# amazon-science/crossnorm-selfnorm

Hardware: AMD Instinct MI355X
Metric: fused CNSN fwd+bwd GB/s vs HBM roofline (higher is better)
Workload: dtype f32

## Files before the change

### crossnorm-selfnorm_amd/_ffi.py

```python
from __future__ import annotations

import ctypes as C
import os

_HERE = os.path.dirname(os.path.abspath(__file__))
LIB_PATH = os.environ.get("CNSN_LIB_PATH") or os.path.join(_HERE, "libcnsn_hip.so")

CNSN_F32, CNSN_BF16, CNSN_F16 = 0, 1, 2
STRATEGY_AUTO, STRATEGY_TWO_PASS, STRATEGY_RESIDENT, STRATEGY_LOCAL, STRATEGY_MONO = 0, 1, 2, 3, 4
ADD_NONE, ADD_PRE, ADD_POST = 0, 1, 2
LAYOUT_NCHW, LAYOUT_NHWC = 0, 1
PATHS = {0: "streaming", 1: "packed", 2: "resident", 3: "local", 4: "mono"}
ABI_VERSION = 9
PERM_INLINE_MAX = 1024
E_UNSUPPORTED = -9


class Problem(C.Structure):
    _fields_ = [
        ("struct_bytes", C.c_int32), ("dtype", C.c_int32),
        ("N", C.c_int32), ("C", C.c_int32), ("H", C.c_int32), ("W", C.c_int32),
        ("cn_active", C.c_int32), ("content_box", C.c_int32 * 4), ("style_box", C.c_int32 * 4),
        ("lam", C.c_float), ("eps_cn", C.c_float),
        ("sn_active", C.c_int32), ("sn_two", C.c_int32), ("sn_training", C.c_int32),
        ("eps_sn", C.c_float), ("eps_bn", C.c_float), ("momentum", C.c_float),
        ("strategy", C.c_int32), ("layout", C.c_int32),
        ("context", C.c_void_p), ("context_bytes", C.c_uint64),
        ("perm_host", C.c_void_p),
    ]


class Gate(C.Structure):
    _fields_ = [("fc_weight", C.c_void_p), ("bn_weight", C.c_void_p), ("bn_bias", C.c_void_p),
                ("running_mean", C.c_void_p), ("running_var", C.c_void_p), ("num_batches_tracked", C.c_void_p)]


class GateGrad(C.Structure):
    _fields_ = [("d_fc_weight", C.c_void_p), ("d_bn_weight", C.c_void_p), ("d_bn_bias", C.c_void_p)]


class BnTail(C.Structure):
    _fields_ = [("struct_bytes", C.c_int32), ("training", C.c_int32), ("eps", C.c_float), ("momentum", C.c_float),
                ("weight", C.c_void_p), ("bias", C.c_void_p), ("running_mean", C.c_void_p), ("running_var", C.c_void_p),
                ("num_batches_tracked", C.c_void_p)]


class Ibn(C.Structure):
    _fields_ = [("struct_bytes", C.c_int32), ("dtype", C.c_int32), ("N", C.c_int32), ("C", C.c_int32), ("H", C.c_int32),
                ("W", C.c_int32), ("half", C.c_int32), ("relu", C.c_int32), ("eps_in", C.c_float), ("reserved", C.c_int32),
                ("in_weight", C.c_void_p), ("in_bias", C.c_void_p), ("bn", BnTail), ("context", C.c_void_p),
                ("context_bytes", C.c_uint64)]


class BnAct(C.Structure):
    _fields_ = [("struct_bytes", C.c_int32), ("dtype", C.c_int32), ("N", C.c_int32), ("C", C.c_int32), ("H", C.c_int32),
                ("W", C.c_int32), ("relu", C.c_int32), ("add", C.c_int32), ("bn", BnTail), ("context", C.c_void_p),
                ("context_bytes", C.c_uint64)]


class ArenaStats(C.Structure):
    _fields_ = [("struct_bytes", C.c_int32), ("device", C.c_int32), ("chunk_bytes", C.c_uint64), ("mapped_bytes", C.c_uint64),
                ("in_use_bytes", C.c_uint64), ("blocks", C.c_uint64), ("blocks_in_use", C.c_uint64), ("hits", C.c_uint64),
                ("misses", C.c_uint64), ("failed", C.c_uint64), ("probed", C.c_uint64), ("tries", C.c_uint64),
                ("evicted", C.c_uint64), ("limit_bytes", C.c_uint64), ("broken", C.c_uint64)]


class Epilogue(C.Structure):
    _fields_ = [("struct_bytes", C.c_int32), ("add_mode", C.c_int32), ("relu", C.c_int32),
                ("reserved", C.c_int32), ("addend", C.c_void_p), ("sum_out", C.c_void_p)]


SIGNATURES = {
    "cnsn_abi_version": (C.c_int, []),
    "cnsn_status_string": (C.c_char_p, [C.c_int]),
    "cnsn_context_bytes": (C.c_size_t, [C.POINTER(Problem)]),
    "cnsn_context_init": (C.c_int, [C.c_void_p, C.c_size_t, C.c_void_p]),
    "cnsn_resident_timeouts": (C.c_int, []),
    "cnsn_resident_enable": (None, [C.c_int]),
    "cnsn_resident_rearm": (C.c_int, []),
    "cnsn_resident_degraded": (C.c_int, []),
    "cnsn_reload_env": (None, []),
    "cnsn_set_wait_ms": (None, [C.c_int]),
    "cnsn_wait_ms": (C.c_int, []),
    "cnsn_set_headroom_cus": (None, [C.c_int]),
    "cnsn_headroom_cus": (C.c_int, []),
    "cnsn_arena_map": (C.c_void_p, [C.c_size_t, C.c_int, C.c_void_p]),
    "cnsn_arena_unmap": (None, [C.c_void_p, C.c_size_t, C.c_int, C.c_void_p]),
    "cnsn_arena_alloc": (C.c_void_p, [C.c_int, C.c_size_t, C.c_void_p]),
    "cnsn_arena_record_stream": (C.c_int, [C.c_void_p, C.c_void_p]),
    "cnsn_arena_set_limit": (C.c_int, [C.c_int, C.c_uint64]),
    "cnsn_arena_free": (C.c_int, [C.c_void_p]),
    "cnsn_arena_trim": (C.c_size_t, [C.c_int]),
    "cnsn_arena_owns": (C.c_int, [C.c_void_p]),
    "cnsn_arena_stats": (C.c_int, [C.c_int, C.POINTER(ArenaStats)]),
    "cnsn_arena_set_chunk_bytes": (C.c_int, [C.c_size_t]),
    "cnsn_arena_prospect": (C.c_int, [C.c_int, C.c_size_t, C.c_int, C.c_int, C.c_void_p, C.POINTER(C.c_float)]),
    "cnsn_arena_block_gbps": (C.c_int, [C.c_void_p, C.POINTER(C.c_float)]),
    "cnsn_arena_set_tries": (C.c_int, [C.c_int]),
    "cnsn_saved_floats": (C.c_size_t, [C.POINTER(Problem)]),
    "cnsn_workspace_bytes": (C.c_size_t, [C.POINTER(Problem)]),
    "cnsn_forward": (C.c_int, [C.POINTER(Problem), C.c_void_p, C.c_void_p, C.c_void_p,
                               C.POINTER(Gate), C.POINTER(Gate), C.c_void_p, C.c_void_p,
                               C.c_void_p, C.c_size_t, C.c_void_p]),
    "cnsn_backward": (C.c_int, [C.POINTER(Problem), C.c_void_p, C.c_void_p, C.c_void_p, C.c_void_p,
                                C.POINTER(Gate), C.POINTER(Gate), C.c_void_p, C.c_void_p,
                                C.POINTER(GateGrad), C.POINTER(GateGrad), C.c_void_p, C.c_size_t,
                                C.c_void_p]),
    "cnsn_forward_fused": (C.c_int, [C.POINTER(Problem), C.POINTER(Epilogue), C.c_void_p, C.c_void_p,
                                     C.c_void_p, C.POINTER(Gate), C.POINTER(Gate), C.c_void_p,
                                     C.c_void_p, C.c_void_p, C.c_size_t, C.c_void_p]),
    "cnsn_backward_fused": (C.c_int, [C.POINTER(Problem), C.POINTER(Epilogue), C.c_void_p, C.c_void_p,
                                      C.c_void_p, C.c_void_p, C.POINTER(Gate), C.POINTER(Gate),
                                      C.c_void_p, C.c_void_p, C.c_void_p, C.POINTER(GateGrad),
                                      C.POINTER(GateGrad), C.c_void_p, C.c_size_t, C.c_void_p]),
    "cnsn_which_path": (C.c_int, [C.POINTER(Problem), C.POINTER(Epilogue), C.c_int, C.c_int]),
    "cnsn_keeps_sum": (C.c_int, [C.POINTER(Problem), C.POINTER(Epilogue)]),
    "cnsn_sn_cluster_plan": (C.c_int, [C.POINTER(Problem), C.POINTER(Epilogue), C.c_int]),
    "cnsn_bnrelu_plan": (C.c_int, [C.POINTER(Problem), C.POINTER(Epilogue), C.c_int]),
    "cnsn_bn_block_plan": (C.c_int, [C.POINTER(Problem), C.POINTER(Epilogue)]),
    "cnsn_forward_bn_block": (C.c_int, [C.POINTER(Problem), C.POINTER(Epilogue), C.POINTER(BnTail), C.POINTER(BnTail), C.c_void_p,
                                        C.POINTER(Gate), C.c_void_p, C.c_void_p, C.c_void_p, C.c_void_p, C.c_size_t, C.c_void_p]),
    "cnsn_backward_bn_block": (C.c_int, [C.POINTER(Problem), C.POINTER(Epilogue), C.POINTER(BnTail), C.POINTER(BnTail), C.c_void_p,
                                         C.c_void_p, C.POINTER(Gate), C.c_void_p, C.c_void_p, C.c_void_p, C.c_void_p,
                                         C.POINTER(GateGrad), C.c_void_p, C.c_void_p, C.c_void_p, C.c_void_p, C.c_void_p, C.c_size_t,
                                         C.c_void_p]),
    "cnsn_forward_bnrelu": (C.c_int, [C.POINTER(Problem), C.POINTER(Epilogue), C.POINTER(BnTail), C.c_void_p,
                                      C.POINTER(Gate), C.c_void_p, C.c_void_p, C.c_void_p, C.c_void_p, C.c_void_p,
                                      C.c_size_t, C.c_void_p]),
    "cnsn_backward_bnrelu": (C.c_int, [C.POINTER(Problem), C.POINTER(Epilogue), C.POINTER(BnTail), C.c_void_p, C.c_void_p,
                                       C.c_void_p, C.POINTER(Gate), C.c_void_p, C.c_void_p, C.c_void_p,
                                       C.POINTER(GateGrad), C.c_void_p, C.c_void_p, C.c_void_p, C.c_size_t, C.c_void_p]),
    "cnsn_ibn_plan": (C.c_int, [C.POINTER(Ibn), C.c_int, C.c_int]),
    "cnsn_ibn_saved_floats": (C.c_size_t, [C.POINTER(Ibn)]),
    "cnsn_ibn_workspace_bytes": (C.c_size_t, [C.POINTER(Ibn)]),
    "cnsn_forward_ibn": (C.c_int, [C.POINTER(Ibn), C.c_void_p, C.c_void_p, C.c_void_p, C.c_void_p, C.c_void_p, C.c_size_t,
                                   C.c_void_p]),
    "cnsn_backward_ibn": (C.c_int, [C.POINTER(Ibn), C.c_void_p, C.c_void_p, C.c_void_p, C.c_void_p, C.c_void_p, C.c_void_p,
                                    C.c_void_p, C.c_void_p, C.c_void_p, C.c_void_p, C.c_size_t, C.c_void_p]),
    "cnsn_bn_act_plan": (C.c_int, [C.POINTER(BnAct), C.c_int, C.c_int]),
    "cnsn_bn_act_saved_floats": (C.c_size_t, [C.POINTER(BnAct)]),
    "cnsn_bn_act_workspace_bytes": (C.c_size_t, [C.POINTER(BnAct)]),
    "cnsn_forward_bn_act": (C.c_int, [C.POINTER(BnAct), C.c_void_p, C.c_void_p, C.c_void_p, C.c_void_p, C.c_void_p, C.c_size_t,
                                      C.c_void_p]),
    "cnsn_backward_bn_act": (C.c_int, [C.POINTER(BnAct), C.c_void_p, C.c_void_p, C.c_void_p, C.c_void_p, C.c_void_p, C.c_void_p,
                                       C.c_void_p, C.c_void_p, C.c_void_p, C.c_size_t, C.c_void_p]),
    "cnsn_jsd_workspace_bytes": (C.c_size_t, [C.c_int]),
    "cnsn_jsd": (C.c_int, [C.c_void_p, C.c_void_p, C.c_void_p, C.c_int, C.c_int, C.c_int, C.c_void_p,
                           C.c_void_p, C.c_void_p, C.c_void_p, C.c_void_p, C.c_size_t, C.c_void_p]),
    "cnsn_plane_stats": (C.c_int, [C.c_void_p, C.c_int, C.c_int, C.c_int, C.c_int, C.c_int,
                                   C.POINTER(C.c_int32), C.c_float, C.c_void_p, C.c_void_p]),
    "cnsn_plane_stats_backward": (C.c_int, [C.c_void_p, C.c_int, C.c_int, C.c_int, C.c_int, C.c_int,
                                            C.POINTER(C.c_int32), C.c_void_p, C.c_void_p,
                                            C.c_void_p, C.c_void_p, C.c_void_p, C.c_void_p]),
    "cnsn_plane_affine": (C.c_int, [C.c_void_p, C.c_int, C.c_int, C.c_int, C.c_int, C.c_int,
                                    C.c_void_p, C.c_void_p, C.c_void_p, C.c_void_p]),
    "cnsn_plane_dot": (C.c_int, [C.c_void_p, C.c_void_p, C.c_int, C.c_int, C.c_int, C.c_int,
                                 C.c_int, C.c_void_p, C.c_void_p]),
    "cnsn_plane_dot_shifted": (C.c_int, [C.c_void_p, C.c_void_p, C.c_int, C.c_int, C.c_int, C.c_int,
                                         C.c_int, C.c_void_p, C.c_void_p, C.c_void_p]),
    "cnsn_plane_combine": (C.c_int, [C.c_void_p, C.c_void_p, C.c_int, C.c_int, C.c_int, C.c_int,
                                     C.c_int, C.c_void_p, C.c_void_p, C.c_void_p]),
}

_lib = None


class CnsnError(RuntimeError):
    pass


def lib():
    global _lib
    if _lib is None:
        if not os.path.exists(LIB_PATH):
            raise CnsnError(
                f"{LIB_PATH} is missing: the CrossNorm/SelfNorm HIP library has not been built. "
                "Run `python __graft_entry__.py` (hipcc --offload-arch=gfx950). There is no "
                "CPU or eager fallback.")
        handle = C.CDLL(LIB_PATH)
        for name, (res, args) in SIGNATURES.items():
            fn = getattr(handle, name)
            fn.restype, fn.argtypes = res, args
        got = handle.cnsn_abi_version()
        if got != ABI_VERSION:
            raise CnsnError(f"libcnsn_hip.so ABI {got} != binding ABI {ABI_VERSION}")
        _lib = handle
    return _lib


GLUE_DIR = os.path.join(_HERE, "_glue")
GLUE_PATH = os.path.join(GLUE_DIR, "cnsn_glue.so")
_glue = None
_glue_tried = False


def glue():
    global _glue, _glue_tried
    if _glue_tried:
        return _glue
    _glue_tried = True
    if os.environ.get("CNSN_NO_GLUE") == "1" or not os.path.exists(GLUE_PATH):
        return None
    lib()
    C.CDLL(LIB_PATH, mode=C.RTLD_GLOBAL)
    import importlib.machinery
    import importlib.util
    import torch
    loader = importlib.machinery.ExtensionFileLoader("cnsn_glue", GLUE_PATH)
    spec = importlib.util.spec_from_loader("cnsn_glue", loader)
    mod = importlib.util.module_from_spec(spec)
    loader.exec_module(mod)
    if mod.abi_version() != ABI_VERSION:
        raise CnsnError(f"cnsn_glue.so was built against ABI {mod.abi_version()}, binding expects {ABI_VERSION}")
    _glue = mod
    return _glue


_timeouts_reported = 0
_defer_depth = 0


def _timeout_count() -> int:
    return lib().cnsn_resident_timeouts()


_TIMEOUT_TEXT = ("{what}: an earlier cluster-resident launch timed out waiting for part of its grid ({n} so far) — the GPU "
                 "is shared with work that kept it off the device for seconds.  The outputs of the step that was in flight "
                 "are invalid: repeat it.  The library now uses the two-pass kernels (CNSN_RESIDENT=0 selects them from "
                 "the start).")


def check_resident_health(what: str):
    global _timeouts_reported
    if _defer_depth:
        return
    n = _timeout_count()
    if n > _timeouts_reported:
        _timeouts_reported = n
        raise CnsnError(_TIMEOUT_TEXT.format(what=what, n=n))


class deferred_timeouts:

    def __enter__(self):
        global _defer_depth
        _defer_depth += 1
        return self

    def __exit__(self, *exc):
        global _defer_depth
        _defer_depth -= 1
        return False


def poll_timeouts() -> int:
    global _timeouts_reported
    n = _timeout_count()
    new = max(0, n - _timeouts_reported)
    _timeouts_reported = max(n, _timeouts_reported)
    return new


def settle_step(device=None, raise_on_timeout: bool = True) -> int:
    import torch
    torch.cuda.current_stream(device).synchronize()
    if not raise_on_timeout:
        return poll_timeouts()
    check_resident_health("training step")
    return 0


_plan_caches = []


def forget_plans():
    for c in _plan_caches:
        c.clear()


def reload_env():
    lib().cnsn_reload_env()
    forget_plans()


_following = False


def follow_environ():
    global _following
    if _following:
        return
    _following = True
    put, unset = os.putenv, os.unsetenv

    def reread(key):
        if os.fsdecode(key).startswith("CNSN_") and _lib is not None:
            _lib.cnsn_reload_env()
            forget_plans()

    def putenv(key, value):
        put(key, value)
        reread(key)

    def unsetenv(key):
        unset(key)
        reread(key)

    os.putenv, os.unsetenv = putenv, unsetenv


def default_headroom_cus() -> int:
    try:
        ch = int(os.environ.get("NCCL_MAX_NCHANNELS", "") or 16)
    except ValueError:
        ch = 16
    return max(0, min(2 * ch, 64))


def under_process_group_defaults() -> dict:
    try:
        import torch.distributed as dist
        if not (dist.is_available() and dist.is_initialized() and dist.get_world_size() > 1):
            return {}
        handle = lib()
        if "CNSN_WAIT_MS" not in os.environ:
            handle.cnsn_set_wait_ms(2000)
        if "CNSN_HEADROOM_CUS" not in os.environ:
            handle.cnsn_set_headroom_cus(default_headroom_cus())
            forget_plans()
        return {"wait_ms": int(handle.cnsn_wait_ms()), "headroom_cus": int(handle.cnsn_headroom_cus())}
    except Exception:
        return {}


def check(status: int, what: str):
    if status != 0:
        msg = lib().cnsn_status_string(status).decode()
        if status == -7:
            raise ValueError(f"{what}: {msg}")
        raise CnsnError(f"{what} failed with status {status}: {msg}")


def box4(b):
    arr = (C.c_int32 * 4)(-1, -1, -1, -1)
    if b is not None:
        for i in range(4):
            arr[i] = int(b[i])
    return arr
```

### crossnorm-selfnorm_amd/callers/_sites.py

```python
import os

import numpy as np
import torch

FUSE_BLOCK = os.environ.get("CNSN_FUSE_BLOCK", "1") != "0"
FUSE_TAIL = FUSE_BLOCK and os.environ.get("CNSN_FUSE_TAIL", "1") != "0"
FUSE_BN_ACT = os.environ.get("CNSN_BN_ACT", "1") != "0"


def residual_sum(cnsn, pos, residual, skip, relu, skip_first=False):
    fb = getattr(cnsn, "forward_block", None) if (FUSE_BLOCK and cnsn is not None) else None
    fusable = (fb is not None and pos in ("post", "residual", "identity") and residual.is_cuda
               and residual.shape == skip.shape and residual.dtype == skip.dtype)
    if fusable:
        if pos == "post":
            a, b = (skip, residual) if skip_first else (residual, skip)
            return fb(a, b, add_mode="pre", relu=relu)
        if pos == "residual":
            return fb(residual, skip, add_mode="post", relu=relu)
        return fb(skip, residual, add_mode="post", relu=relu)
    if pos == "residual":
        residual = cnsn(residual)
    elif pos == "identity":
        skip = cnsn(skip)
    y = torch.add(skip, residual) if skip_first else residual + skip
    if pos == "post":
        y = cnsn(y)
    return torch.relu(y) if relu else y


def make_cnsn(impl, cnsn_type, crop, beta, width):
    assert cnsn_type in ("sn", "cn", "cnsn")
    cross = impl.CrossNorm(crop=crop, beta=beta) if "cn" in cnsn_type else None
    selfn = impl.SelfNorm(width) if "sn" in cnsn_type else None
    return impl.CNSN(crossnorm=cross, selfnorm=selfn)


class CrossNormSites:

    def _collect_sites(self, impl, cnsn_type, active_num):
        object.__setattr__(self, "cn_modules", [m for m in self.modules() if isinstance(m, impl.CrossNorm)])
        if cnsn_type is not None and "cn" in cnsn_type:
            self.cn_num = len(self.cn_modules)
            self.active_num = active_num
            assert self.cn_num > 0 and self.active_num > 0

    def _enable_cross_norm(self):
        picked = np.random.choice(self.cn_num, self.active_num, replace=False).tolist()
        for i in picked:
            self.cn_modules[i].active = True
        return picked
```

### crossnorm-selfnorm_amd/callers/resnet.py

```python
import torch
import torch.nn as nn

from . import _sites
from ._sites import CrossNormSites, make_cnsn, residual_sum
from .bn_act import bn_act
from .ibn import IBN, InstanceNorm2d


class _Bottleneck(nn.Module):
    expansion = 4

    def __init__(self, impl, c_in, planes, stride, downsample, pos, beta, crop, cnsn_type, ibn=None):
        super().__init__()
        c_out = planes * self.expansion
        self.ibn = ibn
        self.conv1 = nn.Conv2d(c_in, planes, 1, bias=False)
        self.bn1 = IBN(planes) if ibn == "a" else nn.BatchNorm2d(planes)
        self.conv2 = nn.Conv2d(planes, planes, 3, stride, 1, bias=False)
        self.bn2 = nn.BatchNorm2d(planes)
        self.conv3 = nn.Conv2d(planes, c_out, 1, bias=False)
        self.bn3 = nn.BatchNorm2d(c_out)
        if ibn == "b":
            self.IN = InstanceNorm2d(c_out, affine=True)
        self.relu = nn.ReLU(inplace=True)
        self.downsample = downsample
        if ibn == "b" and pos == "post":
            cnsn_type = None
        if cnsn_type is not None:
            assert pos in ("residual", "pre", "post", "identity")
            self.cnsn = make_cnsn(impl, cnsn_type, crop, beta, c_in if pos == "pre" else c_out)
        self.pos = pos if cnsn_type is not None else None

    def forward(self, x):
        h = self.cnsn(x) if self.pos == "pre" else x
        h = self.conv1(h)
        h = self.bn1.forward_act(h) if self.ibn == "a" else bn_act(self.bn1, h)
        h = bn_act(self.bn2, self.conv2(h))
        h = self.conv3(h)
        if self.ibn == "b":
            skip = x if self.downsample is None else self.downsample(x)
            h = self.bn3(h)
            if self.pos == "residual":
                h = self.cnsn(h)
            elif self.pos == "identity":
                skip = self.cnsn(skip)
            return self.IN.forward_act(h, skip, relu=True)
        fb = getattr(getattr(self, "cnsn", None), "forward_bn_block", None) if (_sites.FUSE_BLOCK and self.pos == "post") else None
        if fb is not None and h.is_cuda:
            if self.downsample is None:
                return fb(h, self.bn3, x, relu=True)
            if len(self.downsample) == 2 and isinstance(self.downsample[1], nn.BatchNorm2d):
                return fb(h, self.bn3, self.downsample[0](x), relu=True, identity_bn=self.downsample[1])
            return fb(h, self.bn3, self.downsample(x), relu=True)
        skip = x if self.downsample is None else self.downsample(x)
        if getattr(self, "cnsn", None) is None:
            return bn_act(self.bn3, h, skip)
        return residual_sum(self.cnsn, self.pos, self.bn3(h), skip, relu=True)


class ResNet50CNSN(nn.Module, CrossNormSites):
    def __init__(self, num_classes=1000, layers=(3, 4, 6, 3), active_num=1, pos="post", beta=None, crop=None,
                 cnsn_type="sn", impl=None):
        super().__init__()
        if impl is None:
            from .. import cnsn as impl
        self.conv1 = nn.Conv2d(3, 64, 7, 2, 3, bias=False)
        self.bn1 = nn.BatchNorm2d(64)
        self.relu = nn.ReLU(inplace=True)
        self.maxpool = nn.MaxPool2d(3, 2, 1)
        kw = dict(pos=pos, beta=beta, crop=crop, cnsn_type=cnsn_type)
        c_in = 64
        for i, (planes, blocks) in enumerate(zip((64, 128, 256, 512), layers)):
            stride = 1 if i == 0 else 2
            units = []
            for b in range(blocks):
                down = None
                if b == 0 and (stride != 1 or c_in != planes * 4):
                    down = nn.Sequential(nn.Conv2d(c_in, planes * 4, 1, stride, bias=False), nn.BatchNorm2d(planes * 4))
                units.append(_Bottleneck(impl, c_in, planes, stride if b == 0 else 1, down, **kw))
                c_in = planes * 4
            setattr(self, f"layer{i + 1}", nn.Sequential(*units))
        self.avgpool = nn.AdaptiveAvgPool2d((1, 1))
        self.fc = nn.Linear(c_in, num_classes)
        for m in self.modules():
            if isinstance(m, nn.Conv2d):
                nn.init.kaiming_normal_(m.weight, mode="fan_out", nonlinearity="relu")
            elif isinstance(m, nn.BatchNorm2d):
                nn.init.constant_(m.weight, 1)
                nn.init.constant_(m.bias, 0)
        self._collect_sites(impl, cnsn_type, active_num)

    def forward(self, x, aug=False):
        if aug:
            self._enable_cross_norm()
        x = self.maxpool(bn_act(self.bn1, self.conv1(x)))
        x = self.layer4(self.layer3(self.layer2(self.layer1(x))))
        return self.fc(torch.flatten(self.avgpool(x), 1))
```

### crossnorm-selfnorm_amd/cnsn.py

```python
from __future__ import annotations

import functools
from dataclasses import dataclass
from typing import Optional, Tuple

import numpy as np
import torch
import torch.nn as nn

from . import functional as _F
from .functional import FusedConfig, GateParams

__all__ = ["calc_ins_mean_std", "instance_norm_mix", "cn_rand_bbox", "cn_op_2ins_space_chan",
           "CrossNorm", "SelfNorm", "CNSN"]

Box = Tuple[int, int, int, int]
_CROPS = ("neither", "style", "content", "both")


def _is_f64(x) -> bool:
    return isinstance(x, torch.Tensor) and x.dtype == torch.float64


def calc_ins_mean_std(x, eps=1e-5):
    assert x.dim() == 4
    if _is_f64(x):
        mean, std = _F.PlaneStats.apply(x.float(), float(eps), None, True)
        return mean.double(), std.double()
    return _F.PlaneStats.apply(x, float(eps), None)


def instance_norm_mix(content_feat, style_feat):
    assert content_feat.size()[:2] == style_feat.size()[:2]
    if _is_f64(content_feat):
        return instance_norm_mix(content_feat.float(), style_feat.float()).double()
    s_mean, s_std = calc_ins_mean_std(style_feat)
    c_mean, c_std = calc_ins_mean_std(content_feat)
    scale = s_std.float() / c_std.float()
    shift = s_mean.float() - c_mean.float() * scale
    return _F.PlaneAffine.apply(content_feat, scale, shift)


def cn_rand_bbox(size, beta, bbx_thres):
    ext2, ext3 = int(size[2]), int(size[3])
    plane = float(ext2 * ext3)
    while True:
        side = np.sqrt(np.random.beta(beta, beta))
        half2, half3 = int(ext2 * side) // 2, int(ext3 * side) // 2
        mid2 = np.random.randint(ext2)
        mid3 = np.random.randint(ext3)
        x1, x2 = max(mid2 - half2, 0), min(mid2 + half2, ext2)
        y1, y2 = max(mid3 - half3, 0), min(mid3 + half3, ext3)
        if (x2 - x1) * (y2 - y1) / plane > bbx_thres:
            return int(x1), int(y1), int(x2), int(y2)


@dataclass
class CNDraws:
    perm: torch.Tensor
    style_box: Optional[Box] = None
    chan_perm: Optional[torch.Tensor] = None
    content_box: Optional[Box] = None


def draw_cn(size, crop, beta, bbx_thres=0.1, chan=False) -> CNDraws:
    assert crop in _CROPS
    d = CNDraws(perm=torch.randperm(int(size[0])))
    if crop in ("style", "both"):
        d.style_box = cn_rand_bbox(size, beta=beta, bbx_thres=bbx_thres)
    if chan:
        d.chan_perm = torch.randperm(int(size[1]))
    if crop in ("content", "both"):
        d.content_box = cn_rand_bbox(size, beta=beta, bbx_thres=bbx_thres)
    return d


def _cn_config(d: CNDraws, lam) -> FusedConfig:
    return FusedConfig(cn_active=True, content_box=d.content_box, style_box=d.style_box, lam=lam)


def cn_op_2ins_space_chan(x, crop='neither', beta=1, bbx_thres=0.1, lam=None, chan=False, draws=None):
    assert crop in _CROPS
    if draws is None:
        draws = draw_cn(x.size(), crop, beta, bbx_thres, chan)
    if _is_f64(x):
        return _F.fused_cnsn(x.float(), _cn_config(draws, lam), perm=draws.perm, chan_perm=draws.chan_perm).double()
    return _F.fused_cnsn(x, _cn_config(draws, lam), perm=draws.perm, chan_perm=draws.chan_perm)


class CrossNorm(nn.Module):

    def __init__(self, crop=None, beta=None):
        super().__init__()
        self.active = False
        self.crop, self.beta = crop, beta
        self.cn_op = functools.partial(cn_op_2ins_space_chan, crop=crop, beta=beta)
        self.next_draws: Optional[CNDraws] = None

    def _take_draws(self, x) -> CNDraws:
        d, self.next_draws = self.next_draws, None
        return d if d is not None else draw_cn(x.size(), self.crop, self.beta)

    def forward(self, x):
        if self.training and self.active:
            x = self.cn_op(x, draws=self._take_draws(x))
        self.active = False
        return x


class SelfNorm(nn.Module):

    def __init__(self, chan_num, is_two=False):
        super().__init__()
        self.g_fc = nn.Conv1d(chan_num, chan_num, kernel_size=2, bias=False, groups=chan_num)
        self.g_bn = nn.BatchNorm1d(chan_num)
        if is_two is True:
            self.f_fc = nn.Conv1d(chan_num, chan_num, kernel_size=2, bias=False, groups=chan_num)
            self.f_bn = nn.BatchNorm1d(chan_num)
        else:
            self.f_fc = None

    @staticmethod
    def _gate(fc, bn, counter=None) -> GateParams:
        rm, rv = bn.running_mean, bn.running_var
        if rm is None or rv is None:
            w = fc.weight
            rm = torch.zeros(w.shape[0], dtype=torch.float32, device=w.device)
            rv = torch.ones(w.shape[0], dtype=torch.float32, device=w.device)
        return GateParams(fc.weight, bn.weight, bn.bias, rm, rv, counter)

    @staticmethod
    def _bn_call_state(bn, in_kernel=False):
        momentum = 0.0 if bn.momentum is None else float(bn.momentum)
        counter = None
        if bn.training and bn.track_running_stats and bn.num_batches_tracked is not None:
            if in_kernel and bn.momentum is not None and bn.num_batches_tracked.is_cuda and not _F.LEGACY_LAUNCHES:
                counter = bn.num_batches_tracked
            else:
                bn.num_batches_tracked.add_(1)
                if bn.momentum is None:
                    momentum = 1.0 / float(bn.num_batches_tracked)
        use_batch = bn.training or (bn.running_mean is None and bn.running_var is None)
        if in_kernel:
            return use_batch, float(bn.eps), momentum, counter
        return use_batch, float(bn.eps), momentum

    @staticmethod
    def _bn_peek(bn):
        use_batch = bn.training or (bn.running_mean is None and bn.running_var is None)
        return use_batch, float(bn.eps), (None if bn.momentum is None else float(bn.momentum)), bool(
            bn.training and bn.track_running_stats)

    def _fusable(self) -> bool:
        mods = self._modules
        g_bn = mods["g_bn"]

        def affine(bn):
            par, own = bn._parameters, bn.__dict__
            return (par.get("weight") if "weight" in par else own.get("weight")) is not None and \
                   (par.get("bias") if "bias" in par else own.get("bias")) is not None

        if type(g_bn) is not nn.BatchNorm1d or not affine(g_bn):
            return False
        if self.f_fc is None:
            return True
        f_bn = mods["f_bn"]
        if type(f_bn) is not nn.BatchNorm1d or not affine(f_bn):
            return False
        return self._bn_peek(g_bn) == self._bn_peek(f_bn)

    def _forward_composed(self, x):
        b, c = int(x.size(0)), int(x.size(1))
        mean, std = _F.PlaneStats.apply(x, 1e-12, None, True)
        with torch.autocast(device_type=x.device.type, enabled=False):
            stats = torch.cat((mean.view(b, c, 1), std.view(b, c, 1)), -1)
            g_y = torch.sigmoid(self.g_bn(self.g_fc(stats))).view(b, c, 1, 1)
            if self.f_fc is not None:
                f_y = torch.sigmoid(self.f_bn(self.f_fc(stats))).view(b, c, 1, 1)
                shift = mean * (f_y - g_y)
            else:
                shift = torch.zeros_like(g_y)
        return _F.PlaneAffine.apply(x, g_y, shift)

    def _fused_args(self):
        *state, counter = self._bn_call_state(self.g_bn, in_kernel=True)
        state = tuple(state)
        g = self._gate(self.g_fc, self.g_bn, counter)
        f = None
        if self.f_fc is not None:
            *state_f, counter_f = self._bn_call_state(self.f_bn, in_kernel=True)
            state_f = tuple(state_f)
            if state_f != state:
                raise _F._ffi.CnsnError(
                    "SelfNorm(is_two=True): g_bn and f_bn must share mode, eps and momentum "
                    f"(g_bn: training/eps/momentum = {state}, f_bn: {state_f})")
            f = self._gate(self.f_fc, self.f_bn, counter_f)
        use_batch, eps, momentum = state
        kw = dict(sn_active=True, sn_two=f is not None, sn_training=use_batch, eps_bn=eps, momentum=momentum)
        return kw, g, f

    def _fused_args_peek(self):
        bn = self.g_bn
        use_batch = bn.training or (bn.running_mean is None and bn.running_var is None)
        kw = dict(sn_active=True, sn_two=self.f_fc is not None, sn_training=use_batch, eps_bn=float(bn.eps),
                  momentum=0.0 if bn.momentum is None else float(bn.momentum))
        return kw, None, None

    def forward(self, x):
        if _is_f64(x):
            return self.forward(x.float()).double()
        if not self._fusable():
            return self._forward_composed(x)
        kw, g, f = self._fused_args()
        return _F.fused_cnsn(x, FusedConfig(**kw), g=g, f=f)


class CNSN(nn.Module):

    def __init__(self, crossnorm, selfnorm):
        super().__init__()
        self.crossnorm = crossnorm
        self.selfnorm = selfnorm

    def forward(self, x):
        if _is_f64(x):
            return self.forward(x.float()).double()
        cn, sn = self.crossnorm, self.selfnorm
        fuse = (cn is not None and sn is not None and type(cn) is CrossNorm and type(sn) is SelfNorm and sn._fusable()
                and cn.active and cn.training)
        if not fuse:
            if cn and cn.active:
                x = cn(x)
            if sn:
                x = sn(x)
            return x
        d = cn._take_draws(x)
        cn.active = False
        kw, g, f = sn._fused_args()
        cfg = FusedConfig(cn_active=True, content_box=d.content_box, style_box=d.style_box, **kw)
        return _F.fused_cnsn(x, cfg, perm=d.perm, chan_perm=d.chan_perm, g=g, f=f)

    def forward_block(self, x, addend=None, add_mode="none", relu=False):
        assert add_mode in ("none", "pre", "post")
        assert (addend is None) == (add_mode == "none")
        if _is_f64(x):
            return self.forward_block(x.float(), None if addend is None else addend.float(), add_mode, relu).double()
        cn, sn = self.crossnorm, self.selfnorm
        ours = (cn is None or type(cn) is CrossNorm) and (sn is None or (type(sn) is SelfNorm and sn._fusable()))
        cn_on = cn is not None and cn.active and cn.training
        if not ours or not (cn_on or sn is not None):
            if add_mode == "pre":
                x = x + addend
            x = self.forward(x)
            if add_mode == "post":
                x = x + addend
            return torch.relu(x) if relu else x
        kw, g, f, perm, chan = {}, None, None, None, None
        if cn is not None and cn.active:
            if cn_on:
                d = cn._take_draws(x)
                kw.update(cn_active=True, content_box=d.content_box, style_box=d.style_box)
                perm, chan = d.perm, d.chan_perm
            cn.active = False
        if sn is not None:
            skw, g, f = sn._fused_args()
            kw.update(skw)
        cfg = FusedConfig(add_mode=add_mode, relu=bool(relu), **kw)
        return _F.fused_cnsn(x, cfg, perm=perm, chan_perm=chan, g=g, f=f, addend=addend)

    def forward_bn_block(self, conv_out, bn, identity, relu=True, identity_bn=None):
        cn, sn = self.crossnorm, self.selfnorm
        armed = cn is not None and cn.active

        def plain(m):
            return type(m) is nn.BatchNorm2d and m.affine and m.track_running_stats and m.training
        fused = (plain(bn) and (identity_bn is None or plain(identity_bn)) and sn is not None
                 and type(sn) is SelfNorm and sn.f_fc is None and sn._fusable() and not armed and conv_out.is_cuda
                 and (cn is None or type(cn) is CrossNorm) and identity.shape == conv_out.shape
                 and identity.dtype == conv_out.dtype and not torch.cuda.is_current_stream_capturing())
        if fused:
            kw, _, _ = sn._fused_args_peek()
            fused = kw["sn_training"] and _F.bn_block_plan(conv_out, FusedConfig(add_mode="pre", relu=bool(relu), **kw))
        if not fused:
            skip = identity if identity_bn is None else identity_bn(identity)
            return self.forward_block(bn(conv_out), skip, add_mode="pre", relu=relu)
        kw, g, _ = sn._fused_args()
        _, bn_eps, bn_mom, bn_counter = SelfNorm._bn_call_state(bn, in_kernel=True)
        cfg = FusedConfig(add_mode="pre", relu=bool(relu), **kw)
        extra = ()
        if identity_bn is not None:
            _, e2, m2, c2 = SelfNorm._bn_call_state(identity_bn, in_kernel=True)
            extra = (identity_bn.weight, identity_bn.bias, identity_bn.running_mean, identity_bn.running_var, e2, m2, c2)
        return _F.FusedBnBlock.apply(conv_out, identity, cfg, g.fc_weight, g.bn_weight, g.bn_bias, g.running_mean, g.running_var,
                                     bn.weight, bn.bias, bn.running_mean, bn.running_var, bn_eps, bn_mom, g.num_batches_tracked,
                                     bn_counter, *extra)

    def forward_block_bn(self, x, addend, add_mode, bn, want_y=True):
        assert add_mode in ("none", "pre")
        cn, sn = self.crossnorm, self.selfnorm
        armed = cn is not None and cn.active
        fused = (type(bn) is nn.BatchNorm2d and bn.affine and bn.track_running_stats and sn is not None
                 and type(sn) is SelfNorm and sn.f_fc is None and sn._fusable() and not armed and x.is_cuda
                 and (cn is None or type(cn) is CrossNorm))
        if fused:
            kw, g, _ = sn._fused_args_peek()
            cfg = FusedConfig(add_mode=add_mode, relu=False, **kw)
            fused = _F.bnrelu_plan_cached(x, cfg, torch.is_grad_enabled())
        if not fused:
            y = self.forward_block(x, addend, add_mode=add_mode, relu=False) if add_mode != "none" else self.forward(x)
            return (y if want_y else None), torch.relu(bn(y))
        kw, g, _ = sn._fused_args()
        bn_batch, bn_eps, bn_mom, bn_counter = SelfNorm._bn_call_state(bn, in_kernel=True)
        cfg = FusedConfig(add_mode=add_mode, relu=False, **kw)
        return _F.fused_cnsn_tail(x, cfg, addend, bool(want_y), g, bn.weight, bn.bias, bn.running_mean, bn.running_var,
                                  bn_batch, bn_eps, bn_mom, bn_counter)
```

### crossnorm-selfnorm_amd/csrc/cnsn_env.h

```cpp
#pragma once

namespace cnsn {

enum Knob {
    K_LOCAL_LB = 0,
    K_LOCAL_CG,
    K_STAGGER,
    K_WAIT_MS,
    K_FAULT_INJECT,
    K_DEBUG,
    K_PROF,
    K_MONO,
    K_MONO_RELOAD,
    K_NO_PACKED,
    K_MID_TILE,
    K_SNX,
    K_RESIDENT,
    K_CONTEXT,
    K_EPOCH_START,
    K_KEEP,
    K_PIPE,
    K_WIDE,
    K_PONG,
    K_SNXCN,
    K_ARENA_CHUNK_MB,
    K_XCD,
    K_HEADROOM_CUS,
    K_ARENA_TRIES,
    K_ARENA_SPREAD_GB,
    K_MID_BLOCK,
    K_NHWC_FUSED,
    K_ARENA_MAX_MB,
    K_COUNT
};

const char* knob(Knob k);
void reload_knobs();

}
```

### crossnorm-selfnorm_amd/csrc/cnsn_env.hip

```cpp
#include "cnsn_env.h"

#include <cstdlib>
#include <mutex>
#include <string>

namespace cnsn {
namespace {

const char* const kNames[K_COUNT] = {
    "CNSN_LOCAL_LB", "CNSN_LOCAL_CG", "CNSN_STAGGER",     "CNSN_WAIT_MS", "CNSN_FAULT_INJECT", "CNSN_DEBUG",
    "CNSN_PROF",     "CNSN_MONO",     "CNSN_MONO_RELOAD", "CNSN_NO_PACKED", "CNSN_MID_TILE",   "CNSN_SNX",
    "CNSN_RESIDENT", "CNSN_CONTEXT",  "CNSN_EPOCH_START", "CNSN_KEEP",    "CNSN_PIPE",         "CNSN_WIDE",
    "CNSN_PONG",
    "CNSN_SNXCN",
    "CNSN_ARENA_CHUNK_MB",
    "CNSN_XCD",
    "CNSN_HEADROOM_CUS",
    "CNSN_ARENA_TRIES",
    "CNSN_ARENA_SPREAD_GB",
    "CNSN_MID_BLOCK",
    "CNSN_NHWC_FUSED",
    "CNSN_ARENA_MAX_MB",
};

struct Table {
    std::string text[K_COUNT];
    const char* value[K_COUNT];
    std::mutex mu;
    Table() { read(); }
    void read() {
        std::lock_guard<std::mutex> lock(mu);
        for (int k = 0; k < K_COUNT; ++k) {
            const char* e = getenv(kNames[k]);
            if (e) {
                text[k] = e;
                value[k] = text[k].c_str();
            } else {
                text[k].clear();
                value[k] = nullptr;
            }
        }
    }
};

Table& table() {
    static Table t;
    return t;
}

struct AtLoad {
    AtLoad() { (void)table(); }
} g_at_load;

}

const char* knob(Knob k) { return table().value[k]; }
void reload_knobs() { table().read(); }

}
```

### crossnorm-selfnorm_amd/csrc/cnsn_fused.hip

```cpp
#include "../../include/cnsn_hip.h"

#include <hip/hip_runtime.h>

#include "cnsn_fused_stream_kernels.h"
#include "cnsn_host_plan.h"
#include "cnsn_local.h"
#include "cnsn_mono.h"
#include "cnsn_nhwc.h"
#include "cnsn_wide.h"
#include "cnsn_packed.h"
#include "cnsn_resident_fused.h"
#include "cnsn_resident_sn.h"

using namespace cnsn;

namespace {

struct EpiPlan {
    int add;
    int relu;
    const void* addend;
    void* sum_out;
};

int parse_epilogue(const cnsn_epilogue_t* epi, EpiPlan& e) {
    e = EpiPlan{ADD_NONE, 0, nullptr, nullptr};
    if (!epi) return CNSN_OK;
    if (epi->struct_bytes != (int32_t)sizeof(cnsn_epilogue_t)) return CNSN_E_STRUCT;
    if (epi->add_mode != CNSN_ADD_NONE && epi->add_mode != CNSN_ADD_PRE && epi->add_mode != CNSN_ADD_POST)
        return CNSN_E_UNSUPPORTED;
    e.add = epi->add_mode;
    e.relu = epi->relu ? 1 : 0;
    e.addend = epi->addend;
    if (e.add != ADD_NONE) {
        if (!e.addend) return CNSN_E_NULL;
        if (((uintptr_t)e.addend & 15u) != 0) return CNSN_E_ALIGN;
    }
    e.sum_out = epi->sum_out;
    if (e.sum_out) {
        if (e.add != ADD_PRE) return CNSN_E_UNSUPPORTED;
        if (((uintptr_t)e.sum_out & 15u) != 0) return CNSN_E_ALIGN;
    }
    return CNSN_OK;
}

int parse_epilogue_shape(const cnsn_epilogue_t* epi, EpiPlan& e) {
    e = EpiPlan{ADD_NONE, 0, nullptr, nullptr};
    if (!epi) return CNSN_OK;
    if (epi->struct_bytes != (int32_t)sizeof(cnsn_epilogue_t)) return CNSN_E_STRUCT;
    if (epi->add_mode != CNSN_ADD_NONE && epi->add_mode != CNSN_ADD_PRE && epi->add_mode != CNSN_ADD_POST)
        return CNSN_E_UNSUPPORTED;
    e.add = epi->add_mode;
    e.relu = epi->relu ? 1 : 0;
    return CNSN_OK;
}

template <typename F>
inline void with_add(int add, F&& f) {
    if (add == ADD_PRE)
        f(IntTag<ADD_PRE>{});
    else if (add == ADD_POST)
        f(IntTag<ADD_POST>{});
    else
        f(IntTag<ADD_NONE>{});
}

}

extern "C" {

int cnsn_which_path(const cnsn_problem_t* prob, const cnsn_epilogue_t* epi, int has_chan_perm, int backward) {
    EpiPlan e;
    int st = parse_epilogue_shape(epi, e);
    if (st) return st;
    Plan pl;
    st = make_plan(prob, pl);
    if (st) return st;
    const cnsn_problem_t& p = pl.pr;
    const bool chan = p.cn_active && has_chan_perm;
    const bool bwd = backward != 0;
    if (p.layout == CNSN_LAYOUT_NHWC)
        return (chan || !nhwc_supported(pl, false)) ? CNSN_E_UNSUPPORTED : (nhwc_fused_ok(pl) ? CNSN_PATH_RESIDENT : CNSN_PATH_STREAMING);
    const bool fused = bwd ? (e.relu || e.add == ADD_PRE) : (e.relu || e.add != ADD_NONE);
    if (resident_sn_prefers(p, pl.boxed, fused ? e.add : ADD_NONE, fused ? e.relu : 0, bwd)) return CNSN_PATH_RESIDENT;
    if (wide_plan(pl, fused ? e.add : 0, bwd, chan).ok) return CNSN_PATH_MONO;
    if (mono_plan(pl, fused ? e.add : 0, bwd).ok) return CNSN_PATH_MONO;
    if (mono_cn_plan(pl, chan, fused ? e.add : 0, bwd).ok) return CNSN_PATH_MONO;
    if (local_plan(pl, fused ? e.add : 0, bwd).ok) return CNSN_PATH_LOCAL;
    if (resident_sn_plan(p, pl.boxed, fused ? e.add : ADD_NONE, fused ? e.relu : 0, bwd).ok) return CNSN_PATH_RESIDENT;
    if (bwd && !fused && resident_sn_cn_plan(p, pl.boxed, chan).ok) return CNSN_PATH_RESIDENT;
    if (fused ? resident_fused_plan(p, pl.boxed, chan, e.add, bwd).ok : resident_plan(p, pl.boxed, chan, bwd).ok)
        return CNSN_PATH_RESIDENT;
    if (resident_split_plan(p, pl.boxed, chan, fused ? e.add : ADD_NONE, fused ? e.relu : 0, bwd).ok) return CNSN_PATH_RESIDENT;
    PackedGeom pg;
    return packed_plan(pl, pg) ? CNSN_PATH_PACKED : CNSN_PATH_STREAMING;
}

int cnsn_sn_cluster_plan(const cnsn_problem_t* prob, const cnsn_epilogue_t* epi, int backward) {
    EpiPlan e;
    int st = parse_epilogue_shape(epi, e);
    if (st) return st;
    Plan pl;
    st = make_plan(prob, pl);
    if (st) return st;
    const bool bwd = backward != 0;
    const bool fused = bwd ? (e.relu || e.add == ADD_PRE) : (e.relu || e.add != ADD_NONE);
    if (pl.pr.layout == CNSN_LAYOUT_NHWC) return 0;
    if (resident_sn_prefers(pl.pr, pl.boxed, fused ? e.add : ADD_NONE, fused ? e.relu : 0, bwd)) return 1;
    if (wide_plan(pl, fused ? e.add : 0, bwd).ok || mono_plan(pl, fused ? e.add : 0, bwd).ok ||
        local_plan(pl, fused ? e.add : 0, bwd).ok)
        return 0;
    if (bwd && !fused && resident_sn_cn_plan(pl.pr, pl.boxed, false).ok) return 1;
    return resident_sn_plan(pl.pr, pl.boxed, fused ? e.add : ADD_NONE, fused ? e.relu : 0, bwd).ok ? 1 : 0;
}

int cnsn_keeps_sum(const cnsn_problem_t* prob, const cnsn_epilogue_t* epi) {
    EpiPlan e;
    if (!prob || parse_epilogue_shape(epi, e) != CNSN_OK || e.add != ADD_PRE || prob->layout != CNSN_LAYOUT_NHWC) return 0;
    Plan pl;
    if (make_plan(prob, pl) != CNSN_OK) return 0;
    return nhwc_supported(pl, false) ? 1 : 0;
}

namespace {
int bn_block_parse(const cnsn_problem_t* prob, const cnsn_epilogue_t* epi, const cnsn_bn_tail_t* bn, Plan& pl, EpiPlan& e, bool shape_only,
                   bool check_health = true) {
    int st = shape_only ? parse_epilogue_shape(epi, e) : parse_epilogue(epi, e);
    if (st) return st;
    st = make_plan(prob, pl);
    if (st) return st;
    if (bn && bn->struct_bytes != (int32_t)sizeof(cnsn_bn_tail_t)) return CNSN_E_STRUCT;
    if (pl.pr.layout != CNSN_LAYOUT_NHWC || e.add != ADD_PRE || e.sum_out || !nhwc_bnhead_ok(pl, check_health) || (bn && !bn->training))
        return CNSN_E_UNSUPPORTED;
    return CNSN_OK;
}
}

int cnsn_bn_block_plan(const cnsn_problem_t* prob, const cnsn_epilogue_t* epi) {
    Plan pl;
    EpiPlan e;
    const int st = bn_block_parse(prob, epi, nullptr, pl, e, true);
    return st == CNSN_OK ? 1 : (st == CNSN_E_UNSUPPORTED ? 0 : st);
}

int cnsn_forward_bn_block(const cnsn_problem_t* prob, const cnsn_epilogue_t* epi, const cnsn_bn_tail_t* bn,
                          const cnsn_bn_tail_t* bn_skip, const void* conv_out, const cnsn_gate_t* g, void* y, float* saved, float* bn_stats,
                          void* workspace, size_t workspace_bytes, void* stream_) {
    if (!bn) return CNSN_E_NULL;
    if (bn_skip && (bn_skip->struct_bytes != (int32_t)sizeof(cnsn_bn_tail_t))) return CNSN_E_STRUCT;
    if (bn_skip && (!bn_skip->weight || !bn_skip->bias || !bn_skip->running_mean || !bn_skip->running_var)) return CNSN_E_NULL;
    if (bn_skip && !bn_skip->training) return CNSN_E_UNSUPPORTED;
    Plan pl;
    EpiPlan e;
    const int st = bn_block_parse(prob, epi, bn, pl, e, false);
    if (st) return st;
    if (!conv_out || !y || !workspace || !bn_stats || !bn->weight || !bn->bias || !bn->running_mean || !bn->running_var) return CNSN_E_NULL;
    if ((((uintptr_t)conv_out | (uintptr_t)y | (uintptr_t)workspace | (uintptr_t)bn_stats) & 15u) != 0) return CNSN_E_ALIGN;
    if (!gate_ok(g)) return CNSN_E_NULL;
    return nhwc_bnhead_forward(pl, e.relu, *bn, bn_skip, conv_out, e.addend, gate_dev(g), y, saved, bn_stats, workspace, workspace_bytes,
                               (hipStream_t)stream_);
}

int cnsn_backward_bn_block(const cnsn_problem_t* prob, const cnsn_epilogue_t* epi, const cnsn_bn_tail_t* bn,
                           const cnsn_bn_tail_t* bn_skip, const void* grad_y, const void* conv_out, const cnsn_gate_t* g, const float* saved,
                           const float* bn_stats, void* grad_conv_out, void* grad_identity, const cnsn_gate_grad_t* dg, float* d_bn_weight,
                           float* d_bn_bias, float* d_bn_skip_weight, float* d_bn_skip_bias, void* workspace, size_t workspace_bytes,
                           void* stream_) {
    if (!bn) return CNSN_E_NULL;
    if (bn_skip && (bn_skip->struct_bytes != (int32_t)sizeof(cnsn_bn_tail_t))) return CNSN_E_STRUCT;
    if (bn_skip && (!bn_skip->weight || !d_bn_skip_weight || !d_bn_skip_bias)) return CNSN_E_NULL;
    Plan pl;
    EpiPlan e;
    const int st = bn_block_parse(prob, epi, bn, pl, e, false, false);
    if (st) return st;
    if (!grad_y || !conv_out || !grad_conv_out || !grad_identity || !saved || !bn_stats || !workspace || !bn->weight) return CNSN_E_NULL;
    if ((((uintptr_t)grad_y | (uintptr_t)conv_out | (uintptr_t)grad_conv_out | (uintptr_t)grad_identity | (uintptr_t)workspace |
          (uintptr_t)bn_stats) & 15u) != 0)
        return CNSN_E_ALIGN;
    if (!gate_ok(g) || !dg || !dg->d_fc_weight || !dg->d_bn_weight || !dg->d_bn_bias) return CNSN_E_NULL;
    return nhwc_bnhead_backward(pl, e.relu, *bn, bn_skip, grad_y, conv_out, e.addend, gate_dev(g), saved, bn_stats, grad_conv_out,
                                grad_identity, gate_grad_dev(dg), d_bn_weight, d_bn_bias, d_bn_skip_weight, d_bn_skip_bias, workspace,
                                workspace_bytes, (hipStream_t)stream_);
}

int cnsn_forward_fused(const cnsn_problem_t* prob, const cnsn_epilogue_t* epi, const void* x, const int64_t* perm,
                       const int64_t* chan_perm, const cnsn_gate_t* g, const cnsn_gate_t* f, void* y, float* saved,
                       void* workspace, size_t workspace_bytes, void* stream_) {
    EpiPlan e;
    int st = parse_epilogue(epi, e);
    if (st) return st;
    if (prob && prob->layout == CNSN_LAYOUT_NHWC) {
        Plan pl;
        st = make_plan(prob, pl);
        if (st) return st;
        if (!x || !y || !workspace) return CNSN_E_NULL;
        if ((((uintptr_t)x | (uintptr_t)y | (uintptr_t)workspace) & 15u) != 0) return CNSN_E_ALIGN;
        if (chan_perm || !nhwc_supported(pl, false)) return CNSN_E_UNSUPPORTED;
        if (pl.pr.sn_active && !gate_ok(g)) return CNSN_E_NULL;
        if (pl.pr.sn_active && pl.pr.sn_two && !gate_ok(f)) return CNSN_E_NULL;
        return nhwc_forward(pl, e.add, e.relu, x, e.addend, perm, gate_dev(g), gate_dev(f), y, saved, workspace, workspace_bytes,
                            (hipStream_t)stream_, e.sum_out);
    }
    if (e.sum_out) return CNSN_E_UNSUPPORTED;
    if (e.add == ADD_NONE && !e.relu)
        return cnsn_forward(prob, x, perm, chan_perm, g, f, y, saved, workspace, workspace_bytes, stream_);
    Plan pl;
    st = make_plan(prob, pl);
    if (st) return st;
    const cnsn_problem_t& p = pl.pr;
    if (!x || !y || !workspace) return CNSN_E_NULL;
    if ((((uintptr_t)x | (uintptr_t)y | (uintptr_t)workspace) & 15u) != 0) return CNSN_E_ALIGN;
    const bool perm_inline = p.cn_active && !perm;
    if (perm_inline && (!p.perm_host || chan_perm || p.N > CNSN_PERM_INLINE_MAX)) return p.perm_host ? CNSN_E_UNSUPPORTED : CNSN_E_NULL;
    if (p.sn_active && !gate_ok(g)) return CNSN_E_NULL;
    if (p.sn_active && p.sn_two && !gate_ok(f)) return CNSN_E_NULL;
    if (workspace_bytes < workspace_bytes_of(pl)) return CNSN_E_WORKSPACE;
    hipStream_t stream = (hipStream_t)stream_;
    pl.mid.save_coefs = (e.relu && saved) ? 1 : 0;

    double* mom = (double*)workspace;
    double* saved_d = saved ? (double*)saved : mom + 6 * pl.P;
    float* coef = (float*)(mom + 6 * pl.P + saved_doubles_of(pl));

    if (resident_sn_prefers(p, pl.boxed, e.add, e.relu, false)) {
        st = resident_sn_forward(pl.pr, pl.mid, e.add, e.relu, x, e.addend, gate_dev(g), y, saved ? saved_d : nullptr, workspace,
                                 stream);
        if (st != CNSN_E_UNSUPPORTED) return st;
    }
    {
        const WidePlan wp = wide_plan(pl, e.add, false, chan_perm != nullptr);
        if (wp.ok && !perm_inline) {
            st = wide_forward(pl, wp, e.add, e.relu, x, e.addend, perm, gate_dev(g), y, saved ? saved_d : nullptr, stream);
            if (st != CNSN_E_UNSUPPORTED) return st;
        }
    }
    {
        const MonoPlan mp = mono_plan(pl, e.add, false);
        if (mp.ok) {
            st = mono_forward(pl, mp, e.add, e.relu, x, e.addend, gate_dev(g), gate_dev(f), y, saved ? saved_d : nullptr, stream);
            if (st != CNSN_E_UNSUPPORTED) return st;
        }
    }
    {
        const MonoPlan mp = mono_cn_plan(pl, chan_perm != nullptr, e.add, false);
        if (mp.ok && !perm_inline) {
            st = mono_cn_forward(pl, mp, e.add, e.relu, x, e.addend, perm, gate_dev(g), y, saved ? saved_d : nullptr, stream);
            if (st != CNSN_E_UNSUPPORTED) return st;
        }
    }
    {
        const LocalPlan lp = local_plan(pl, e.add, false);
        if (lp.ok) {
            st = local_forward(pl, lp, e.add, e.relu, x, e.addend, gate_dev(g), gate_dev(f), y, saved ? saved_d : nullptr,
                               stream);
            if (st != CNSN_E_UNSUPPORTED) return st;
        }
    }
    if (resident_sn_plan(p, pl.boxed, e.add, e.relu, false).ok) {
        st = resident_sn_forward(pl.pr, pl.mid, e.add, e.relu, x, e.addend, gate_dev(g), y, saved ? saved_d : nullptr, workspace,
                                 stream);
        if (st != CNSN_E_UNSUPPORTED) return st;
    }
    if (resident_fused_plan(p, pl.boxed, p.cn_active && chan_perm != nullptr, e.add, false).ok) {
        st = resident_fused_forward(pl.pr, pl.cb, pl.sb, pl.boxed, pl.mid, e.add, e.relu, x, e.addend, perm, gate_dev(g),
                                    gate_dev(f), y, saved ? saved_d : nullptr, workspace, stream);
        if (st != CNSN_E_UNSUPPORTED) return st;
    }
    if (resident_split_plan(p, pl.boxed, p.cn_active && chan_perm != nullptr, e.add, e.relu, false).ok) {
        st = resident_split_forward(pl.pr, pl.cb, pl.sb, pl.boxed, pl.mid, e.add, e.relu, x, e.addend, perm, gate_dev(g),
                                    gate_dev(f), y, saved ? saved_d : nullptr, workspace, stream);
        if (st != CNSN_E_UNSUPPORTED) return st;
    }

    if (perm_inline) return CNSN_E_UNSUPPORTED;
    PackedGeom pg;
    if (packed_plan(pl, pg)) {
        packed_stats(pl, pg, e.add, x, e.addend, mom, stream);
        launch_mid_fwd(pl, mom, perm, chan_perm, gate_dev(g), gate_dev(f), coef, saved_d, stream);
        packed_apply_fwd(pl, pg, e.add, e.relu, x, e.addend, y, coef, stream);
        return launch_status();
    }

    const int blocks = blocks_for(pl.geom.P, pl.shape.lpp);
    dispatch(p.dtype, pl.shape, [&](auto tt, auto vt, auto lt) {
        using T = typename decltype(tt)::type;
        constexpr int VEC = decltype(vt)::value, LPP = decltype(lt)::value;
        if (e.add == ADD_PRE) {
            if (pl.boxed)
                fused_stats_kernel<T, VEC, LPP, true><<<blocks, kBlock, 0, stream>>>((const T*)x, (const T*)e.addend, pl.geom, mom);
            else
                fused_stats_kernel<T, VEC, LPP, false><<<blocks, kBlock, 0, stream>>>((const T*)x, (const T*)e.addend, pl.geom, mom);
        } else {
            if (pl.boxed)
                plane_stats_kernel<T, VEC, LPP, true><<<blocks, kBlock, 0, stream>>>((const T*)x, pl.geom, mom, nullptr, 0.f);
            else
                plane_stats_kernel<T, VEC, LPP, false><<<blocks, kBlock, 0, stream>>>((const T*)x, pl.geom, mom, nullptr, 0.f);
        }
    });
    launch_mid_fwd(pl, mom, perm, chan_perm, gate_dev(g), gate_dev(f), coef, saved_d, stream);
    const size_t P = pl.P;
    ApplyCoef cf{coef + FC_A_IN * P, coef + FC_XR * P, coef + FC_B_IN * P, coef + FC_A_OUT * P, coef + FC_B_OUT * P};
    dispatch(p.dtype, pl.shape, [&](auto tt, auto vt, auto lt) {
        using T = typename decltype(tt)::type;
        constexpr int VEC = decltype(vt)::value, LPP = decltype(lt)::value;
        with_add(e.add, [&](auto at) {
            constexpr int ADD = decltype(at)::value;
            if (pl.boxed)
                fused_apply_fwd_kernel<T, VEC, LPP, true, ADD><<<blocks, kBlock, 0, stream>>>(
                    (const T*)x, (const T*)e.addend, (T*)y, pl.geom, cf, e.relu);
            else
                fused_apply_fwd_kernel<T, VEC, LPP, false, ADD><<<blocks, kBlock, 0, stream>>>(
                    (const T*)x, (const T*)e.addend, (T*)y, pl.geom, cf, e.relu);
        });
    });
    return launch_status();
}

int cnsn_backward_fused(const cnsn_problem_t* prob, const cnsn_epilogue_t* epi, const void* grad_y, const void* x,
                        const int64_t* perm, const int64_t* chan_perm, const cnsn_gate_t* g, const cnsn_gate_t* f,
                        const float* saved, void* grad_x, void* grad_addend, const cnsn_gate_grad_t* dg,
                        const cnsn_gate_grad_t* df, void* workspace, size_t workspace_bytes, void* stream_) {
    EpiPlan e;
    int st = parse_epilogue(epi, e);
    if (st) return st;
    if (prob && prob->layout == CNSN_LAYOUT_NHWC) {
        Plan pl;
        st = make_plan(prob, pl);
        if (st) return st;
        if (!grad_y || !x || !grad_x || !saved || !workspace) return CNSN_E_NULL;
        if ((((uintptr_t)x | (uintptr_t)grad_y | (uintptr_t)grad_x | (uintptr_t)grad_addend | (uintptr_t)workspace) & 15u) != 0)
            return CNSN_E_ALIGN;
        if (chan_perm || !nhwc_supported(pl, false)) return CNSN_E_UNSUPPORTED;
        if (pl.pr.sn_active && (!gate_ok(g) || !gate_grad_ok(dg))) return CNSN_E_NULL;
        if (pl.pr.sn_active && pl.pr.sn_two && (!gate_ok(f) || !gate_grad_ok(df))) return CNSN_E_NULL;
        return nhwc_backward(pl, e.add, e.relu, grad_y, x, e.addend, perm, gate_dev(g), gate_dev(f), saved, grad_x, grad_addend,
                             gate_grad_dev(dg), gate_grad_dev(df), workspace, workspace_bytes, (hipStream_t)stream_);
    }
    if (!e.relu && e.add != ADD_PRE)
        return cnsn_backward(prob, grad_y, x, perm, chan_perm, g, f, saved, grad_x, dg, df, workspace, workspace_bytes,
                             stream_);
    Plan pl;
    st = make_plan(prob, pl);
    if (st) return st;
    const cnsn_problem_t& p = pl.pr;
    if (!grad_y || !x || !grad_x || !saved || !workspace) return CNSN_E_NULL;
    if (e.add == ADD_POST && !grad_addend) return CNSN_E_NULL;
    if ((((uintptr_t)x | (uintptr_t)grad_y | (uintptr_t)grad_x | (uintptr_t)grad_addend | (uintptr_t)workspace) & 15u) != 0)
        return CNSN_E_ALIGN;
    const bool perm_inline = p.cn_active && !perm;
    if (perm_inline && (!p.perm_host || chan_perm || p.N > CNSN_PERM_INLINE_MAX)) return p.perm_host ? CNSN_E_UNSUPPORTED : CNSN_E_NULL;
    if (p.sn_active && (!gate_ok(g) || !gate_grad_ok(dg))) return CNSN_E_NULL;
    if (p.sn_active && p.sn_two && (!gate_ok(f) || !gate_grad_ok(df))) return CNSN_E_NULL;
    if (workspace_bytes < workspace_bytes_of(pl)) return CNSN_E_WORKSPACE;
    hipStream_t stream = (hipStream_t)stream_;

    const size_t P = pl.P;
    double* tmp = (double*)workspace;
    float* sums = (float*)(tmp + BT_ROWS * P);
    float* coef = sums + 4 * P;
    const double* saved_d = (const double*)saved;

    if (resident_sn_prefers(p, pl.boxed, e.add, e.relu, true)) {
        st = resident_sn_backward(pl.pr, pl.mid, e.add, e.relu, grad_y, x, e.addend, gate_dev(g), saved_d, grad_x,
                                  gate_grad_dev(dg), workspace, stream);
        if (st != CNSN_E_UNSUPPORTED) return st;
    }
    {
        const WidePlan wp = wide_plan(pl, e.add, true, chan_perm != nullptr);
        if (wp.ok && !perm_inline) {
            st = wide_backward(pl, wp, e.add, e.relu, grad_y, x, e.addend, perm, gate_dev(g), saved_d, grad_x, gate_grad_dev(dg), stream);
            if (st != CNSN_E_UNSUPPORTED) return st;
        }
    }
    {
        const MonoPlan mp = mono_plan(pl, e.add, true);
        if (mp.ok) {
            st = mono_backward(pl, mp, e.add, e.relu, grad_y, x, e.addend, gate_dev(g), gate_dev(f), saved_d, grad_x,
                               gate_grad_dev(dg), gate_grad_dev(df), stream);
            if (st != CNSN_E_UNSUPPORTED) return st;
        }
    }
    {
        const MonoPlan mp = mono_cn_plan(pl, chan_perm != nullptr, e.add, true);
        if (mp.ok && !perm_inline) {
            st = mono_cn_backward(pl, mp, e.add, e.relu, grad_y, x, e.addend, perm, gate_dev(g), saved_d, grad_x,
                                  gate_grad_dev(dg), stream);
            if (st != CNSN_E_UNSUPPORTED) return st;
        }
    }
    {
        const LocalPlan lp = local_plan(pl, e.add, true);
        if (lp.ok) {
            st = local_backward(pl, lp, e.add, e.relu, grad_y, x, e.addend, gate_dev(g), gate_dev(f), saved_d, grad_x,
                                gate_grad_dev(dg), gate_grad_dev(df), stream);
            if (st != CNSN_E_UNSUPPORTED) return st;
        }
    }
    if (resident_sn_plan(p, pl.boxed, e.add, e.relu, true).ok) {
        st = resident_sn_backward(pl.pr, pl.mid, e.add, e.relu, grad_y, x, e.addend, gate_dev(g), saved_d, grad_x,
                                  gate_grad_dev(dg), workspace, stream);
        if (st != CNSN_E_UNSUPPORTED) return st;
    }
    if (resident_fused_plan(p, pl.boxed, p.cn_active && chan_perm != nullptr, e.add, true).ok) {
        st = resident_fused_backward(pl.pr, pl.cb, pl.sb, pl.boxed, pl.mid, e.add, e.relu, grad_y, x, e.addend, perm,
                                     gate_dev(g), gate_dev(f), saved_d, grad_x, grad_addend, gate_grad_dev(dg),
                                     gate_grad_dev(df), workspace, stream);
        if (st != CNSN_E_UNSUPPORTED) return st;
    }
    if (resident_split_plan(p, pl.boxed, p.cn_active && chan_perm != nullptr, e.add, e.relu, true).ok) {
        st = resident_split_backward(pl.pr, pl.cb, pl.sb, pl.boxed, pl.mid, e.add, e.relu, grad_y, x, e.addend, perm,
                                     gate_dev(g), gate_dev(f), saved_d, grad_x, grad_addend, gate_grad_dev(dg),
                                     gate_grad_dev(df), workspace, stream);
        if (st != CNSN_E_UNSUPPORTED) return st;
    }

    if (perm_inline) return CNSN_E_UNSUPPORTED;
    PackedGeom pg;
    if (packed_plan(pl, pg)) {
        packed_reduce(pl, pg, e.add, e.relu, grad_y, x, e.addend, saved_d, sums, stream);
        launch_mid_bwd(pl, sums, saved_d, perm, chan_perm, gate_dev(g), gate_dev(f), gate_grad_dev(dg), gate_grad_dev(df),
                       tmp, coef, stream);
        packed_apply_bwd(pl, pg, e.add, e.relu, grad_y, x, e.addend, grad_x, grad_addend, coef, saved_d, stream);
        return launch_status();
    }

    const int blocks = blocks_for(pl.geom.P, pl.shape.lpp);
    dispatch(p.dtype, pl.shape, [&](auto tt, auto vt, auto lt) {
        using T = typename decltype(tt)::type;
        constexpr int VEC = decltype(vt)::value, LPP = decltype(lt)::value;
        with_add(e.add, [&](auto at) {
            constexpr int ADD = decltype(at)::value;
            if (pl.boxed)
                fused_bwd_reduce_kernel<T, VEC, LPP, true, ADD><<<blocks, kBlock, 0, stream>>>(
                    (const T*)grad_y, (const T*)x, (const T*)e.addend, pl.geom, saved_d, e.relu, sums);
            else
                fused_bwd_reduce_kernel<T, VEC, LPP, false, ADD><<<blocks, kBlock, 0, stream>>>(
                    (const T*)grad_y, (const T*)x, (const T*)e.addend, pl.geom, saved_d, e.relu, sums);
        });
    });
    launch_mid_bwd(pl, sums, saved_d, perm, chan_perm, gate_dev(g), gate_dev(f), gate_grad_dev(dg), gate_grad_dev(df), tmp,
                   coef, stream);
    dispatch(p.dtype, pl.shape, [&](auto tt, auto vt, auto lt) {
        using T = typename decltype(tt)::type;
        constexpr int VEC = decltype(vt)::value, LPP = decltype(lt)::value;
        with_add(e.add, [&](auto at) {
            constexpr int ADD = decltype(at)::value;
            if (pl.boxed)
                fused_apply_bwd_kernel<T, VEC, LPP, true, ADD><<<blocks, kBlock, 0, stream>>>(
                    (const T*)grad_y, (const T*)x, (const T*)e.addend, (T*)grad_x, (T*)grad_addend, pl.geom, coef, saved_d,
                    e.relu);
            else
                fused_apply_bwd_kernel<T, VEC, LPP, false, ADD><<<blocks, kBlock, 0, stream>>>(
                    (const T*)grad_y, (const T*)x, (const T*)e.addend, (T*)grad_x, (T*)grad_addend, pl.geom, coef, saved_d,
                    e.relu);
        });
    });
    return launch_status();
}

}
```

### crossnorm-selfnorm_amd/csrc/cnsn_nhwc.h

```cpp
#pragma once
#include <type_traits>

#include "cnsn_host_plan.h"

namespace cnsn {

namespace nhwc_host {

inline int vec_of(int dtype) { return 16 / elem_bytes(dtype); }
inline size_t align256(size_t v) { return (v + 255) & ~(size_t)255; }
inline bool aligned16(const void* p) { return ((uintptr_t)p & 15u) == 0; }

template <typename F>
bool dispatch_t(int dtype, F&& f) {
    if (dtype == CNSN_F32) return f(TypeTag<float>{}, IntTag<4>{}), true;
    if (dtype == CNSN_BF16) return f(TypeTag<bf16_t>{}, IntTag<8>{}), true;
    if (dtype == CNSN_F16) return f(TypeTag<_Float16>{}, IntTag<8>{}), true;
    return false;
}

template <typename F>
void with_add(int add, F&& f) {
    if (add == CNSN_ADD_PRE)
        f(IntTag<CNSN_ADD_PRE>{});
    else if (add == CNSN_ADD_POST)
        f(IntTag<CNSN_ADD_POST>{});
    else
        f(IntTag<CNSN_ADD_NONE>{});
}

template <typename F>
void with_flag(bool on, F&& f) {
    if (on)
        f(std::true_type{});
    else
        f(std::false_type{});
}

struct Carver {
    char* base;
    size_t used = 0;
    explicit Carver(void* workspace) : base((char*)workspace) {}
    template <typename T = float>
    T* take(size_t bytes) {
        T* p = base ? (T*)(base + used) : nullptr;
        used += align256(bytes);
        return p;
    }
    size_t bytes() const { return used + 256; }
};

inline int keep_first_read(int tensors, size_t tensor_bytes) { return (size_t)tensors * tensor_bytes <= ((size_t)320 << 20) ? 1 : 0; }

}

bool nhwc_supported(const Plan& pl, bool has_chan_perm);
size_t nhwc_extra_bytes(const Plan& pl);
int nhwc_forward(Plan& pl, int add, int relu, const void* x, const void* addend, const int64_t* perm, GateDev g, GateDev f, void* y,
                 float* saved, void* workspace, size_t workspace_bytes, hipStream_t stream, void* sum_out = nullptr);
int nhwc_backward(Plan& pl, int add, int relu, const void* gy, const void* x, const void* addend, const int64_t* perm, GateDev g,
                  GateDev f, const float* saved, void* dx, void* d_addend, GateGradDev dg, GateGradDev df, void* workspace,
                  size_t workspace_bytes, hipStream_t stream);

size_t nhwc_workspace_bytes(const Plan& pl);

bool nhwc_slim_record(const Plan& pl);
bool nhwc_fused_ok(const Plan& pl, bool check_health = true);
size_t nhwc_fused_extra_bytes(const Plan& pl);
int nhwc_fused_forward(Plan& pl, int add, int relu, const void* x, const void* addend, GateDev g, void* y, float* saved,
                       void* workspace, size_t workspace_bytes, hipStream_t stream, void* sum_out = nullptr);
int nhwc_fused_backward(Plan& pl, int add, int relu, const void* gy, const void* x, const void* addend, GateDev g,
                        const float* saved, void* dx, void* d_addend, GateGradDev dg, void* workspace, size_t workspace_bytes,
                        hipStream_t stream);
void nhwc_slim_from_saved(const Plan& pl, const double* saved_d, float* slim, hipStream_t stream);
void nhwc_saved_from_slim(const Plan& pl, const float* slim, int relu, double* saved_d, float* rows, hipStream_t stream);

bool nhwc_bnhead_ok(const Plan& pl, bool check_health = true);
size_t nhwc_bnhead_extra_bytes(const Plan& pl);
int nhwc_bnhead_forward(Plan& pl, int relu, const cnsn_bn_tail_t& bn, const cnsn_bn_tail_t* bn2, const void* conv_out, const void* identity,
                        GateDev gg, void* y, float* saved, float* bn_stats, void* workspace, size_t workspace_bytes, hipStream_t stream);
int nhwc_bnhead_backward(Plan& pl, int relu, const cnsn_bn_tail_t& bn, const cnsn_bn_tail_t* bn2, const void* gy, const void* conv_out,
                         const void* identity, GateDev gg, const float* saved, const float* bn_stats, void* d_conv, void* d_identity,
                         GateGradDev dg, float* dbn_w, float* dbn_b, float* dbn2_w, float* dbn2_b, void* workspace,
                         size_t workspace_bytes, hipStream_t stream);

}
```

### crossnorm-selfnorm_amd/csrc/cnsn_nhwc_bnhead_kernels.h

```cpp
#pragma once
#include "cnsn_nhwc_fused_kernels.h"

#ifndef CNSN_BNHEAD_UA
#define CNSN_BNHEAD_UA 2
#endif
#ifndef CNSN_BNHEAD_WG_PER_CU
#define CNSN_BNHEAD_WG_PER_CU 3
#endif

namespace cnsn {

enum BnSlimRow { SLB_E = SL_ROWS, SLB_DM, SLB_E2, SLB_DM2, SLB_ROWS };
__host__ __device__ inline size_t bn_slim_floats(size_t P, int C) { return (size_t)SLB_ROWS * P + 2 * (size_t)C; }
__host__ __device__ inline double* bn_slim_rstd(float* slim, size_t P) { return reinterpret_cast<double*>(slim + (size_t)SLB_ROWS * P); }
__host__ __device__ inline const double* bn_slim_rstd(const float* slim, size_t P) {
    return reinterpret_cast<const double*>(slim + (size_t)SLB_ROWS * P);
}
enum BnStatRow { BS_MEAN = 0, BS_RSTD, BS_ALPHA, BS_BETA, BS_ROWS };

struct BnHeadDev {
    const float* weight;
    const float* bias;
    float* run_mean;
    float* run_var;
    long long* nbt;
    float eps, momentum;
};

struct NhwcBnArgs {
    NhwcFusedArgs f;
    BnHeadDev bn;
    BnHeadDev bn2;
    double inv_r, unbias_r;
    float* kshift_b;
    float* chan;
    float* bn_stats;
    float* dbn_w;
    float* dbn_b;
    float* dbn2_w;
    float* dbn2_b;
};

template <int VEC, int NK, int NTOT>
__device__ __forceinline__ void nhwc_rows_sum_part(const NhwcGeom& g, const NhwcThread<VEC>& t, const float (&acc)[NK][VEC], int k0,
                                                   float* lds, float* __restrict__ part) {
    const int col = (int)threadIdx.x % g.tcb, width = g.tcb * VEC;
    if (t.r < g.rows) {
#pragma unroll
        for (int k = 0; k < NK; ++k)
#pragma unroll
            for (int j = 0; j < VEC; ++j) lds[((size_t)k * g.rows + t.r) * width + col * VEC + j] = t.active ? acc[k][j] : 0.f;
    }
    __syncthreads();
    const CohBuf pb(part);
    const int total = NK * width, first = (t.vc - col) * VEC;
    for (int ch = (int)threadIdx.x * 4; ch < total; ch += kBlock * 4) {
        const int k = ch / width, off = ch - k * width;
        if (first + off >= g.C) continue;
        float4 v = make_float4(0.f, 0.f, 0.f, 0.f);
        for (int q = 0; q < g.rows; ++q) {
            const float4 w = *reinterpret_cast<const float4*>(lds + ((size_t)k * g.rows + q) * width + off);
            v.x += w.x, v.y += w.y, v.z += w.z, v.w += w.w;
        }
        pb.st4(((size_t)t.s * NTOT + k0 + k) * g.P + (size_t)t.n * g.C + first + off, v.x, v.y, v.z, v.w);
    }
    __syncthreads();
}

template <int GC>
__device__ __forceinline__ double pick(const double (&v)[GC], int j) {
    double r = 0.0;
#pragma unroll
    for (int q = 0; q < GC; ++q)
        if (q == j) r = v[q];
    return r;
}

template <typename T>
__device__ __forceinline__ float bn_sum(float c, float b, float alpha, float beta) {
    const float x = to_float(from_float<T>(fmaf(alpha, c, beta)));
    return sum_t<T>(x, b);
}

template <typename T, bool TWO>
__device__ __forceinline__ float bn_skip(float c2, float alpha2, float beta2) {
    if constexpr (TWO)
        return to_float(from_float<T>(fmaf(alpha2, c2, beta2)));
    else
        return c2;
}

constexpr int kBnGc = 4;
constexpr int kBnFwd = 5;
constexpr int kBnBwd = 4;

template <typename T, int VEC, bool KEEP, bool TWO>
__global__ __launch_bounds__(kBlock, CNSN_BNHEAD_WG_PER_CU) void nhwc_bnhead_fwd_kernel(NhwcBnArgs a, const T* __restrict__ cv,
                                                                                         const T* __restrict__ idt, T* __restrict__ y,
                                                                                         GateDev gg) {
    extern __shared__ float lds[];
    __shared__ double red[4 * kBnGc];
    __shared__ int bar_flag;
    constexpr int GC = kBnGc;
    const NhwcGeom& g = a.f.g;

    for (int tile = blockIdx.x; tile < a.f.ntiles; tile += gridDim.x) {
        const NhwcThread<VEC> t(g, tile);
        float Kc[VEC], Kb[VEC], acc[3][VEC], acc2[2][VEC];
#pragma unroll
        for (int j = 0; j < VEC; ++j) Kc[j] = Kb[j] = acc[0][j] = acc[1][j] = acc[2][j] = acc2[0][j] = acc2[1][j] = 0.f;
        if (t.active) {
            const size_t o = t.elem(g, 0);
            const Vec<T, VEC> c0 = load_vec<T, VEC>(cv + o), b0 = load_vec<T, VEC>(idt + o);
#pragma unroll
            for (int j = 0; j < VEC; ++j) Kc[j] = to_float(c0.v[j]), Kb[j] = to_float(b0.v[j]);
            auto eat = [&](const Vec<T, VEC>& vc, const Vec<T, VEC>& vb) {
#pragma unroll
                for (int j = 0; j < VEC; ++j) {
                    const float dc = to_float(vc.v[j]) - Kc[j], db = to_float(vb.v[j]) - Kb[j];
                    acc[0][j] += dc;
                    acc[1][j] = fmaf(dc, dc, acc[1][j]);
                    acc[2][j] += db;
                    acc2[0][j] = fmaf(db, db, acc2[0][j]);
                    acc2[1][j] = fmaf(dc, db, acc2[1][j]);
                }
            };
            constexpr int U = CNSN_BNHEAD_UA;
            int p = t.p0 + t.r;
            for (; p + (U - 1) * g.rows < t.p1; p += U * g.rows) {
                Vec<T, VEC> vc[U], vb[U];
#pragma unroll
                for (int u = 0; u < U; ++u) {
                    const size_t e = t.elem(g, p + u * g.rows);
                    vc[u] = nhwc_ld<T, VEC, !KEEP>(cv + e);
                    vb[u] = nhwc_ld<T, VEC, !KEEP>(idt + e);
                }
#pragma unroll
                for (int u = 0; u < U; ++u) eat(vc[u], vb[u]);
            }
            for (; p < t.p1; p += g.rows) {
                const size_t e = t.elem(g, p);
                const Vec<T, VEC> vc = nhwc_ld<T, VEC, !KEEP>(cv + e), vb = nhwc_ld<T, VEC, !KEEP>(idt + e);
                eat(vc, vb);
            }
            if (t.s == 0 && t.r == 0) {
                CohBuf(a.f.kshift).store<VEC>(t.plane0(g), Kc);
                CohBuf(a.kshift_b).store<VEC>(t.plane0(g), Kb);
            }
        }
        nhwc_rows_sum_part<VEC, 3, kBnFwd>(g, t, acc, 0, lds, a.f.part);
        nhwc_rows_sum_part<VEC, 2, kBnFwd>(g, t, acc2, 3, lds, a.f.part);
    }
    if (!grid_barrier(a.f.bar, 1, &bar_flag)) {
        nhwc_mark_owed<T, VEC>(g, a.f.ntiles, y);
        return;
    }

    for (int slot = blockIdx.x; slot < a.f.ngroups; slot += gridDim.x) {
        const int grp = phase_b_group(slot, a.f.ngroups);
        const int c0 = grp * GC, n = threadIdx.x;
        const bool live = n < g.N;
        const size_t p0 = (size_t)(live ? n : 0) * g.C + c0;
        double Sc[GC], Qc[GC], Sb[GC], Qb[GC], Pcb[GC], Kc[GC], Kb[GC];
#pragma unroll
        for (int j = 0; j < GC; ++j) Sc[j] = Qc[j] = Sb[j] = Qb[j] = Pcb[j] = 0.0;
        const CohBuf pb(a.f.part);
        for (int s = 0; s < g.S; ++s) {
            const size_t base = (size_t)s * kBnFwd * g.P + p0;
            add_group_coh<GC>(pb, base, Sc);
            add_group_coh<GC>(pb, base + g.P, Qc);
            add_group_coh<GC>(pb, base + 2 * g.P, Sb);
            add_group_coh<GC>(pb, base + 3 * g.P, Qb);
            add_group_coh<GC>(pb, base + 4 * g.P, Pcb);
        }
        load_group_coh<GC>(CohBuf(a.f.kshift), p0, Kc);
        load_group_coh<GC>(CohBuf(a.kshift_b), p0, Kb);
        const double M = (double)g.M;
        double mc[GC], M2c[GC], mb[GC], M2b[GC], Ccb[GC], t1[GC], m2d[GC], v2d[GC];
#pragma unroll
        for (int j = 0; j < GC; ++j) {
            mc[j] = Kc[j] + Sc[j] / M;
            M2c[j] = Qc[j] - Sc[j] * Sc[j] / M;
            mb[j] = Kb[j] + Sb[j] / M;
            M2b[j] = Qb[j] - Sb[j] * Sb[j] / M;
            Ccb[j] = Pcb[j] - Sc[j] * Sb[j] / M;
            t1[j] = live ? mc[j] : 0.0;
        }
        block_sum_d<GC>(t1, red);
#pragma unroll
        for (int j = 0; j < GC; ++j) {
            m2d[j] = t1[j] * a.f.inv_n;
            const double d = mc[j] - m2d[j];
            t1[j] = live ? M2c[j] + M * d * d : 0.0;
        }
        block_sum_d<GC>(t1, red);
        double al[GC], be[GC], mf[GC], rs2[GC], al2[GC], be2[GC], mf2[GC];
#pragma unroll
        for (int j = 0; j < GC; ++j) al2[j] = 1.0, be2[j] = 0.0, mf2[j] = 0.0;
#pragma unroll
        for (int j = 0; j < GC; ++j) {
            v2d[j] = t1[j] * a.inv_r;
            v2d[j] = v2d[j] > 0.0 ? v2d[j] : 0.0;
            rs2[j] = 1.0 / sqrt(v2d[j] + (double)a.bn.eps);
            const double alpha = (double)a.bn.weight[c0 + j] * rs2[j];
            const float af = (float)alpha, bf = (float)((double)a.bn.bias[c0 + j] - m2d[j] * alpha);
            al[j] = (double)af, be[j] = (double)bf;
            mf[j] = (double)(float)m2d[j];
        }
        if (threadIdx.x < GC) {
            const int j = threadIdx.x, c = c0 + j;
            const double mj = pick<GC>(m2d, j), vj = pick<GC>(v2d, j), mom = (double)a.bn.momentum;
            a.bn.run_mean[c] = (float)((1.0 - mom) * (double)a.bn.run_mean[c] + mom * mj);
            a.bn.run_var[c] = (float)((1.0 - mom) * (double)a.bn.run_var[c] + mom * vj * a.unbias_r);
            if (c == 0) bump_batches_tracked(a.bn.nbt);
            a.bn_stats[(size_t)BS_MEAN * g.C + c] = (float)pick<GC>(mf, j);
            a.bn_stats[(size_t)BS_RSTD * g.C + c] = (float)pick<GC>(rs2, j);
        }
        if (threadIdx.x == 0) {
            const CohBuf sb(a.bn_stats);
            sb.st4((size_t)BS_ALPHA * g.C + c0, (float)al[0], (float)al[1], (float)al[2], (float)al[3]);
            sb.st4((size_t)BS_BETA * g.C + c0, (float)be[0], (float)be[1], (float)be[2], (float)be[3]);
        }
        if constexpr (TWO) {
            double m2b[GC], v2b[GC], rsb[GC];
#pragma unroll
            for (int j = 0; j < GC; ++j) t1[j] = live ? mb[j] : 0.0;
            block_sum_d<GC>(t1, red);
#pragma unroll
            for (int j = 0; j < GC; ++j) {
                m2b[j] = t1[j] * a.f.inv_n;
                const double d = mb[j] - m2b[j];
                t1[j] = live ? M2b[j] + M * d * d : 0.0;
            }
            block_sum_d<GC>(t1, red);
#pragma unroll
            for (int j = 0; j < GC; ++j) {
                v2b[j] = t1[j] * a.inv_r;
                v2b[j] = v2b[j] > 0.0 ? v2b[j] : 0.0;
                rsb[j] = 1.0 / sqrt(v2b[j] + (double)a.bn2.eps);
                const double alpha = (double)a.bn2.weight[c0 + j] * rsb[j];
                const float af = (float)alpha, bf = (float)((double)a.bn2.bias[c0 + j] - m2b[j] * alpha);
                al2[j] = (double)af, be2[j] = (double)bf;
                mf2[j] = (double)(float)m2b[j];
            }
            float* st2 = a.bn_stats + (size_t)BS_ROWS * g.C;
            if (threadIdx.x < GC) {
                const int j = threadIdx.x, c = c0 + j;
                const double mj = pick<GC>(m2b, j), vj = pick<GC>(v2b, j), mom = (double)a.bn2.momentum;
                a.bn2.run_mean[c] = (float)((1.0 - mom) * (double)a.bn2.run_mean[c] + mom * mj);
                a.bn2.run_var[c] = (float)((1.0 - mom) * (double)a.bn2.run_var[c] + mom * vj * a.unbias_r);
                if (c == 0) bump_batches_tracked(a.bn2.nbt);
                st2[(size_t)BS_MEAN * g.C + c] = (float)pick<GC>(mf2, j);
                st2[(size_t)BS_RSTD * g.C + c] = (float)pick<GC>(rsb, j);
            }
            if (threadIdx.x == 0) {
                const CohBuf sb(st2);
                sb.st4((size_t)BS_ALPHA * g.C + c0, (float)al2[0], (float)al2[1], (float)al2[2], (float)al2[3]);
                sb.st4((size_t)BS_BETA * g.C + c0, (float)be2[0], (float)be2[1], (float)be2[2], (float)be2[3]);
            }
        }
        double mean[GC], sig[GC], z[GC], s1[GC], s2[GC];
#pragma unroll
        for (int j = 0; j < GC; ++j) {
            mean[j] = al[j] * mc[j] + be[j] + al2[j] * mb[j] + be2[j];
            const double m2 = al[j] * al[j] * M2c[j] + al2[j] * al2[j] * M2b[j] + 2.0 * al[j] * al2[j] * Ccb[j];
            sig[j] = sqrt((m2 > 0.0 ? m2 : 0.0) / (M - 1.0) + (double)a.f.eps_sn);
            z[j] = (double)gg.w[2 * (c0 + j)] * mean[j] + (double)gg.w[2 * (c0 + j) + 1] * sig[j];
            s1[j] = live ? z[j] : 0.0;
        }
        double mz[GC], rstd[GC];
        block_sum_d<GC>(s1, red);
#pragma unroll
        for (int j = 0; j < GC; ++j) {
            mz[j] = s1[j] * a.f.inv_n;
            const double d = z[j] - mz[j];
            s2[j] = live ? d * d : 0.0;
        }
        block_sum_d<GC>(s2, red);
#pragma unroll
        for (int j = 0; j < GC; ++j) rstd[j] = 1.0 / sqrt(s2[j] * a.f.inv_n + (double)a.f.eps_bn);
        if (threadIdx.x < GC) {
            const int j = threadIdx.x, c = c0 + j;
            const double vj = pick<GC>(s2, j) * a.f.inv_n, mj = pick<GC>(mz, j), mom = a.f.momentum;
            gg.run_mean[c] = (float)((1.0 - mom) * gg.run_mean[c] + mom * mj);
            gg.run_var[c] = (float)((1.0 - mom) * gg.run_var[c] + mom * vj * a.f.unbias_n);
            if (c == 0) bump_batches_tracked(gg.nbt);
            if (a.f.slim) bn_slim_rstd(a.f.slim, g.P)[c] = pick<GC>(rstd, j);
        }
        if (live) {
            float o_g[GC], o_zh[GC], o_hi[GC], o_lo[GC], o_sig[GC], o_e[GC], o_dm[GC], o_e2[GC], o_dm2[GC];
#pragma unroll
            for (int j = 0; j < GC; ++j) {
                const double zh = (z[j] - mz[j]) * rstd[j];
                o_g[j] = (float)sigmoid_d((double)gg.gamma[c0 + j] * zh + (double)gg.beta[c0 + j]);
                o_zh[j] = (float)zh;
                o_hi[j] = (float)mean[j];
                o_lo[j] = (float)(mean[j] - (double)o_hi[j]);
                o_sig[j] = (float)sig[j];
                o_e[j] = (float)(al[j] * M2c[j] + al2[j] * Ccb[j]);
                o_dm[j] = (float)(mc[j] - mf[j]);
                o_e2[j] = (float)(al2[j] * M2b[j] + al[j] * Ccb[j]);
                o_dm2[j] = (float)(mb[j] - mf2[j]);
            }
            CohBuf(a.f.gout).store<GC>(p0, o_g);
            if (a.f.slim) {
                store_group<GC>(a.f.slim + (size_t)SL_MU_HI * g.P + p0, o_hi);
                store_group<GC>(a.f.slim + (size_t)SL_MU_LO * g.P + p0, o_lo);
                store_group<GC>(a.f.slim + (size_t)SL_SIG * g.P + p0, o_sig);
                store_group<GC>(a.f.slim + (size_t)SL_ZH * g.P + p0, o_zh);
                store_group<GC>(a.f.slim + (size_t)SLB_E * g.P + p0, o_e);
                store_group<GC>(a.f.slim + (size_t)SLB_DM * g.P + p0, o_dm);
                if constexpr (TWO) {
                    store_group<GC>(a.f.slim + (size_t)SLB_E2 * g.P + p0, o_e2);
                    store_group<GC>(a.f.slim + (size_t)SLB_DM2 * g.P + p0, o_dm2);
                }
            }
        }
        __syncthreads();
    }
    if (!grid_barrier(a.f.bar, 2, &bar_flag)) {
        nhwc_mark_owed<T, VEC>(g, a.f.ntiles, y);
        return;
    }

    const int relu = a.f.relu;
    const int mine = a.f.ntiles > (int)blockIdx.x ? (a.f.ntiles - 1 - (int)blockIdx.x) / (int)gridDim.x : -1;
    for (int i = mine; i >= 0; --i) {
        const int tile = blockIdx.x + i * gridDim.x;
        const NhwcThread<VEC> t(g, tile);
        if (!t.active) continue;
        float gate[VEC], al[VEC], be[VEC], al2[TWO ? VEC : 1], be2[TWO ? VEC : 1];
        CohBuf(a.f.gout).load<VEC>(t.plane0(g), gate);
        const CohBuf sb(a.bn_stats);
        sb.load<VEC>((size_t)BS_ALPHA * g.C + (size_t)t.vc * VEC, al);
        sb.load<VEC>((size_t)BS_BETA * g.C + (size_t)t.vc * VEC, be);
        if constexpr (TWO) {
            sb.load<VEC>((size_t)(BS_ROWS + BS_ALPHA) * g.C + (size_t)t.vc * VEC, al2);
            sb.load<VEC>((size_t)(BS_ROWS + BS_BETA) * g.C + (size_t)t.vc * VEC, be2);
        }
        auto emit = [&](const Vec<T, VEC>& vc, const Vec<T, VEC>& vb, size_t e) {
            Vec<T, VEC> o;
#pragma unroll
            for (int j = 0; j < VEC; ++j) {
                const float b = bn_skip<T, TWO>(to_float(vb.v[j]), al2[TWO ? j : 0], be2[TWO ? j : 0]);
                const float X = bn_sum<T>(to_float(vc.v[j]), b, al[j], be[j]);
                const float v = gate[j] * X;
                o.v[j] = from_float<T>(relu ? fmaxf(v, 0.f) : v);
            }
            store_vec_nt<T, VEC>(y + e, o);
        };
        constexpr int U = 2;
        const int cnt = (t.p1 - t.p0 - t.r + g.rows - 1) / g.rows;
        int q = cnt - 1;
        for (; q - (U - 1) >= 0; q -= U) {
            Vec<T, VEC> vc[U], vb[U];
#pragma unroll
            for (int u = 0; u < U; ++u) {
                const size_t e = t.elem(g, t.p0 + t.r + (q - u) * g.rows);
                vc[u] = load_vec_nt<T, VEC>(cv + e);
                vb[u] = load_vec_nt<T, VEC>(idt + e);
            }
#pragma unroll
            for (int u = 0; u < U; ++u) emit(vc[u], vb[u], t.elem(g, t.p0 + t.r + (q - u) * g.rows));
        }
        for (; q >= 0; --q) {
            const size_t e = t.elem(g, t.p0 + t.r + q * g.rows);
            emit(load_vec_nt<T, VEC>(cv + e), load_vec_nt<T, VEC>(idt + e), e);
        }
    }
}

template <typename T, int VEC, bool KEEP, bool TWO>
__global__ __launch_bounds__(kBlock, TWO ? 2 : CNSN_BNHEAD_WG_PER_CU) void nhwc_bnhead_bwd_kernel(NhwcBnArgs a, const T* __restrict__ gy,
                                                                                         const T* __restrict__ cv,
                                                                                         const T* __restrict__ idt, T* __restrict__ dconv,
                                                                                         T* __restrict__ didt, GateDev gg, GateGradDev dg) {
    extern __shared__ float lds[];
    __shared__ double red[4 * 2 * kBnGc];
    __shared__ int bar_flag;
    constexpr int GC = kBnGc;
    const NhwcGeom& g = a.f.g;
    const float* __restrict__ row_mu = a.f.slim + (size_t)SL_MU_HI * g.P;
    const float* __restrict__ row_g = a.f.slim + (size_t)SL_G * g.P;
    const float* __restrict__ st_m = a.bn_stats + (size_t)BS_MEAN * g.C;
    const float* __restrict__ st_al = a.bn_stats + (size_t)BS_ALPHA * g.C;
    const float* __restrict__ st_be = a.bn_stats + (size_t)BS_BETA * g.C;
    const float* __restrict__ st2 = a.bn_stats + (size_t)BS_ROWS * g.C;
    const int relu = a.f.relu;

    for (int tile = blockIdx.x; tile < a.f.ntiles; tile += gridDim.x) {
        const NhwcThread<VEC> t(g, tile);
        float acc[3][VEC], acc4[1][VEC], mu[VEC], gate[VEC], al[VEC], be[VEC], mch[VEC], al2[TWO ? VEC : 1], be2[TWO ? VEC : 1],
            m2ch[TWO ? VEC : 1];
#pragma unroll
        for (int j = 0; j < VEC; ++j) acc[0][j] = acc[1][j] = acc[2][j] = acc4[0][j] = mu[j] = gate[j] = al[j] = be[j] = mch[j] = 0.f;
#pragma unroll
        for (int j = 0; j < (TWO ? VEC : 1); ++j) al2[j] = be2[j] = m2ch[j] = 0.f;
        if (t.active) {
            const size_t pl = t.plane0(g), ch = (size_t)t.vc * VEC;
            load_planes<VEC>(row_mu + pl, mu);
            load_planes<VEC>(row_g + pl, gate);
            load_planes<VEC>(st_al + ch, al);
            load_planes<VEC>(st_be + ch, be);
            load_planes<VEC>(st_m + ch, mch);
            if constexpr (TWO) {
                load_planes<VEC>(st2 + (size_t)BS_ALPHA * g.C + ch, al2);
                load_planes<VEC>(st2 + (size_t)BS_BETA * g.C + ch, be2);
                load_planes<VEC>(st2 + (size_t)BS_MEAN * g.C + ch, m2ch);
            }
            auto eat = [&](const Vec<T, VEC>& vg, const Vec<T, VEC>& vc, const Vec<T, VEC>& vb) {
#pragma unroll
                for (int j = 0; j < VEC; ++j) {
                    const float c = to_float(vc.v[j]), c2 = to_float(vb.v[j]);
                    const float X = bn_sum<T>(c, bn_skip<T, TWO>(c2, al2[TWO ? j : 0], be2[TWO ? j : 0]), al[j], be[j]);
                    float G = to_float(vg.v[j]);
                    if (relu) G = relu_open<T>(gate[j] * X) ? G : 0.f;
                    acc[0][j] += G;
                    acc[1][j] = fmaf(G, X - mu[j], acc[1][j]);
                    acc[2][j] = fmaf(G, c - mch[j], acc[2][j]);
                    if constexpr (TWO) acc4[0][j] = fmaf(G, c2 - m2ch[j], acc4[0][j]);
                }
            };
            int p = t.p0 + t.r;
            for (; p + g.rows < t.p1; p += 2 * g.rows) {
                Vec<T, VEC> vg[2], vc[2], vb[2];
#pragma unroll
                for (int u = 0; u < 2; ++u) {
                    const size_t e = t.elem(g, p + u * g.rows);
                    vg[u] = nhwc_ld<T, VEC, !KEEP>(gy + e);
                    vc[u] = nhwc_ld<T, VEC, !KEEP>(cv + e);
                    vb[u] = nhwc_ld<T, VEC, !KEEP>(idt + e);
                }
#pragma unroll
                for (int u = 0; u < 2; ++u) eat(vg[u], vc[u], vb[u]);
            }
            for (; p < t.p1; p += g.rows) {
                const size_t e = t.elem(g, p);
                eat(nhwc_ld<T, VEC, !KEEP>(gy + e), nhwc_ld<T, VEC, !KEEP>(cv + e), nhwc_ld<T, VEC, !KEEP>(idt + e));
            }
        }
        nhwc_rows_sum_part<VEC, 3, kBnBwd>(g, t, acc, 0, lds, a.f.part);
        if constexpr (TWO) nhwc_rows_sum_part<VEC, 1, kBnBwd>(g, t, acc4, 3, lds, a.f.part);
    }
    if (!grid_barrier(a.f.bar, 1, &bar_flag)) {
        nhwc_mark_owed<T, VEC>(g, a.f.ntiles, dconv);
        return;
    }

    for (int slot = blockIdx.x; slot < a.f.ngroups; slot += gridDim.x) {
        const int grp = phase_b_group(slot, a.f.ngroups);
        const int c0 = grp * GC, n = threadIdx.x;
        const bool live = n < g.N;
        const size_t p0 = (size_t)(live ? n : 0) * g.C + c0;
        double S1[GC], S2[GC], S3[GC], S4[GC], mu[GC], lo[GC], gate[GC], zh[GC], sig[GC], E[GC], DM[GC], E2[GC], DM2[GC];
#pragma unroll
        for (int j = 0; j < GC; ++j) S1[j] = S2[j] = S3[j] = S4[j] = E2[j] = DM2[j] = 0.0;
        const CohBuf pb(a.f.part);
        for (int s = 0; s < g.S; ++s) {
            const size_t base = (size_t)s * kBnBwd * g.P + p0;
            add_group_coh<GC>(pb, base, S1);
            add_group_coh<GC>(pb, base + g.P, S2);
            add_group_coh<GC>(pb, base + 2 * g.P, S3);
            if constexpr (TWO) add_group_coh<GC>(pb, base + 3 * g.P, S4);
        }
        load_group<GC>(a.f.slim + (size_t)SL_MU_HI * g.P + p0, mu);
        load_group<GC>(a.f.slim + (size_t)SL_MU_LO * g.P + p0, lo);
        load_group<GC>(a.f.slim + (size_t)SL_G * g.P + p0, gate);
        load_group<GC>(a.f.slim + (size_t)SL_ZH * g.P + p0, zh);
        load_group<GC>(a.f.slim + (size_t)SL_SIG * g.P + p0, sig);
        load_group<GC>(a.f.slim + (size_t)SLB_E * g.P + p0, E);
        load_group<GC>(a.f.slim + (size_t)SLB_DM * g.P + p0, DM);
        if constexpr (TWO) {
            load_group<GC>(a.f.slim + (size_t)SLB_E2 * g.P + p0, E2);
            load_group<GC>(a.f.slim + (size_t)SLB_DM2 * g.P + p0, DM2);
        }
        double dt[GC], acc[2 * GC];
#pragma unroll
        for (int j = 0; j < GC; ++j) {
            const double s2c = S2[j] - lo[j] * S1[j];
            const double mex = mu[j] + lo[j];
            dt[j] = (s2c + mex * S1[j]) * gate[j] * (1.0 - gate[j]);
            acc[j] = live ? dt[j] : 0.0;
            acc[GC + j] = live ? dt[j] * zh[j] : 0.0;
        }
        block_sum_d<2 * GC>(acc, red);
        if (threadIdx.x < GC) {
            double sd = 0.0, sdz = 0.0;
#pragma unroll
            for (int q = 0; q < GC; ++q)
                if (q == (int)threadIdx.x) sd = acc[q], sdz = acc[GC + q];
            dg.dgamma[c0 + threadIdx.x] = (float)sdz;
            dg.dbeta[c0 + threadIdx.x] = (float)sd;
        }
        const double M = (double)g.M;
        double dz[GC], cx[GC], cz[GC];
        float o_cx[GC], o_c0[GC];
#pragma unroll
        for (int j = 0; j < GC; ++j) {
            const double kg = (double)gg.gamma[c0 + j] * bn_slim_rstd(a.f.slim, g.P)[c0 + j];
            dz[j] = kg * (dt[j] - acc[j] * a.f.inv_n - zh[j] * acc[GC + j] * a.f.inv_n);
            const double dmu = dz[j] * (double)gg.w[2 * (c0 + j)], dsig = dz[j] * (double)gg.w[2 * (c0 + j) + 1];
            cx[j] = dsig / (sig[j] * (M - 1.0));
            cz[j] = dmu / M - cx[j] * lo[j];
            o_cx[j] = (float)cx[j];
            o_c0[j] = (float)cz[j];
        }
#pragma unroll
        for (int j = 0; j < GC; ++j) {
            acc[j] = live ? dz[j] * (mu[j] + lo[j]) : 0.0;
            acc[GC + j] = live ? dz[j] * sig[j] : 0.0;
        }
        block_sum_d<2 * GC>(acc, red);
        if (threadIdx.x < GC) {
            double w0 = 0.0, w1 = 0.0;
#pragma unroll
            for (int q = 0; q < GC; ++q)
                if (q == (int)threadIdx.x) w0 = acc[q], w1 = acc[GC + q];
            dg.dw[2 * (c0 + threadIdx.x)] = (float)w0;
            dg.dw[2 * (c0 + threadIdx.x) + 1] = (float)w1;
        }
#pragma unroll
        for (int j = 0; j < GC; ++j) {
            const double fx = (double)o_cx[j], f0 = (double)o_c0[j];
            acc[j] = live ? gate[j] * S1[j] + fx * M * lo[j] + f0 * M : 0.0;
            acc[GC + j] = live ? gate[j] * S3[j] + fx * (E[j] + lo[j] * M * DM[j]) + f0 * M * DM[j] : 0.0;
        }
        block_sum_d<2 * GC>(acc, red);
        if (threadIdx.x < GC) {
            const int c = c0 + threadIdx.x;
            double D1 = 0.0, D2 = 0.0;
#pragma unroll
            for (int q = 0; q < GC; ++q)
                if (q == (int)threadIdx.x) D1 = acc[q], D2 = acc[GC + q];
            const double rs = (double)a.bn_stats[(size_t)BS_RSTD * g.C + c], al = (double)a.bn_stats[(size_t)BS_ALPHA * g.C + c];
            a.dbn_b[c] = (float)D1;
            a.dbn_w[c] = (float)(rs * D2);
            const float e0 = (float)(-al * D1 * a.inv_r), e1 = (float)(-al * rs * rs * D2 * a.inv_r);
            __hip_atomic_store(a.chan + c, e0, __ATOMIC_RELAXED, __HIP_MEMORY_SCOPE_AGENT);
            __hip_atomic_store(a.chan + g.C + c, e1, __ATOMIC_RELAXED, __HIP_MEMORY_SCOPE_AGENT);
        }
        if constexpr (TWO) {
            double a2[GC];
#pragma unroll
            for (int j = 0; j < GC; ++j) {
                const double fx = (double)o_cx[j], f0 = (double)o_c0[j];
                a2[j] = live ? gate[j] * S4[j] + fx * (E2[j] + lo[j] * M * DM2[j]) + f0 * M * DM2[j] : 0.0;
            }
            double D1k = 0.0;
            if (threadIdx.x < GC) {
#pragma unroll
                for (int q = 0; q < GC; ++q)
                    if (q == (int)threadIdx.x) D1k = acc[q];
            }
            block_sum_d<GC>(a2, red);
            if (threadIdx.x < GC) {
                const int c = c0 + threadIdx.x;
                const double D2b = pick<GC>(a2, (int)threadIdx.x);
                const float* s2 = a.bn_stats + (size_t)BS_ROWS * g.C;
                const double rs = (double)s2[(size_t)BS_RSTD * g.C + c], al = (double)s2[(size_t)BS_ALPHA * g.C + c];
                a.dbn2_b[c] = (float)D1k;
                a.dbn2_w[c] = (float)(rs * D2b);
                const float e0 = (float)(-al * D1k * a.inv_r), e1 = (float)(-al * rs * rs * D2b * a.inv_r);
                __hip_atomic_store(a.chan + 2 * (size_t)g.C + c, e0, __ATOMIC_RELAXED, __HIP_MEMORY_SCOPE_AGENT);
                __hip_atomic_store(a.chan + 3 * (size_t)g.C + c, e1, __ATOMIC_RELAXED, __HIP_MEMORY_SCOPE_AGENT);
            }
        }
        if (live) {
            const CohBuf cb(a.f.coefb);
            cb.store<GC>(p0, o_cx);
            cb.store<GC>(g.P + p0, o_c0);
        }
        __syncthreads();
    }
    if (!grid_barrier(a.f.bar, 2, &bar_flag)) {
        nhwc_mark_owed<T, VEC>(g, a.f.ntiles, dconv);
        return;
    }

    const int mine = a.f.ntiles > (int)blockIdx.x ? (a.f.ntiles - 1 - (int)blockIdx.x) / (int)gridDim.x : -1;
    for (int i = mine; i >= 0; --i) {
        const int tile = blockIdx.x + i * gridDim.x;
        const NhwcThread<VEC> t(g, tile);
        if (!t.active) continue;
        const size_t pl = t.plane0(g), ch = (size_t)t.vc * VEC;
        float cG[VEC], cX[VEC], xr[VEC], c0[VEC], al[VEC], be[VEC], mch[VEC], e0[VEC], e1[VEC];
        float al2[TWO ? VEC : 1], be2[TWO ? VEC : 1], m2ch[TWO ? VEC : 1], e0b[TWO ? VEC : 1], e1b[TWO ? VEC : 1];
        load_planes<VEC>(row_g + pl, cG);
        load_planes<VEC>(row_mu + pl, xr);
        const CohBuf cb(a.f.coefb), eb(a.chan);
        cb.load<VEC>(pl, cX);
        cb.load<VEC>(g.P + pl, c0);
        load_planes<VEC>(st_al + ch, al);
        load_planes<VEC>(st_be + ch, be);
        load_planes<VEC>(st_m + ch, mch);
        eb.load<VEC>(ch, e0);
        eb.load<VEC>((size_t)g.C + ch, e1);
        if constexpr (TWO) {
            load_planes<VEC>(st2 + (size_t)BS_ALPHA * g.C + ch, al2);
            load_planes<VEC>(st2 + (size_t)BS_BETA * g.C + ch, be2);
            load_planes<VEC>(st2 + (size_t)BS_MEAN * g.C + ch, m2ch);
            eb.load<VEC>(2 * (size_t)g.C + ch, e0b);
            eb.load<VEC>(3 * (size_t)g.C + ch, e1b);
        }
        auto emit = [&](const Vec<T, VEC>& vg, const Vec<T, VEC>& vc, const Vec<T, VEC>& vb, size_t e) {
            Vec<T, VEC> o, od;
#pragma unroll
            for (int j = 0; j < VEC; ++j) {
                const float c = to_float(vc.v[j]), c2 = to_float(vb.v[j]);
                const float X = bn_sum<T>(c, bn_skip<T, TWO>(c2, al2[TWO ? j : 0], be2[TWO ? j : 0]), al[j], be[j]);
                float G = to_float(vg.v[j]);
                if (relu) G = relu_open<T>(cG[j] * X) ? G : 0.f;
                const float dX = fmaf(cG[j], G, fmaf(cX[j], X - xr[j], c0[j]));
                if constexpr (TWO)
                    od.v[j] = from_float<T>(fmaf(al2[j], dX, fmaf(e1b[j], c2 - m2ch[j], e0b[j])));
                else
                    od.v[j] = from_float<T>(dX);
                o.v[j] = from_float<T>(fmaf(al[j], dX, fmaf(e1[j], c - mch[j], e0[j])));
            }
            store_vec_nt<T, VEC>(dconv + e, o);
            store_vec_nt<T, VEC>(didt + e, od);
        };
        const int cnt = (t.p1 - t.p0 - t.r + g.rows - 1) / g.rows;
        for (int q = cnt - 1; q >= 0; --q) {
            const size_t e = t.elem(g, t.p0 + t.r + q * g.rows);
            emit(load_vec_nt<T, VEC>(gy + e), load_vec_nt<T, VEC>(cv + e), load_vec_nt<T, VEC>(idt + e), e);
        }
    }
}

}
```

### crossnorm-selfnorm_amd/csrc/cnsn_nhwc_fused.hip

```cpp
#include "cnsn_nhwc.h"

#include "cnsn_nhwc_fused_host.h"

namespace cnsn {

using namespace nhwc_host;

namespace {
struct FusedWs { float *part, *side; void* bar; size_t bytes; };
FusedWs fused_layout(const NhwcGeom& g, void* workspace) {
    Carver c(workspace);
    return {c.take((size_t)g.S * 2 * g.P * 4), c.take(4 * g.P * 4), c.take<void>(kBarBlock), c.bytes()};
}
struct BnHeadWs { float *part, *side, *chan; void* bar; size_t bytes; };
BnHeadWs bnhead_layout(const NhwcGeom& g, void* workspace) {
    Carver c(workspace);
    return {c.take((size_t)g.S * kBnFwd * g.P * 4), c.take(4 * g.P * 4), c.take(4 * (size_t)g.C * 4), c.take<void>(kBarBlock), c.bytes()};
}
}

NhwcGeom nhwc_fused_geom(const Plan& pl) {
    const cnsn_problem_t& p = pl.pr;
    NhwcGeom g;
    g.N = p.N;
    g.C = p.C;
    g.M = p.H * p.W;
    g.tc = p.C / vec_of(p.dtype);
    const long target = 2l * CNSN_NHWC_WG_PER_CU * reshost::cu_count();
    g.tcb = g.tc < kBlock ? g.tc : kBlock;
    while (g.tcb > 64 && g.tcb % 2 == 0 && (long)g.N * ((g.tc + g.tcb - 1) / g.tcb) < target) g.tcb /= 2;
    g.rows = kBlock / g.tcb;
    g.ncb = (g.tc + g.tcb - 1) / g.tcb;
    const long per_chunk = (long)g.N * g.ncb;
    int S = (int)((target + per_chunk - 1) / per_chunk);
    const int s_max = g.M / (8 * g.rows) > 0 ? g.M / (8 * g.rows) : 1;
    if (S > s_max) S = s_max;
    if (S < 1) S = 1;
    g.mchunk = (g.M + S - 1) / S;
    g.S = (g.M + g.mchunk - 1) / g.mchunk;
    g.P = pl.P;
    return g;
}

bool nhwc_slim_record(const Plan& pl) {
    const cnsn_problem_t& p = pl.pr;
    return p.layout == CNSN_LAYOUT_NHWC && !p.cn_active && p.sn_active && !p.sn_two;
}

bool nhwc_fused_ok(const Plan& pl, bool check_health) {
    const cnsn_problem_t& p = pl.pr;
    if (!nhwc_slim_record(pl) || !nhwc_supported(pl, false)) return false;
    if (p.strategy == CNSN_STRATEGY_TWO_PASS || p.strategy == CNSN_STRATEGY_LOCAL || p.strategy == CNSN_STRATEGY_MONO) return false;
    if (check_health && resident_degraded()) return false;
    const int mode = fused_mode();
    if (mode == 0) return false;
    if (p.N > kBlock || p.C % CNSN_NHWC_GC != 0 || p.H * p.W < 2) return false;
    if (check_health && p.strategy == CNSN_STRATEGY_AUTO && !resident_auto_enabled()) return false;
    if (mode > 2 && p.strategy == CNSN_STRATEGY_AUTO && tensor_bytes(pl) > ((size_t)mode << 20)) return false;
    const NhwcGeom g = nhwc_fused_geom(pl);
    return (long)g.N * g.S * g.ncb >= 8;
}

size_t nhwc_fused_extra_bytes(const Plan& pl) { return fused_layout(nhwc_fused_geom(pl), nullptr).bytes; }

int nhwc_fused_forward(Plan& pl, int add, int relu, const void* x, const void* addend, GateDev gg, void* y, float* saved,
                       void* workspace, size_t workspace_bytes, hipStream_t stream, void* sum_out) {
    if (!nhwc_fused_ok(pl)) return CNSN_E_UNSUPPORTED;
    if (add != ADD_NONE && !addend) return CNSN_E_NULL;
    const NhwcGeom ng = nhwc_fused_geom(pl);
    const FusedWs w = fused_layout(ng, workspace);
    if (workspace_bytes < w.bytes) return CNSN_E_WORKSPACE;
    NhwcFusedArgs a = make_args(pl, ng, relu, CNSN_NHWC_GC);
    a.part = w.part;
    a.kshift = w.side;
    a.slim = saved;
    a.sum_out = add == ADD_PRE ? sum_out : nullptr;
    a.gout = saved ? saved + (size_t)SL_G * pl.P : a.kshift + pl.P;
    a.keep = keep_first_read(add == ADD_PRE ? 2 : 1, tensor_bytes(pl));
    int status = CNSN_E_UNSUPPORTED;
    dispatch_t(pl.pr.dtype, [&](auto tt, auto vt) {
        using T = typename decltype(tt)::type;
        constexpr int VEC = decltype(vt)::value;
        const size_t lds = (size_t)2 * ng.rows * ng.tcb * VEC * 4;
        auto go = [&](auto kern) {
            status = launch_fused(pl, kern, lds, a, a, w.bar, stream, (const T*)x, (const T*)addend, (T*)y, gg);
        };
        if (a.sum_out)
            return go(nhwc_fused_fwd_kernel<T, VEC, ADD_PRE, false, true>);
        with_add(add, [&](auto at) {
            constexpr int ADD = decltype(at)::value;
            a.keep ? go(nhwc_fused_fwd_kernel<T, VEC, ADD, true>) : go(nhwc_fused_fwd_kernel<T, VEC, ADD, false>);
        });
    });
    if (knob(K_DEBUG))
        fprintf(stderr, "[cnsn] nhwc single-launch fwd: tiles=%d (S=%d rows=%d tcb=%d) groups=%d keep=%d -> status %d\n", a.ntiles,
                ng.S, ng.rows, ng.tcb, a.ngroups, a.keep, status);
    return status;
}

int nhwc_fused_backward(Plan& pl, int add, int relu, const void* gy, const void* x, const void* addend, GateDev gg,
                        const float* saved, void* dx, void* d_addend, GateGradDev dg, void* workspace, size_t workspace_bytes,
                        hipStream_t stream) {
    if (!nhwc_fused_ok(pl)) return CNSN_E_UNSUPPORTED;
    if (!saved) return CNSN_E_NULL;
    if (add == ADD_POST && relu && !d_addend) return CNSN_E_NULL;
    const NhwcGeom ng = nhwc_fused_geom(pl);
    const FusedWs w = fused_layout(ng, workspace);
    if (workspace_bytes < w.bytes) return CNSN_E_WORKSPACE;
    const int eff_add = (relu || add == ADD_PRE) ? add : ADD_NONE;
    if (eff_add != ADD_NONE && !addend) return CNSN_E_NULL;
    NhwcFusedArgs a = make_args(pl, ng, relu, CNSN_NHWC_GC_BWD);
    a.keep = keep_first_read(eff_add != ADD_NONE ? 3 : 2, tensor_bytes(pl));
    a.part = w.part;
    a.coefb = w.side;
    a.slim = const_cast<float*>(saved);
    int status = CNSN_E_UNSUPPORTED;
    dispatch_t(pl.pr.dtype, [&](auto tt, auto vt) {
        using T = typename decltype(tt)::type;
        constexpr int VEC = decltype(vt)::value;
        const size_t lds = (size_t)2 * ng.rows * ng.tcb * VEC * 4;
        auto go = [&](auto kern) {
            status = launch_fused(pl, kern, lds, a, a, w.bar, stream, (const T*)gy, (const T*)x, (const T*)addend, (T*)dx, (T*)d_addend, gg,
                                  dg);
        };
        with_add(eff_add, [&](auto at) {
            constexpr int ADD = decltype(at)::value;
            a.keep ? go(nhwc_fused_bwd_kernel<T, VEC, ADD, true>) : go(nhwc_fused_bwd_kernel<T, VEC, ADD, false>);
        });
    });
    if (knob(K_DEBUG))
        fprintf(stderr, "[cnsn] nhwc single-launch bwd: tiles=%d (S=%d rows=%d tcb=%d) groups=%d keep=%d -> status %d\n", a.ntiles,
                ng.S, ng.rows, ng.tcb, a.ngroups, a.keep, status);
    return status;
}

void nhwc_slim_from_saved(const Plan& pl, const double* saved_d, float* slim, hipStream_t stream) {
    const int blocks = (int)((pl.P + kBlock - 1) / kBlock);
    nhwc_slim_from_saved_kernel<<<blocks, kBlock, 0, stream>>>(saved_d, pl.pr.N, pl.pr.C, slim);
}

void nhwc_saved_from_slim(const Plan& pl, const float* slim, int relu, double* saved_d, float* rows, hipStream_t stream) {
    const int blocks = (int)((pl.P + kBlock - 1) / kBlock);
    nhwc_saved_from_slim_kernel<<<blocks, kBlock, 0, stream>>>(slim, pl.pr.N, pl.pr.C, relu, saved_d, rows);
}

bool nhwc_bnhead_ok(const Plan& pl, bool check_health) {
    const cnsn_problem_t& p = pl.pr;
    if (!nhwc_fused_ok(pl, check_health) || !p.sn_training || p.N < 2 || p.C % kBnGc != 0) return false;
    const NhwcGeom g = nhwc_fused_geom(pl);
    if ((long)g.N * g.S * g.ncb < 8) return false;
    return (size_t)g.S * kBnFwd * g.P * 4 < ((size_t)1 << 31);
}

namespace {
NhwcBnArgs make_bn_args(const Plan& pl, const NhwcGeom& ng, int relu, const cnsn_bn_tail_t& bn, const cnsn_bn_tail_t* bn2, float* bn_stats,
                        const BnHeadWs& w) {
    NhwcBnArgs a{};
    a.f = make_args(pl, ng, relu, kBnGc);
    a.bn = bn_head_dev(bn);
    if (bn2) a.bn2 = bn_head_dev(*bn2);
    set_bn_count(a, (double)ng.N * (double)ng.M);
    a.bn_stats = bn_stats;
    a.f.part = w.part;
    a.f.kshift = w.side;
    a.kshift_b = w.side + pl.P;
    a.f.gout = w.side + 2 * pl.P;
    a.f.coefb = w.side + 2 * pl.P;
    a.chan = w.chan;
    return a;
}
}

size_t nhwc_bnhead_extra_bytes(const Plan& pl) { return bnhead_layout(nhwc_fused_geom(pl), nullptr).bytes; }

int nhwc_bnhead_forward(Plan& pl, int relu, const cnsn_bn_tail_t& bn, const cnsn_bn_tail_t* bn2, const void* conv_out, const void* identity,
                        GateDev gg, void* y, float* saved, float* bn_stats, void* workspace, size_t workspace_bytes, hipStream_t stream) {
    if (!nhwc_bnhead_ok(pl) || !bn.training || (bn2 && !bn2->training)) return CNSN_E_UNSUPPORTED;
    const NhwcGeom ng = nhwc_fused_geom(pl);
    const BnHeadWs w = bnhead_layout(ng, workspace);
    if (workspace_bytes < w.bytes) return CNSN_E_WORKSPACE;
    NhwcBnArgs a = make_bn_args(pl, ng, relu, bn, bn2, bn_stats, w);
    a.f.slim = saved;
    if (saved) a.f.gout = saved + (size_t)SL_G * pl.P;
    a.f.keep = keep_first_read(2, tensor_bytes(pl));
    int status = CNSN_E_UNSUPPORTED;
    dispatch_t(pl.pr.dtype, [&](auto tt, auto vt) {
        using T = typename decltype(tt)::type;
        constexpr int VEC = decltype(vt)::value;
        const size_t lds = (size_t)3 * ng.rows * ng.tcb * VEC * 4;
        auto go = [&](auto kern) {
            status = launch_fused(pl, kern, lds, a, a.f, w.bar, stream, (const T*)conv_out, (const T*)identity, (T*)y, gg);
        };
        if (bn2)
            a.f.keep ? go(nhwc_bnhead_fwd_kernel<T, VEC, true, true>) : go(nhwc_bnhead_fwd_kernel<T, VEC, false, true>);
        else
            a.f.keep ? go(nhwc_bnhead_fwd_kernel<T, VEC, true, false>) : go(nhwc_bnhead_fwd_kernel<T, VEC, false, false>);
    });
    if (knob(K_DEBUG))
        fprintf(stderr, "[cnsn] nhwc bn-block fwd: tiles=%d (S=%d rows=%d tcb=%d) groups=%d keep=%d -> status %d\n", a.f.ntiles, ng.S,
                ng.rows, ng.tcb, a.f.ngroups, a.f.keep, status);
    return status;
}

int nhwc_bnhead_backward(Plan& pl, int relu, const cnsn_bn_tail_t& bn, const cnsn_bn_tail_t* bn2, const void* gy, const void* conv_out,
                         const void* identity, GateDev gg, const float* saved, const float* bn_stats, void* d_conv, void* d_identity,
                         GateGradDev dg, float* dbn_w, float* dbn_b, float* dbn2_w, float* dbn2_b, void* workspace,
                         size_t workspace_bytes, hipStream_t stream) {
    if (!nhwc_bnhead_ok(pl, false) || !bn.training || (bn2 && !bn2->training)) return CNSN_E_UNSUPPORTED;
    if (!saved || !bn_stats || !d_conv || !d_identity || !dbn_w || !dbn_b || (bn2 && (!dbn2_w || !dbn2_b))) return CNSN_E_NULL;
    const NhwcGeom ng = nhwc_fused_geom(pl);
    const BnHeadWs w = bnhead_layout(ng, workspace);
    if (workspace_bytes < w.bytes) return CNSN_E_WORKSPACE;
    NhwcBnArgs a = make_bn_args(pl, ng, relu, bn, bn2, const_cast<float*>(bn_stats), w);
    a.f.slim = const_cast<float*>(saved);
    a.dbn_w = dbn_w;
    a.dbn_b = dbn_b;
    a.dbn2_w = dbn2_w;
    a.dbn2_b = dbn2_b;
    a.f.keep = keep_first_read(3, tensor_bytes(pl));
    int status = CNSN_E_UNSUPPORTED;
    dispatch_t(pl.pr.dtype, [&](auto tt, auto vt) {
        using T = typename decltype(tt)::type;
        constexpr int VEC = decltype(vt)::value;
        const size_t lds = (size_t)3 * ng.rows * ng.tcb * VEC * 4;
        auto go = [&](auto kern) {
            status = launch_fused(pl, kern, lds, a, a.f, w.bar, stream, (const T*)gy, (const T*)conv_out, (const T*)identity,
                                  (T*)d_conv, (T*)d_identity, gg, dg);
        };
        if (bn2)
            a.f.keep ? go(nhwc_bnhead_bwd_kernel<T, VEC, true, true>) : go(nhwc_bnhead_bwd_kernel<T, VEC, false, true>);
        else
            a.f.keep ? go(nhwc_bnhead_bwd_kernel<T, VEC, true, false>) : go(nhwc_bnhead_bwd_kernel<T, VEC, false, false>);
    });
    if (knob(K_DEBUG))
        fprintf(stderr, "[cnsn] nhwc bn-block bwd: tiles=%d (S=%d rows=%d tcb=%d) groups=%d keep=%d -> status %d\n", a.f.ntiles, ng.S,
                ng.rows, ng.tcb, a.f.ngroups, a.f.keep, status);
    return status;
}

}
```

### crossnorm-selfnorm_amd/functional.py

```python
from __future__ import annotations

import ctypes as C
import dataclasses
import os
import threading
from dataclasses import dataclass
from typing import Optional, Sequence, Tuple

import torch

from . import _ffi

Box = Tuple[int, int, int, int]

_DTYPES = {torch.float32: _ffi.CNSN_F32, torch.bfloat16: _ffi.CNSN_BF16, torch.float16: _ffi.CNSN_F16}

_strategy = _ffi.STRATEGY_AUTO


def set_strategy(name: str):
    global _strategy
    _strategy = {"auto": _ffi.STRATEGY_AUTO, "two_pass": _ffi.STRATEGY_TWO_PASS,
                 "resident": _ffi.STRATEGY_RESIDENT, "local": _ffi.STRATEGY_LOCAL, "mono": _ffi.STRATEGY_MONO}[name]
    _ffi.forget_plans()


def set_resident(enabled: bool):
    global _resident_set
    _ffi.lib().cnsn_resident_enable(int(bool(enabled)))
    _resident_set = bool(enabled)
    _ffi.forget_plans()


_resident_set = None


def resident_allowed() -> bool:
    return _resident_set if _resident_set is not None else os.environ.get("CNSN_RESIDENT", "1") != "0"


def _require_device(x: torch.Tensor, what: str):
    if not isinstance(x, torch.Tensor):
        raise TypeError(f"{what}: expected a tensor")
    if not x.is_cuda:
        raise _ffi.CnsnError(
            f"{what}: got a {x.device.type} tensor. This implementation runs on MI355X HIP device "
            "tensors only; there is no CPU path.")
    if x.dtype not in _DTYPES:
        raise TypeError(f"{what}: dtype {x.dtype} not supported (float32, bfloat16, float16)")
    assert x.dim() == 4, "expected an (N, C, H, W) tensor"


def _dense(t: torch.Tensor) -> torch.Tensor:
    t = t.contiguous()
    if t.data_ptr() % 16:
        t = t.clone(memory_format=torch.contiguous_format)
    return t


NHWC = None


def _nhwc_call(x: torch.Tensor, cfg, chan_perm) -> bool:
    global NHWC
    if NHWC is None:
        NHWC = os.environ.get("CNSN_NHWC") != "0"
    if not NHWC or x.dim() != 4 or chan_perm is not None or cfg.content_box is not None or cfg.style_box is not None:
        return False
    if x.is_contiguous() or not x.is_contiguous(memory_format=torch.channels_last):
        return False
    vec = 16 // x.element_size()
    return x.shape[1] % vec == 0 and x.shape[2] * x.shape[3] >= 2 and x.data_ptr() % 16 == 0


def _dense_cl(t: torch.Tensor) -> torch.Tensor:
    t = t.contiguous(memory_format=torch.channels_last)
    if t.data_ptr() % 16:
        t = t.clone(memory_format=torch.channels_last)
    return t


def _on_device_of(fn):
    import functools

    @functools.wraps(fn)
    def wrapped(ctx, first, *rest):
        if not (isinstance(first, torch.Tensor) and first.is_cuda):
            return fn(ctx, first, *rest)
        with torch.cuda.device(first.device):
            return fn(ctx, first, *rest)
    return wrapped


def _out_like(x: torch.Tensor) -> torch.Tensor:
    g = _ffi.glue()
    return g.out_like(x) if g is not None else torch.empty_like(x)


def _stream(x):
    return C.c_void_p(torch._C._cuda_getCurrentRawStream(x.device.index))


def _ptr(t: Optional[torch.Tensor]):
    return C.c_void_p(t.data_ptr()) if t is not None else None


def _f32(t: torch.Tensor) -> torch.Tensor:
    if t.dtype == torch.float32 and t.is_contiguous():
        return t.detach() if t.requires_grad else t
    return t.detach().to(torch.float32).contiguous()


def _addend_like(x, addend, what, dense, name="addend"):
    _require_device(addend, f"{what}({name})")
    assert addend.shape == x.shape and addend.dtype == x.dtype, f"{name} must match the first input"
    return dense(addend)


def _cl_inputs(x, addend, what):
    x = _dense_cl(x)
    return x, (None if addend is None else _addend_like(x, addend, what, _dense_cl))


def _workspace(nbytes: int, dev) -> torch.Tensor:
    return torch.empty(nbytes // 4 + 4, dtype=torch.float32, device=dev)


def _grad_like(gy, x, cl: bool):
    gy = gy if gy.dtype == x.dtype else gy.to(x.dtype)
    return _dense_cl(gy) if cl else _dense(gy)


def _cast_grads(tensors, dtypes):
    return [None if d is None else (t if t.dtype == d else t.to(d)) for t, d in zip(tensors, dtypes)]


def _gate_grad_views(c: int, dev, extra: int = 0):
    flat = torch.empty((4 + extra) * c, dtype=torch.float32, device=dev)
    rows = [flat[:2 * c].view(c, 1, 2), *flat[2 * c:].view(2 + extra, c).unbind(0)]
    return rows, _ffi.GateGrad(_ptr(rows[0]), _ptr(rows[1]), _ptr(rows[2]))


def _plan_cache() -> dict:
    cache = {}
    _ffi._plan_caches.append(cache)
    return cache


def _remembered(cache: dict, key, ask) -> bool:
    hit = cache.get(key)
    if hit is None:
        hit = cache[key] = bool(ask())
    return hit


def _single_launch_tensor(x, poll: bool = True) -> bool:
    if not x.is_cuda or x.dim() != 4 or x.dtype not in _DTYPES:
        return False
    if not x.is_contiguous(memory_format=torch.channels_last) or x.is_contiguous():
        return False
    return not (poll and _ffi.lib().cnsn_resident_degraded())


_lock = threading.RLock()

_size_cache = _plan_cache()


def _sizes(prob):
    key = (prob.dtype, prob.N, prob.C, prob.H, prob.W, prob.cn_active, prob.sn_active, prob.sn_two,
           prob.sn_training, prob.content_box[0] >= 0, prob.style_box[0] >= 0, prob.strategy, prob.layout)
    hit = _size_cache.get(key)
    if hit is None:
        lib = _ffi.lib()
        hit = (lib.cnsn_saved_floats(C.byref(prob)), lib.cnsn_workspace_bytes(C.byref(prob)),
               lib.cnsn_context_bytes(C.byref(prob)))
        if hit[1] > 0:
            _size_cache[key] = hit
    return hit


_contexts = {}
_retired_contexts = []


def _context(prob, dev: torch.device):
    need = _sizes(prob)[2]
    if need == 0 or torch.cuda.is_current_stream_capturing():
        return
    have = _contexts.get(dev.index)
    if have is None or have.numel() < need:
        with _lock:
            have = _grow_context(need, dev)
    prob.context = have.data_ptr()
    prob.context_bytes = have.numel()


def _grow_context(need, dev):
    have = _contexts.get(dev.index)
    if have is None or have.numel() < need:
        size = max(need, 2 * have.numel() if have is not None else (4 << 20))
        buf = torch.empty(size, dtype=torch.uint8, device=dev)
        stream = torch.cuda.current_stream(dev)
        _ffi.check(_ffi.lib().cnsn_context_init(C.c_void_p(buf.data_ptr()), size, C.c_void_p(stream.cuda_stream)),
                   "cnsn_context_init")
        stream.synchronize()
        if have is not None:
            _retired_contexts.append(have)
        _contexts[dev.index] = have = buf
    return have


def _nhwc_context(x):
    prob = _problem(x, FusedConfig(sn_active=True))
    prob.layout = _ffi.LAYOUT_NHWC
    _context(prob, x.device)
    return prob.context, prob.context_bytes


class _PinnedRing:
    SLOTS = 8

    def __init__(self):
        self.rings = {}

    def to_device(self, idx: torch.Tensor, dev: torch.device) -> torch.Tensor:
        if idx.is_cuda:
            return idx.to(device=dev, dtype=torch.int64).contiguous()
        n = idx.numel()
        with _lock:
            ring = self.rings.setdefault((dev.index, n), {"next": 0, "slots": [None] * self.SLOTS})
            k = ring["next"] % self.SLOTS
            ring["next"] += 1
        if ring["slots"][k] is None:
            ring["slots"][k] = (torch.empty(n, dtype=torch.int64).pin_memory(), torch.cuda.Event())
        else:
            ring["slots"][k][1].synchronize()
        buf, evt = ring["slots"][k]
        buf.copy_(idx.reshape(-1))
        out = buf.to(dev, non_blocking=True)
        evt.record(torch.cuda.current_stream(dev))
        return out


_h2d = _PinnedRing()


@dataclass
class GateParams:
    fc_weight: torch.Tensor
    bn_weight: torch.Tensor
    bn_bias: torch.Tensor
    running_mean: torch.Tensor
    running_var: torch.Tensor
    num_batches_tracked: Optional[torch.Tensor] = None


@dataclass
class FusedConfig:
    cn_active: bool = False
    content_box: Optional[Box] = None
    style_box: Optional[Box] = None
    lam: Optional[float] = None
    sn_active: bool = False
    sn_two: bool = False
    sn_training: bool = True
    eps_cn: float = 1e-5
    eps_sn: float = 1e-12
    eps_bn: float = 1e-5
    momentum: float = 0.1
    add_mode: str = "none"
    relu: bool = False

    @property
    def has_epilogue(self):
        return self.add_mode != "none" or self.relu


_ADD_MODES = {"none": _ffi.ADD_NONE, "pre": _ffi.ADD_PRE, "post": _ffi.ADD_POST}


def _epilogue(cfg: FusedConfig, addend, sum_out=None):
    e = _ffi.Epilogue()
    e.struct_bytes = C.sizeof(_ffi.Epilogue)
    e.add_mode = _ADD_MODES[cfg.add_mode]
    e.relu = int(cfg.relu)
    e.addend = addend.data_ptr() if addend is not None else None
    e.sum_out = sum_out.data_ptr() if sum_out is not None else None
    return e


_KEEP_SUM = os.environ.get("CNSN_KEEP_SUM", "1") != "0"


def which_path(x: torch.Tensor, cfg: FusedConfig, backward: bool = False, chan_perm: bool = False) -> str:
    prob = _problem(x, cfg)
    if _nhwc_call(x, cfg, True if chan_perm else None):
        prob.layout = _ffi.LAYOUT_NHWC
    epi = _epilogue(cfg, None) if cfg.has_epilogue else None
    st = _ffi.lib().cnsn_which_path(C.byref(prob), C.byref(epi) if epi else None, int(chan_perm), int(backward))
    if st < 0:
        _ffi.check(st, "cnsn_which_path")
    return _ffi.PATHS[st]


_perm_inline_cache = _plan_cache()
LEGACY_LAUNCHES = os.environ.get("CNSN_LEGACY_LAUNCHES") == "1"


def perm_inline_ok(x: torch.Tensor, cfg: FusedConfig, perm, chan_perm) -> bool:
    if LEGACY_LAUNCHES or chan_perm is not None or not isinstance(perm, torch.Tensor) or perm.is_cuda or perm.dtype != torch.int64 \
            or not perm.is_contiguous() or perm.numel() > _ffi.PERM_INLINE_MAX or perm.numel() != x.shape[0]:
        return False
    key = (tuple(x.shape), x.dtype, x.device.index, cfg.sn_active, cfg.sn_two, cfg.sn_training, cfg.content_box is not None,
           cfg.style_box is not None, cfg.add_mode, cfg.relu, _strategy)
    return _remembered(_perm_inline_cache, key,
                       lambda: which_path(x, cfg, False) == "resident" and which_path(x, cfg, True) == "resident")


def sn_cluster(x: torch.Tensor, cfg: FusedConfig, backward: bool = False) -> bool:
    prob = _problem(x, cfg)
    epi = _epilogue(cfg, None) if cfg.has_epilogue else None
    st = _ffi.lib().cnsn_sn_cluster_plan(C.byref(prob), C.byref(epi) if epi else None, int(backward))
    if st < 0:
        _ffi.check(st, "cnsn_sn_cluster_plan")
    return st == 1


def _problem(x: torch.Tensor, cfg: FusedConfig) -> _ffi.Problem:
    p = _ffi.Problem()
    p.struct_bytes = C.sizeof(_ffi.Problem)
    p.dtype = _DTYPES[x.dtype]
    p.N, p.C, p.H, p.W = (int(s) for s in x.shape)
    p.cn_active = int(cfg.cn_active)
    p.content_box = _ffi.box4(cfg.content_box)
    p.style_box = _ffi.box4(cfg.style_box)
    p.lam = 0.0 if cfg.lam is None else float(cfg.lam)
    p.eps_cn = cfg.eps_cn
    p.sn_active = int(cfg.sn_active)
    p.sn_two = int(cfg.sn_two)
    p.sn_training = int(cfg.sn_training)
    p.eps_sn, p.eps_bn, p.momentum = cfg.eps_sn, cfg.eps_bn, cfg.momentum
    p.strategy = _strategy
    return p


class _RunningBuffers:

    def _take_running(self, rm, rv, nbt, training=True):
        self.src_rm, self.src_rv, self.training = rm, rv, bool(training)
        self.direct = rm.dtype == torch.float32 and rm.is_contiguous() and rv.dtype == torch.float32 and rv.is_contiguous()
        self.rm = rm.detach() if self.direct else _f32(rm)
        self.rv = rv.detach() if self.direct else _f32(rv)
        if nbt is not None and not (training and nbt.dtype == torch.int64 and nbt.is_cuda and nbt.numel() == 1):
            if training:
                nbt.add_(1)
            nbt = None
        self.nbt = nbt

    def write_back(self):
        if self.training and not self.direct:
            self.src_rm.copy_(self.rm)
            self.src_rv.copy_(self.rv)


class _GateBuffers(_RunningBuffers):

    def __init__(self, w, gamma, beta, rm, rv, nbt=None):
        self.w, self.gamma, self.beta = _f32(w), _f32(gamma), _f32(beta)
        self._take_running(rm, rv, nbt)
        self.c = _ffi.Gate(_ptr(self.w), _ptr(self.gamma), _ptr(self.beta), _ptr(self.rm), _ptr(self.rv), _ptr(self.nbt))


class _Bn2dBuffers(_RunningBuffers):

    def __init__(self, w, b, rm, rv, eps, momentum, nbt, training=True):
        self.w, self.b = _f32(w), _f32(b)
        self.eps, self.momentum = float(eps), float(momentum)
        self._take_running(rm, rv, nbt, training)
        self.c = self.struct(self.nbt)

    def struct(self, nbt=None):
        return _ffi.BnTail(C.sizeof(_ffi.BnTail), int(self.training), self.eps, self.momentum, self.w.data_ptr(), self.b.data_ptr(),
                           self.rm.data_ptr(), self.rv.data_ptr(), _ptr(nbt))


class FusedCNSN(torch.autograd.Function):

    @staticmethod
    def forward(ctx, x, cfg: FusedConfig, perm, chan_perm, g_w, g_gamma, g_beta, g_rm, g_rv,
                f_w, f_gamma, f_beta, f_rm, f_rv, addend=None, g_nbt=None, f_nbt=None):
        _require_device(x, "cnsn_forward")
        with torch.cuda.device(x.device):
            return FusedCNSN._forward(ctx, x, cfg, perm, chan_perm, g_w, g_gamma, g_beta, g_rm, g_rv,
                                      f_w, f_gamma, f_beta, f_rm, f_rv, addend, g_nbt, f_nbt)

    @staticmethod
    def _forward(ctx, x, cfg, perm, chan_perm, g_w, g_gamma, g_beta, g_rm, g_rv,
                 f_w, f_gamma, f_beta, f_rm, f_rv, addend, g_nbt, f_nbt):
        lib = _ffi.lib()
        _ffi.check_resident_health("cnsn_forward")
        nhwc = _nhwc_call(x, cfg, chan_perm if cfg.cn_active else None)
        x = x if nhwc else _dense(x)
        addend = _addend_like(x, addend, "cnsn_forward", _dense_cl if nhwc else _dense) if cfg.add_mode != "none" else None
        prob = _problem(x, cfg)
        prob.layout = _ffi.LAYOUT_NHWC if nhwc else _ffi.LAYOUT_NCHW
        dev = x.device
        _context(prob, dev)
        perm_host = None
        if cfg.cn_active:
            if not nhwc and perm_inline_ok(x, cfg, perm, chan_perm):
                perm_host, perm = (perm.clone() if any(ctx.needs_input_grad) else perm), None
                prob.perm_host = perm_host.data_ptr()
            else:
                perm = _h2d.to_device(perm, dev)
                if chan_perm is not None:
                    chan_perm = _h2d.to_device(chan_perm, dev)
        gate_g = _GateBuffers(g_w, g_gamma, g_beta, g_rm, g_rv, g_nbt if cfg.sn_training else None) if cfg.sn_active else None
        gate_f = _GateBuffers(f_w, f_gamma, f_beta, f_rm, f_rv, f_nbt if cfg.sn_training else None) \
            if (cfg.sn_active and cfg.sn_two) else None
        y = _out_like(x)
        need_bwd = any(ctx.needs_input_grad)
        saved_floats, ws_bytes = _sizes(prob)[:2]
        saved = torch.empty(saved_floats, dtype=torch.float32, device=dev) if need_bwd else None
        ws = _workspace(ws_bytes, dev)
        epi = _epilogue(cfg, addend) if cfg.has_epilogue else None
        xsum = None
        if need_bwd and nhwc and cfg.add_mode == "pre" and _KEEP_SUM and lib.cnsn_keeps_sum(C.byref(prob), C.byref(epi)) == 1:
            xsum = _out_like(x)
            epi.sum_out = xsum.data_ptr()

        def launch():
            return lib.cnsn_forward_fused(C.byref(prob), C.byref(epi) if epi else None, _ptr(x),
                                          _ptr(perm if cfg.cn_active else None),
                                          _ptr(chan_perm if cfg.cn_active else None),
                                          C.byref(gate_g.c) if gate_g else None, C.byref(gate_f.c) if gate_f else None,
                                          _ptr(y), _ptr(saved), _ptr(ws), ws_bytes, _stream(x))

        st = launch()
        if st == _ffi.E_UNSUPPORTED and perm_host is not None:
            perm, perm_host = _h2d.to_device(perm_host, dev), None
            prob.perm_host = None
            st = launch()
        _ffi.check(st, "cnsn_forward")
        if cfg.sn_active and cfg.sn_training:
            gate_g.write_back()
            if gate_f:
                gate_f.write_back()
        if need_bwd:
            ctx.cfg, ctx.prob = cfg, prob
            ctx.gates = (gate_g, gate_f)
            ctx.param_dtypes = tuple(t.dtype if t is not None else None
                                     for t in (g_w, g_gamma, g_beta, f_w, f_gamma, f_beta))
            ctx.perm_host = perm_host
            ctx.kept_sum = xsum is not None
            if xsum is not None:
                ctx.cfg = dataclasses.replace(cfg, add_mode="none")
                ctx.save_for_backward(xsum, saved, perm if cfg.cn_active else None,
                                      chan_perm if cfg.cn_active else None, None)
            else:
                ctx.save_for_backward(x, saved, perm if cfg.cn_active else None,
                                      chan_perm if cfg.cn_active else None, addend)
        return y

    @staticmethod
    @_on_device_of
    def backward(ctx, gy):
        lib = _ffi.lib()
        x, saved, perm, chan_perm, addend = ctx.saved_tensors
        cfg, prob = ctx.cfg, ctx.prob
        gate_g, gate_f = ctx.gates
        gy = _grad_like(gy, x, prob.layout == _ffi.LAYOUT_NHWC)
        dev = x.device
        dx = _out_like(x)
        ws_bytes = _sizes(prob)[1]
        _context(prob, dev)
        if torch.cuda.is_current_stream_capturing():
            prob.context, prob.context_bytes = None, 0
        ws = _workspace(ws_bytes, dev)
        gg = gf = None
        gg_c = gf_c = None
        if cfg.sn_active:
            gg, gg_c = _gate_grad_views(x.shape[1], dev)
            if cfg.sn_two:
                gf, gf_c = _gate_grad_views(x.shape[1], dev)
        epi = _epilogue(cfg, addend) if cfg.has_epilogue else None
        d_add = None
        if cfg.add_mode == "post":
            d_add = _out_like(x) if cfg.relu else gy
        perm_host = ctx.perm_host
        prob.perm_host = perm_host.data_ptr() if perm_host is not None else None

        def launch(perm_dev):
            return lib.cnsn_backward_fused(C.byref(prob), C.byref(epi) if epi else None, _ptr(gy), _ptr(x), _ptr(perm_dev),
                                           _ptr(chan_perm), C.byref(gate_g.c) if gate_g else None,
                                           C.byref(gate_f.c) if gate_f else None, _ptr(saved), _ptr(dx),
                                           _ptr(d_add) if (cfg.add_mode == "post" and cfg.relu) else None,
                                           C.byref(gg_c) if gg_c else None, C.byref(gf_c) if gf_c else None,
                                           _ptr(ws), ws_bytes, _stream(x))

        st = launch(perm)
        if st == _ffi.E_UNSUPPORTED and perm_host is not None:
            prob.perm_host = None
            st = launch(_h2d.to_device(perm_host, dev))
        _ffi.check(st, "cnsn_backward")
        if cfg.add_mode == "pre" or ctx.kept_sum:
            d_add = dx
        pd = ctx.param_dtypes
        out_g = [None] * 3 if gg is None else _cast_grads(gg, pd[:3])
        out_f = [None] * 3 if gf is None else _cast_grads(gf, pd[3:])
        return (dx, None, None, None, *out_g, None, None, *out_f, None, None, d_add, None, None)


def bnrelu_plan(x: torch.Tensor, cfg: FusedConfig, backward: bool = False) -> bool:
    prob = _problem(x, cfg)
    epi = _epilogue(cfg, None) if cfg.has_epilogue else None
    st = _ffi.lib().cnsn_bnrelu_plan(C.byref(prob), C.byref(epi) if epi else None, int(backward))
    if st < 0:
        _ffi.check(st, "cnsn_bnrelu_plan")
    return st == 1


class FusedCNSNTail(torch.autograd.Function):

    @staticmethod
    def forward(ctx, x, cfg: FusedConfig, addend, want_y, g_w, g_gamma, g_beta, g_rm, g_rv, bn_w, bn_b, bn_rm, bn_rv,
                bn_training, bn_eps, bn_momentum, g_nbt=None, bn_nbt=None):
        _require_device(x, "cnsn_forward_bnrelu")
        with torch.cuda.device(x.device):
            lib = _ffi.lib()
            _ffi.check_resident_health("cnsn_forward_bnrelu")
            x = _dense(x)
            addend = _addend_like(x, addend, "cnsn_forward_bnrelu", _dense) if cfg.add_mode != "none" else None
            prob = _problem(x, cfg)
            dev = x.device
            gate = _GateBuffers(g_w, g_gamma, g_beta, g_rm, g_rv, g_nbt if cfg.sn_training else None)
            bn = _Bn2dBuffers(bn_w, bn_b, bn_rm, bn_rv, bn_eps, bn_momentum, bn_nbt, bn_training)
            y = _out_like(x) if want_y else None
            z = _out_like(x)
            need_bwd = any(ctx.needs_input_grad)
            saved_floats, ws_bytes = _sizes(prob)[:2]
            saved = torch.empty(saved_floats, dtype=torch.float32, device=dev) if need_bwd else None
            stats = torch.empty(2 * x.shape[1], dtype=torch.float32, device=dev)
            ws = _workspace(ws_bytes, dev)
            epi = _epilogue(cfg, addend) if cfg.has_epilogue else None
            st = lib.cnsn_forward_bnrelu(C.byref(prob), C.byref(epi) if epi else None, C.byref(bn.c), _ptr(x),
                                         C.byref(gate.c), _ptr(y), _ptr(z), _ptr(saved), _ptr(stats), _ptr(ws), ws_bytes,
                                         _stream(x))
            _ffi.check(st, "cnsn_forward_bnrelu")
            if cfg.sn_training:
                gate.write_back()
            bn.write_back()
            ctx.set_materialize_grads(False)
            if need_bwd:
                ctx.cfg, ctx.prob, ctx.gate, ctx.bn, ctx.want_y = cfg, prob, gate, bn, want_y
                ctx.param_dtypes = (g_w.dtype, g_gamma.dtype, g_beta.dtype, bn_w.dtype, bn_b.dtype)
                ctx.save_for_backward(x, saved, addend, stats)
            return (y, z) if want_y else z

    @staticmethod
    def backward(ctx, *grads):
        gy, gz = grads if ctx.want_y else (None, grads[0])
        x, saved, addend, stats = ctx.saved_tensors
        with torch.cuda.device(x.device):
            lib = _ffi.lib()
            cfg, prob, gate = ctx.cfg, ctx.prob, ctx.gate
            dev = x.device
            gz = _grad_like(gz if gz is not None else torch.zeros_like(x), x, False)
            if gy is not None:
                gy = _grad_like(gy, x, False)
            tail = ctx.bn.struct()
            dx = _out_like(x)
            grads, gg = _gate_grad_views(x.shape[1], dev, 2)
            dbw, dbb = grads[3:]
            ws_bytes = _sizes(prob)[1]
            ws = _workspace(ws_bytes, dev)
            epi = _epilogue(cfg, addend) if cfg.has_epilogue else None
            st = lib.cnsn_backward_bnrelu(C.byref(prob), C.byref(epi) if epi else None, C.byref(tail), _ptr(gy), _ptr(gz),
                                          _ptr(x), C.byref(gate.c), _ptr(saved), _ptr(stats), _ptr(dx), C.byref(gg),
                                          _ptr(dbw), _ptr(dbb), _ptr(ws), ws_bytes, _stream(x))
            _ffi.check(st, "cnsn_backward_bnrelu")
            outs = _cast_grads(grads, ctx.param_dtypes)
            d_add = dx if cfg.add_mode == "pre" else None
            return (dx, None, d_add, None, outs[0], outs[1], outs[2], None, None, outs[3], outs[4], None, None, None, None, None,
                    None, None)


_bn_block_plan_cache = _plan_cache()
_BN_BLOCK = os.environ.get("CNSN_BN_BLOCK", "1") != "0"


def bn_block_plan(x: torch.Tensor, cfg: FusedConfig) -> bool:
    if not _BN_BLOCK or cfg.cn_active or not cfg.sn_training or not _single_launch_tensor(x):
        return False

    def ask():
        prob = _problem(x, cfg)
        prob.layout = _ffi.LAYOUT_NHWC
        return _ffi.lib().cnsn_bn_block_plan(C.byref(prob), C.byref(_epilogue(cfg, None))) == 1
    return _remembered(_bn_block_plan_cache, (tuple(x.shape), x.dtype, x.device.index, cfg.relu, cfg.sn_two, _strategy), ask)


class FusedBnBlock(torch.autograd.Function):

    @staticmethod
    def forward(ctx, conv_out, identity, cfg: FusedConfig, g_w, g_gamma, g_beta, g_rm, g_rv, bn_w, bn_b, bn_rm, bn_rv, bn_eps,
                bn_momentum, g_nbt=None, bn_nbt=None, bn2_w=None, bn2_b=None, bn2_rm=None, bn2_rv=None, bn2_eps=0.0,
                bn2_momentum=0.0, bn2_nbt=None):
        _require_device(conv_out, "cnsn_forward_bn_block")
        with torch.cuda.device(conv_out.device):
            lib = _ffi.lib()
            _ffi.check_resident_health("cnsn_forward_bn_block")
            x = _dense_cl(conv_out)
            idt = _addend_like(x, identity, "cnsn_forward_bn_block", _dense_cl, "identity")
            prob = _problem(x, cfg)
            prob.layout = _ffi.LAYOUT_NHWC
            dev = x.device
            _context(prob, dev)
            gate = _GateBuffers(g_w, g_gamma, g_beta, g_rm, g_rv, g_nbt)
            head = _Bn2dBuffers(bn_w, bn_b, bn_rm, bn_rv, bn_eps, bn_momentum, bn_nbt)
            skip = _Bn2dBuffers(bn2_w, bn2_b, bn2_rm, bn2_rv, bn2_eps, bn2_momentum, bn2_nbt) if bn2_w is not None else None
            y = _out_like(x)
            need_bwd = any(ctx.needs_input_grad)
            saved_floats, ws_bytes = _sizes(prob)[:2]
            saved = torch.empty(saved_floats, dtype=torch.float32, device=dev) if need_bwd else None
            stats = torch.empty((8 if skip else 4) * x.shape[1], dtype=torch.float32, device=dev)
            ws = _workspace(ws_bytes, dev)
            epi = _epilogue(cfg, idt)
            st = lib.cnsn_forward_bn_block(C.byref(prob), C.byref(epi), C.byref(head.c), C.byref(skip.c) if skip else None, _ptr(x),
                                           C.byref(gate.c), _ptr(y), _ptr(saved), _ptr(stats), _ptr(ws), ws_bytes, _stream(x))
            _ffi.check(st, "cnsn_forward_bn_block")
            gate.write_back()
            head.write_back()
            if skip:
                skip.write_back()
            if need_bwd:
                ctx.cfg, ctx.prob, ctx.gate, ctx.head, ctx.skip = cfg, prob, gate, head, skip
                ctx.param_dtypes = (g_w.dtype, g_gamma.dtype, g_beta.dtype, bn_w.dtype, bn_b.dtype,
                                    bn2_w.dtype if skip else None, bn2_b.dtype if skip else None)
                ctx.save_for_backward(x, idt, saved, stats)
            return y

    @staticmethod
    def backward(ctx, gy):
        x, idt, saved, stats = ctx.saved_tensors
        with torch.cuda.device(x.device):
            lib = _ffi.lib()
            cfg, prob, gate, head, skip = ctx.cfg, ctx.prob, ctx.gate, ctx.head, ctx.skip
            dev = x.device
            gy = _grad_like(gy, x, True)
            hs = head.struct()
            ss = skip.struct() if skip else None
            d_conv, d_idt = _out_like(x), _out_like(x)
            grads, gg = _gate_grad_views(x.shape[1], dev, 4)
            dbw, dbb, d2w, d2b = grads[3:]
            ws_bytes = _sizes(prob)[1]
            _context(prob, dev)
            if torch.cuda.is_current_stream_capturing():
                prob.context, prob.context_bytes = None, 0
            ws = _workspace(ws_bytes, dev)
            epi = _epilogue(cfg, idt)
            st = lib.cnsn_backward_bn_block(C.byref(prob), C.byref(epi), C.byref(hs), C.byref(ss) if ss else None, _ptr(gy), _ptr(x),
                                            C.byref(gate.c), _ptr(saved), _ptr(stats), _ptr(d_conv), _ptr(d_idt), C.byref(gg),
                                            _ptr(dbw), _ptr(dbb), _ptr(d2w) if skip else None, _ptr(d2b) if skip else None, _ptr(ws),
                                            ws_bytes, _stream(x))
            _ffi.check(st, "cnsn_backward_bn_block")
            outs = _cast_grads(grads, ctx.param_dtypes)
            return (d_conv, d_idt, None, outs[0], outs[1], outs[2], None, None, outs[3], outs[4], None, None, None, None, None, None,
                    outs[5], outs[6], None, None, None, None, None)


def _glue_cfg(cfg: FusedConfig, need_bwd: bool, inline: bool = False):
    cb = cfg.content_box if cfg.content_box is not None else (-1, -1, -1, -1)
    sb = cfg.style_box if cfg.style_box is not None else (-1, -1, -1, -1)
    icfg = [int(cfg.cn_active), *(int(v) for v in cb), *(int(v) for v in sb), int(cfg.sn_active), int(cfg.sn_two),
            int(cfg.sn_training), _strategy, int(need_bwd), _ADD_MODES[cfg.add_mode], int(cfg.relu), int(inline)]
    fcfg = [0.0 if cfg.lam is None else float(cfg.lam), cfg.eps_cn, cfg.eps_sn, cfg.eps_bn, cfg.momentum]
    return icfg, fcfg


_tail_plan_cache = _plan_cache()


def fused_cnsn_tail(x, cfg: FusedConfig, addend, want_y: bool, g: GateParams, bn_w, bn_b, bn_rm, bn_rv, bn_training: bool,
                    bn_eps: float, bn_momentum: float, bn_nbt=None):
    glue = _ffi.glue()
    if glue is None:
        out = FusedCNSNTail.apply(x, cfg, addend, bool(want_y), g.fc_weight, g.bn_weight, g.bn_bias, g.running_mean,
                                  g.running_var, bn_w, bn_b, bn_rm, bn_rv, bn_training, bn_eps, bn_momentum,
                                  g.num_batches_tracked, bn_nbt)
        return out if want_y else (None, out)
    _require_device(x, "cnsn_forward_bnrelu")
    _ffi.check_resident_health("cnsn_forward_bnrelu")
    need_bwd = torch.is_grad_enabled() and (x.requires_grad or any(
        t is not None and t.requires_grad for t in (g.fc_weight, g.bn_weight, g.bn_bias, bn_w, bn_b, addend)))
    icfg, fcfg = _glue_cfg(cfg, need_bwd)
    out = glue.fused_cnsn_tail(x, icfg, fcfg, g.fc_weight, g.bn_weight, g.bn_bias, g.running_mean, g.running_var,
                               addend if cfg.add_mode != "none" else None, bn_w, bn_b, bn_rm, bn_rv,
                               [int(want_y), int(bn_training)], [float(bn_eps), float(bn_momentum)],
                               g.num_batches_tracked if cfg.sn_training else None, bn_nbt if bn_training else None)
    return (out[0], out[1]) if want_y else (None, out[0])


def bnrelu_plan_cached(x: torch.Tensor, cfg: FusedConfig, need_bwd: bool) -> bool:
    key = (tuple(x.shape), x.dtype, x.device.index, cfg.add_mode, cfg.sn_training, cfg.sn_two, _strategy, need_bwd)
    return _remembered(_tail_plan_cache, key, lambda: bnrelu_plan(x, cfg) and (not need_bwd or bnrelu_plan(x, cfg, backward=True)))


def fused_cnsn(x, cfg: FusedConfig, perm=None, chan_perm=None, g: Optional[GateParams] = None,
               f: Optional[GateParams] = None, addend: Optional[torch.Tensor] = None):
    ga = (g.fc_weight, g.bn_weight, g.bn_bias, g.running_mean, g.running_var) if g else (None,) * 5
    fa = (f.fc_weight, f.bn_weight, f.bn_bias, f.running_mean, f.running_var) if f else (None,) * 5
    g_nbt = g.num_batches_tracked if (g and cfg.sn_training) else None
    f_nbt = f.num_batches_tracked if (f and cfg.sn_training) else None
    glue = _ffi.glue()
    if glue is None:
        return FusedCNSN.apply(x, cfg, perm, chan_perm, *ga, *fa, addend, g_nbt, f_nbt)
    _require_device(x, "cnsn_forward")
    _ffi.check_resident_health("cnsn_forward")
    if cfg.add_mode == "none":
        addend = None
    need_bwd = torch.is_grad_enabled() and (x.requires_grad or any(
        t is not None and t.requires_grad for t in (*ga[:3], *fa[:3], addend)))
    icfg, fcfg = _glue_cfg(cfg, need_bwd, cfg.cn_active and perm_inline_ok(x, cfg, perm, chan_perm))
    return glue.fused_cnsn(x, icfg, fcfg, perm if cfg.cn_active else None, chan_perm if cfg.cn_active else None,
                           *ga, *fa, addend, g_nbt, f_nbt)


def _dims(x):
    return tuple(int(s) for s in x.shape)


class PlaneStats(torch.autograd.Function):

    @staticmethod
    @_on_device_of
    def forward(ctx, x, eps, box, keep_fp32=False):
        _require_device(x, "calc_ins_mean_std")
        lib = _ffi.lib()
        x = _dense(x)
        n, c, h, w = _dims(x)
        ms = torch.empty(2, n * c, dtype=torch.float32, device=x.device)
        st = lib.cnsn_plane_stats(_ptr(x), _DTYPES[x.dtype], n, c, h, w, _ffi.box4(box) if box else None,
                                  float(eps), _ptr(ms), _stream(x))
        _ffi.check(st, "cnsn_plane_stats")
        ctx.box = box
        ctx.save_for_backward(x, ms)
        out_dtype = torch.float32 if keep_fp32 else x.dtype
        mean = ms[0].view(n, c, 1, 1).to(out_dtype)
        std = ms[1].view(n, c, 1, 1).to(out_dtype)
        return mean, std

    @staticmethod
    @_on_device_of
    def backward(ctx, gmean, gstd):
        lib = _ffi.lib()
        x, ms = ctx.saved_tensors
        n, c, h, w = _dims(x)
        gm = _f32(gmean).view(-1)
        gs = _f32(gstd).view(-1)
        dx = _out_like(x)
        st = lib.cnsn_plane_stats_backward(_ptr(x), _DTYPES[x.dtype], n, c, h, w,
                                           _ffi.box4(ctx.box) if ctx.box else None, _ptr(ms[0]), _ptr(ms[1]),
                                           _ptr(gm), _ptr(gs), _ptr(dx), _stream(x))
        _ffi.check(st, "cnsn_plane_stats_backward")
        return dx, None, None, None


class PlaneAffine(torch.autograd.Function):

    @staticmethod
    @_on_device_of
    def forward(ctx, x, scale, shift):
        _require_device(x, "plane_affine")
        lib = _ffi.lib()
        x = _dense(x)
        n, c, h, w = _dims(x)
        sc, sh = _f32(scale).view(-1), _f32(shift).view(-1)
        y = _out_like(x)
        st = lib.cnsn_plane_affine(_ptr(x), _DTYPES[x.dtype], n, c, h, w, _ptr(sc), _ptr(sh), _ptr(y), _stream(x))
        _ffi.check(st, "cnsn_plane_affine")
        ctx.save_for_backward(x, sc)
        ctx.meta = (scale.shape, scale.dtype, shift.shape, shift.dtype)
        return y

    @staticmethod
    @_on_device_of
    def backward(ctx, gy):
        lib = _ffi.lib()
        x, sc = ctx.saved_tensors
        n, c, h, w = _dims(x)
        gy = _dense(gy.to(x.dtype))
        dt = _DTYPES[x.dtype]
        dx = dscale = dshift = None
        if ctx.needs_input_grad[0]:
            dx = _out_like(x)
            zero = torch.zeros_like(sc)
            st = lib.cnsn_plane_affine(_ptr(gy), dt, n, c, h, w, _ptr(sc), _ptr(zero), _ptr(dx), _stream(x))
            _ffi.check(st, "cnsn_plane_affine(backward)")
        if ctx.needs_input_grad[1] or ctx.needs_input_grad[2]:
            sums = torch.empty(2, n * c, dtype=torch.float32, device=x.device)
            st = lib.cnsn_plane_dot(_ptr(gy), _ptr(x), dt, n, c, h, w, _ptr(sums), _stream(x))
            _ffi.check(st, "cnsn_plane_dot")
            s_shape, s_dtype, t_shape, t_dtype = ctx.meta
            dscale = sums[1].view(s_shape).to(s_dtype)
            dshift = sums[0].view(t_shape).to(t_dtype)
        return dx, dscale, dshift


class InstanceNorm(torch.autograd.Function):

    @staticmethod
    @_on_device_of
    def forward(ctx, x, weight, bias, eps):
        _require_device(x, "instance_norm")
        lib = _ffi.lib()
        x = _dense(x)
        n, c, h, w = _dims(x)
        m = h * w
        assert m > 1, "InstanceNorm2d needs more than one value per plane"
        dt = _DTYPES[x.dtype]
        ms = torch.empty(2, n * c, dtype=torch.float32, device=x.device)
        st = lib.cnsn_plane_stats(_ptr(x), dt, n, c, h, w, None, float(eps) * m / (m - 1.0), _ptr(ms), _stream(x))
        _ffi.check(st, "cnsn_plane_stats")
        mean = ms[0].view(n, c)
        rstd = 1.0 / (ms[1].view(n, c) * ((m - 1.0) / m) ** 0.5)
        wf = weight.detach().float().view(1, c) if weight is not None else None
        scale = rstd * wf if wf is not None else rstd
        shift = -mean * scale
        if bias is not None:
            shift = shift + bias.detach().float().view(1, c)
        scale, shift = scale.contiguous().view(-1), shift.contiguous().view(-1)
        y = _out_like(x)
        st = lib.cnsn_plane_affine(_ptr(x), dt, n, c, h, w, _ptr(scale), _ptr(shift), _ptr(y), _stream(x))
        _ffi.check(st, "cnsn_plane_affine")
        ctx.save_for_backward(x, mean, rstd, weight)
        ctx.has_bias = bias is not None
        return y

    @staticmethod
    @_on_device_of
    def backward(ctx, gy):
        lib = _ffi.lib()
        x, mean, rstd, weight = ctx.saved_tensors
        n, c, h, w = _dims(x)
        m = float(h * w)
        dt = _DTYPES[x.dtype]
        gy = _dense(gy.to(x.dtype))
        mean64 = mean.double().contiguous().view(-1)
        sums = torch.empty(2, n * c, dtype=torch.float32, device=x.device)
        st = lib.cnsn_plane_dot_shifted(_ptr(gy), _ptr(x), dt, n, c, h, w, _ptr(mean64), _ptr(sums), _stream(x))
        _ffi.check(st, "cnsn_plane_dot_shifted")
        s1 = sums[0].view(n, c).double()
        sgx = sums[1].view(n, c).double() * rstd.double()
        wd = weight.detach().double().view(1, c) if weight is not None else torch.ones(1, c, dtype=torch.float64, device=x.device)
        rw = rstd.double() * wd
        coef = torch.stack([rw, -rw * rstd.double() * sgx / m, mean.double(), -rw * s1 / m]).float().contiguous()
        dx = _out_like(x)
        st = lib.cnsn_plane_combine(_ptr(gy), _ptr(x), dt, n, c, h, w, _ptr(coef), _ptr(dx), _stream(x))
        _ffi.check(st, "cnsn_plane_combine")
        dweight = dbias = None
        if weight is not None and ctx.needs_input_grad[1]:
            dweight = sgx.sum(0).to(weight.dtype)
        if ctx.has_bias and ctx.needs_input_grad[2]:
            dbias = s1.sum(0).to(weight.dtype if weight is not None else torch.float32)
        return dx, dweight, dbias, None


_ibn_plan_cache = _plan_cache()


def _ibn_desc(x: torch.Tensor, half: int, relu: bool, eps_in: float, in_w=None, in_b=None, bn: Optional[_ffi.BnTail] = None):
    n, c, h, w = _dims(x)
    d = _ffi.Ibn()
    d.struct_bytes = C.sizeof(_ffi.Ibn)
    d.dtype, d.N, d.C, d.H, d.W = _DTYPES[x.dtype], n, c, h, w
    d.half, d.relu, d.eps_in = int(half), int(bool(relu)), float(eps_in)
    d.in_weight, d.in_bias = (in_w.data_ptr() if in_w is not None else None), (in_b.data_ptr() if in_b is not None else None)
    if bn is not None:
        d.bn = bn
    elif half < c:
        d.bn.struct_bytes = C.sizeof(_ffi.BnTail)
    return d


def ibn_plan(x: torch.Tensor, half: int, relu: bool = True, has_addend: bool = False, bn_training: bool = True) -> bool:
    if not _single_launch_tensor(x) or torch.cuda.is_current_stream_capturing():
        return False

    def ask():
        d = _ibn_desc(x, half, relu, 1e-5)
        d.bn.training = int(bool(bn_training))
        return all(_ffi.lib().cnsn_ibn_plan(C.byref(d), int(has_addend), back) == 1 for back in (0, 1))
    key = (tuple(x.shape), x.dtype, x.device.index, int(half), bool(relu), bool(has_addend), bool(bn_training))
    return _remembered(_ibn_plan_cache, key, ask)


class IBNorm(torch.autograd.Function):

    @staticmethod
    def forward(ctx, x, addend, in_w, in_b, bn_w, bn_b, bn_rm, bn_rv, half, relu, eps_in, bn_training, bn_eps, bn_momentum,
                bn_nbt=None):
        _require_device(x, "cnsn_forward_ibn")
        with torch.cuda.device(x.device):
            lib = _ffi.lib()
            _ffi.check_resident_health("cnsn_forward_ibn")
            x, addend = _cl_inputs(x, addend, "cnsn_forward_ibn")
            dev = x.device
            iw = _f32(in_w) if in_w is not None else None
            ib = _f32(in_b) if in_b is not None else None
            bn = _Bn2dBuffers(bn_w, bn_b, bn_rm, bn_rv, bn_eps, bn_momentum, bn_nbt, bn_training) if half < x.shape[1] else None
            d = _ibn_desc(x, half, relu, eps_in, iw, ib, bn.c if bn else None)
            d.context, d.context_bytes = _nhwc_context(x)
            need_bwd = any(ctx.needs_input_grad)
            saved = torch.empty(lib.cnsn_ibn_saved_floats(C.byref(d)), dtype=torch.float32, device=dev) if need_bwd else None
            ws_bytes = lib.cnsn_ibn_workspace_bytes(C.byref(d))
            ws = _workspace(ws_bytes, dev)
            y = _out_like(x)
            st = lib.cnsn_forward_ibn(C.byref(d), _ptr(x), _ptr(addend), _ptr(y), _ptr(saved), _ptr(ws), ws_bytes, _stream(x))
            _ffi.check(st, "cnsn_forward_ibn")
            if bn:
                bn.write_back()
            if need_bwd:
                ctx.desc, ctx.keep = d, (iw, ib, bn)
                ctx.has_addend = addend is not None
                ctx.param_dtypes = tuple(t.dtype if t is not None else None for t in (in_w, in_b, bn_w, bn_b))
                ctx.save_for_backward(x, addend, saved)
            return y

    @staticmethod
    def backward(ctx, gy):
        x, addend, saved = ctx.saved_tensors
        with torch.cuda.device(x.device):
            lib = _ffi.lib()
            d = ctx.desc
            dev = x.device
            c, half = int(x.shape[1]), int(d.half)
            gy = _grad_like(gy, x, True)
            d.context, d.context_bytes = _nhwc_context(x)
            dx = _out_like(x)
            flat = torch.empty(2 * c, dtype=torch.float32, device=dev)
            diw, dib, dbw, dbb = flat[:half], flat[half:2 * half], flat[2 * half:c + half], flat[c + half:]
            pd = ctx.param_dtypes
            ws_bytes = lib.cnsn_ibn_workspace_bytes(C.byref(d))
            ws = _workspace(ws_bytes, dev)
            st = lib.cnsn_backward_ibn(C.byref(d), _ptr(gy), _ptr(x), _ptr(addend), _ptr(saved), _ptr(dx),
                                       _ptr(diw) if pd[0] is not None else None, _ptr(dib) if pd[1] is not None else None,
                                       _ptr(dbw) if pd[2] is not None else None, _ptr(dbb) if pd[3] is not None else None,
                                       _ptr(ws), ws_bytes, _stream(x))
            _ffi.check(st, "cnsn_backward_ibn")
            grads = _cast_grads((diw, dib, dbw, dbb), pd)
            return (dx, dx if ctx.has_addend else None, grads[0], grads[1], grads[2], grads[3], None, None, None, None, None, None, None,
                    None, None)


_bn_act_plan_cache = _plan_cache()


def _bn_act_desc(x: torch.Tensor, relu: bool, has_addend: bool, bn: Optional[_ffi.BnTail] = None, training: bool = True):
    n, c, h, w = _dims(x)
    d = _ffi.BnAct()
    d.struct_bytes = C.sizeof(_ffi.BnAct)
    d.dtype, d.N, d.C, d.H, d.W = _DTYPES[x.dtype], n, c, h, w
    d.relu, d.add = int(bool(relu)), int(bool(has_addend))
    if bn is not None:
        d.bn = bn
    else:
        d.bn.struct_bytes = C.sizeof(_ffi.BnTail)
    d.bn.training = int(bool(training))
    return d


def bn_act_plan(x: torch.Tensor, relu: bool = True, has_addend: bool = False, training: bool = True) -> bool:
    if not _single_launch_tensor(x, poll=training):
        return False

    def ask():
        d = _bn_act_desc(x, relu, has_addend, training=training)
        return all(_ffi.lib().cnsn_bn_act_plan(C.byref(d), int(has_addend), back) == 1 for back in ((0, 1) if training else (0,)))
    return _remembered(_bn_act_plan_cache, (tuple(x.shape), x.dtype, x.device.index, bool(relu), bool(has_addend), bool(training)), ask)


class BatchNormAct(torch.autograd.Function):

    @staticmethod
    def forward(ctx, x, addend, bn_w, bn_b, bn_rm, bn_rv, relu, training, bn_eps, bn_momentum, bn_nbt=None):
        _require_device(x, "cnsn_forward_bn_act")
        with torch.cuda.device(x.device):
            lib = _ffi.lib()
            if training:
                _ffi.check_resident_health("cnsn_forward_bn_act")
            x, addend = _cl_inputs(x, addend, "cnsn_forward_bn_act")
            dev = x.device
            bn = _Bn2dBuffers(bn_w, bn_b, bn_rm, bn_rv, bn_eps, bn_momentum, bn_nbt, training)
            d = _bn_act_desc(x, relu, addend is not None, bn.c, training)
            need_bwd = bool(training) and any(ctx.needs_input_grad)
            if training:
                d.context, d.context_bytes = _nhwc_context(x)
            saved = torch.empty(lib.cnsn_bn_act_saved_floats(C.byref(d)), dtype=torch.float32, device=dev) if need_bwd else None
            ws_bytes = lib.cnsn_bn_act_workspace_bytes(C.byref(d))
            ws = _workspace(ws_bytes, dev)
            y = _out_like(x)
            st = lib.cnsn_forward_bn_act(C.byref(d), _ptr(x), _ptr(addend), _ptr(y), _ptr(saved), _ptr(ws), ws_bytes, _stream(x))
            _ffi.check(st, "cnsn_forward_bn_act")
            bn.write_back()
            if not training:
                ctx.mark_non_differentiable(y)
            if need_bwd:
                ctx.desc, ctx.keep = d, bn
                ctx.has_addend, ctx.relu = addend is not None, bool(relu)
                ctx.param_dtypes = (bn_w.dtype, bn_b.dtype)
                ctx.save_for_backward(x, addend if relu else None, saved)
            return y

    @staticmethod
    def backward(ctx, gy):
        x, addend, saved = ctx.saved_tensors
        with torch.cuda.device(x.device):
            lib = _ffi.lib()
            d = ctx.desc
            dev = x.device
            c = int(x.shape[1])
            gy = _grad_like(gy, x, True)
            d.context, d.context_bytes = _nhwc_context(x)
            dx = _out_like(x)
            da = _out_like(x) if addend is not None else None
            dw, db = torch.empty(2 * c, dtype=torch.float32, device=dev).view(2, c).unbind(0)
            ws_bytes = lib.cnsn_bn_act_workspace_bytes(C.byref(d))
            ws = _workspace(ws_bytes, dev)
            st = lib.cnsn_backward_bn_act(C.byref(d), _ptr(gy), _ptr(x), _ptr(addend), _ptr(saved), _ptr(dx), _ptr(da), _ptr(dw),
                                          _ptr(db), _ptr(ws), ws_bytes, _stream(x))
            _ffi.check(st, "cnsn_backward_bn_act")
            if ctx.has_addend and da is None:
                da = gy
            dw, db = _cast_grads((dw, db), ctx.param_dtypes)
            return dx, (da if ctx.has_addend else None), dw, db, None, None, None, None, None, None, None


class JsdConsistency(torch.autograd.Function):

    @staticmethod
    @_on_device_of
    def forward(ctx, l0, l1, l2):
        lib = _ffi.lib()
        for t in (l0, l1, l2):
            if not (isinstance(t, torch.Tensor) and t.is_cuda):
                raise _ffi.CnsnError("jsd_consistency: HIP device tensors only")
        assert l0.dim() == 2 and l0.shape == l1.shape == l2.shape and l0.dtype == l1.dtype == l2.dtype
        if l0.dtype not in _DTYPES:
            raise TypeError(f"jsd_consistency: dtype {l0.dtype} not supported")
        l0, l1, l2 = _dense(l0), _dense(l1), _dense(l2)
        b, k = int(l0.shape[0]), int(l0.shape[1])
        need = any(ctx.needs_input_grad)
        loss = torch.empty((), dtype=torch.float32, device=l0.device)
        grads = torch.empty((3, b, k), dtype=l0.dtype, device=l0.device) if need else None
        wsb = lib.cnsn_jsd_workspace_bytes(b)
        ws = torch.empty(wsb // 4 + 1, dtype=torch.float32, device=l0.device)
        st = lib.cnsn_jsd(_ptr(l0), _ptr(l1), _ptr(l2), _DTYPES[l0.dtype], b, k, _ptr(loss),
                          _ptr(grads[0]) if need else None, _ptr(grads[1]) if need else None,
                          _ptr(grads[2]) if need else None, _ptr(ws), wsb, _stream(l0))
        _ffi.check(st, "cnsn_jsd")
        if need:
            ctx.save_for_backward(grads)
        return loss

    @staticmethod
    def backward(ctx, gloss):
        (grads,) = ctx.saved_tensors
        g = grads * gloss.to(grads.dtype)
        return g[0], g[1], g[2]


def jsd_consistency(logits_clean, logits_aug1, logits_aug2):
    return JsdConsistency.apply(logits_clean, logits_aug1, logits_aug2)
```

### include/cnsn_hip.h

```cpp
#ifndef CNSN_HIP_H_
#define CNSN_HIP_H_

#include <stddef.h>
#include <stdint.h>

#ifdef __cplusplus
extern "C" {
#endif

#define CNSN_ABI_VERSION 9

#define CNSN_PERM_INLINE_MAX 1024

enum cnsn_dtype { CNSN_F32 = 0, CNSN_BF16 = 1, CNSN_F16 = 2 };

enum cnsn_status {
    CNSN_OK = 0,
    CNSN_E_NULL = -1,
    CNSN_E_SHAPE = -2,
    CNSN_E_DTYPE = -3,
    CNSN_E_ALIGN = -4,
    CNSN_E_BOX = -5,
    CNSN_E_WORKSPACE = -6,
    CNSN_E_BATCH = -7,
    CNSN_E_STRUCT = -8,
    CNSN_E_UNSUPPORTED = -9
};

enum cnsn_layout { CNSN_LAYOUT_NCHW = 0, CNSN_LAYOUT_NHWC = 1 };

enum cnsn_strategy {
    CNSN_STRATEGY_AUTO = 0,
    CNSN_STRATEGY_TWO_PASS = 1,
    CNSN_STRATEGY_RESIDENT = 2,
    CNSN_STRATEGY_LOCAL = 3,
    CNSN_STRATEGY_MONO = 4
};

typedef struct cnsn_problem {
    int32_t struct_bytes;
    int32_t dtype;
    int32_t N, C, H, W;
    int32_t cn_active;
    int32_t content_box[4];
    int32_t style_box[4];
    float lam;
    float eps_cn;
    int32_t sn_active;
    int32_t sn_two;
    int32_t sn_training;
    float eps_sn;
    float eps_bn;
    float momentum;
    int32_t strategy;
    int32_t layout;
    void* context;
    uint64_t context_bytes;
    const int64_t* perm_host;
} cnsn_problem_t;

typedef struct cnsn_gate {
    const float* fc_weight;
    const float* bn_weight;
    const float* bn_bias;
    float* running_mean;
    float* running_var;
    int64_t* num_batches_tracked;
} cnsn_gate_t;

typedef struct cnsn_gate_grad {
    float* d_fc_weight;
    float* d_bn_weight;
    float* d_bn_bias;
} cnsn_gate_grad_t;

int cnsn_abi_version(void);
const char* cnsn_status_string(int status);

size_t cnsn_saved_floats(const cnsn_problem_t* prob);
size_t cnsn_workspace_bytes(const cnsn_problem_t* prob);

int cnsn_forward(const cnsn_problem_t* prob, const void* x, const int64_t* perm,
                 const int64_t* chan_perm, const cnsn_gate_t* g, const cnsn_gate_t* f, void* y,
                 float* saved, void* workspace, size_t workspace_bytes, void* stream);

int cnsn_backward(const cnsn_problem_t* prob, const void* grad_y, const void* x,
                  const int64_t* perm, const int64_t* chan_perm, const cnsn_gate_t* g,
                  const cnsn_gate_t* f, const float* saved, void* grad_x,
                  const cnsn_gate_grad_t* dg, const cnsn_gate_grad_t* df, void* workspace,
                  size_t workspace_bytes, void* stream);

enum cnsn_add_mode {
    CNSN_ADD_NONE = 0,
    CNSN_ADD_PRE = 1,
    CNSN_ADD_POST = 2
};

typedef struct cnsn_epilogue {
    int32_t struct_bytes;
    int32_t add_mode;
    int32_t relu;
    int32_t reserved;
    const void* addend;
    void* sum_out;
} cnsn_epilogue_t;

int cnsn_keeps_sum(const cnsn_problem_t* prob, const cnsn_epilogue_t* epi);

int cnsn_forward_fused(const cnsn_problem_t* prob, const cnsn_epilogue_t* epi, const void* x,
                       const int64_t* perm, const int64_t* chan_perm, const cnsn_gate_t* g,
                       const cnsn_gate_t* f, void* y, float* saved, void* workspace,
                       size_t workspace_bytes, void* stream);

int cnsn_backward_fused(const cnsn_problem_t* prob, const cnsn_epilogue_t* epi, const void* grad_y,
                        const void* x, const int64_t* perm, const int64_t* chan_perm,
                        const cnsn_gate_t* g, const cnsn_gate_t* f, const float* saved, void* grad_x,
                        void* grad_addend, const cnsn_gate_grad_t* dg, const cnsn_gate_grad_t* df,
                        void* workspace, size_t workspace_bytes, void* stream);

typedef struct cnsn_bn_tail {
    int32_t struct_bytes;
    int32_t training;
    float eps;
    float momentum;
    const float* weight;
    const float* bias;
    float* running_mean;
    float* running_var;
    int64_t* num_batches_tracked;
} cnsn_bn_tail_t;

int cnsn_bnrelu_plan(const cnsn_problem_t* prob, const cnsn_epilogue_t* epi, int backward);
int cnsn_forward_bnrelu(const cnsn_problem_t* prob, const cnsn_epilogue_t* epi, const cnsn_bn_tail_t* tail,
                        const void* x, const cnsn_gate_t* g, void* y, void* z, float* saved, float* bn_stats,
                        void* workspace, size_t workspace_bytes, void* stream);
int cnsn_backward_bnrelu(const cnsn_problem_t* prob, const cnsn_epilogue_t* epi, const cnsn_bn_tail_t* tail,
                         const void* grad_y, const void* grad_z, const void* x, const cnsn_gate_t* g,
                         const float* saved, const float* bn_stats, void* grad_x, const cnsn_gate_grad_t* dg,
                         float* d_bn_weight, float* d_bn_bias, void* workspace, size_t workspace_bytes, void* stream);

int cnsn_plane_stats(const void* x, int dtype, int N, int C, int H, int W, const int32_t* box,
                     float eps, float* mean_std, void* stream);

int cnsn_plane_stats_backward(const void* x, int dtype, int N, int C, int H, int W,
                              const int32_t* box, const float* mean, const float* std,
                              const float* dmean, const float* dstd, void* dx, void* stream);

int cnsn_plane_affine(const void* x, int dtype, int N, int C, int H, int W, const float* scale,
                      const float* shift, void* y, void* stream);

int cnsn_plane_dot(const void* g, const void* x, int dtype, int N, int C, int H, int W,
                   float* sums, void* stream);

int cnsn_plane_dot_shifted(const void* g, const void* x, int dtype, int N, int C, int H, int W,
                           const double* shift, float* sums, void* stream);
int cnsn_plane_combine(const void* g, const void* x, int dtype, int N, int C, int H, int W, const float* coef,
                       void* out, void* stream);

enum cnsn_path {
    CNSN_PATH_STREAMING = 0,
    CNSN_PATH_PACKED = 1,
    CNSN_PATH_RESIDENT = 2,
    CNSN_PATH_LOCAL = 3,
    CNSN_PATH_MONO = 4
};
int cnsn_which_path(const cnsn_problem_t* prob, const cnsn_epilogue_t* epi, int has_chan_perm, int backward);
int cnsn_sn_cluster_plan(const cnsn_problem_t* prob, const cnsn_epilogue_t* epi, int backward);

int cnsn_bn_block_plan(const cnsn_problem_t* prob, const cnsn_epilogue_t* epi);
int cnsn_forward_bn_block(const cnsn_problem_t* prob, const cnsn_epilogue_t* epi, const cnsn_bn_tail_t* bn,
                          const cnsn_bn_tail_t* bn_skip, const void* conv_out, const cnsn_gate_t* g, void* y, float* saved,
                          float* bn_stats, void* workspace, size_t workspace_bytes, void* stream);
int cnsn_backward_bn_block(const cnsn_problem_t* prob, const cnsn_epilogue_t* epi, const cnsn_bn_tail_t* bn,
                           const cnsn_bn_tail_t* bn_skip, const void* grad_y, const void* conv_out, const cnsn_gate_t* g,
                           const float* saved, const float* bn_stats, void* grad_conv_out, void* grad_identity,
                           const cnsn_gate_grad_t* dg, float* d_bn_weight, float* d_bn_bias, float* d_bn_skip_weight,
                           float* d_bn_skip_bias, void* workspace, size_t workspace_bytes, void* stream);

typedef struct cnsn_ibn {
    int32_t struct_bytes;
    int32_t dtype;
    int32_t N, C, H, W;
    int32_t half;
    int32_t relu;
    float eps_in;
    int32_t reserved;
    const float* in_weight;
    const float* in_bias;
    cnsn_bn_tail_t bn;
    void* context;
    uint64_t context_bytes;
} cnsn_ibn_t;

int cnsn_ibn_plan(const cnsn_ibn_t* desc, int has_addend, int backward);
size_t cnsn_ibn_saved_floats(const cnsn_ibn_t* desc);
size_t cnsn_ibn_workspace_bytes(const cnsn_ibn_t* desc);
int cnsn_forward_ibn(const cnsn_ibn_t* desc, const void* x, const void* addend, void* y, float* saved, void* workspace,
                     size_t workspace_bytes, void* stream);
int cnsn_backward_ibn(const cnsn_ibn_t* desc, const void* grad_y, const void* x, const void* addend, const float* saved,
                      void* grad_x, float* d_in_weight, float* d_in_bias, float* d_bn_weight, float* d_bn_bias, void* workspace,
                      size_t workspace_bytes, void* stream);

typedef struct cnsn_bn_act {
    int32_t struct_bytes;
    int32_t dtype;
    int32_t N, C, H, W;
    int32_t relu;
    int32_t add;
    cnsn_bn_tail_t bn;
    void* context;
    uint64_t context_bytes;
} cnsn_bn_act_t;

int cnsn_bn_act_plan(const cnsn_bn_act_t* desc, int has_addend, int backward);
size_t cnsn_bn_act_saved_floats(const cnsn_bn_act_t* desc);
size_t cnsn_bn_act_workspace_bytes(const cnsn_bn_act_t* desc);
int cnsn_forward_bn_act(const cnsn_bn_act_t* desc, const void* x, const void* addend, void* y, float* saved, void* workspace,
                        size_t workspace_bytes, void* stream);
int cnsn_backward_bn_act(const cnsn_bn_act_t* desc, const void* grad_y, const void* x, const void* addend, const float* saved,
                         void* grad_x, void* grad_addend, float* d_weight, float* d_bias, void* workspace, size_t workspace_bytes,
                         void* stream);

size_t cnsn_context_bytes(const cnsn_problem_t* prob);
int cnsn_context_init(void* context, size_t bytes, void* stream);

int cnsn_resident_timeouts(void);
int cnsn_resident_rearm(void);
int cnsn_resident_degraded(void);
void cnsn_resident_enable(int on);

void cnsn_set_wait_ms(int ms);
int cnsn_wait_ms(void);

void cnsn_set_headroom_cus(int n);
int cnsn_headroom_cus(void);

typedef struct cnsn_arena_stats {
    int32_t struct_bytes;
    int32_t device;
    uint64_t chunk_bytes;
    uint64_t mapped_bytes;
    uint64_t in_use_bytes;
    uint64_t blocks, blocks_in_use;
    uint64_t hits;
    uint64_t misses;
    uint64_t failed;
    uint64_t probed;
    uint64_t tries;
    uint64_t evicted;
    uint64_t limit_bytes;
    uint64_t broken;
} cnsn_arena_stats_t;
void* cnsn_arena_map(size_t bytes, int device, void* stream);
void cnsn_arena_unmap(void* ptr, size_t bytes, int device, void* stream);
void* cnsn_arena_alloc(int device, size_t bytes, void* stream);
int cnsn_arena_free(void* ptr);
int cnsn_arena_record_stream(void* ptr, void* stream);
int cnsn_arena_set_limit(int device, uint64_t bytes);
size_t cnsn_arena_trim(int device);
int cnsn_arena_owns(const void* ptr);
int cnsn_arena_stats(int device, cnsn_arena_stats_t* out);
int cnsn_arena_prospect(int device, size_t bytes, int keep, int candidates, void* stream, float* gbps_out);
int cnsn_arena_set_tries(int tries);
int cnsn_arena_block_gbps(const void* ptr, float* gbps);
int cnsn_arena_set_chunk_bytes(size_t chunk_bytes);

void cnsn_reload_env(void);

size_t cnsn_jsd_workspace_bytes(int B);
int cnsn_jsd(const void* logits_clean, const void* logits_aug1, const void* logits_aug2, int dtype, int B,
             int K, float* loss, void* d_clean, void* d_aug1, void* d_aug2, void* workspace,
             size_t workspace_bytes, void* stream);

#ifdef __cplusplus
}
#endif
#endif
```

Baseline: 8704.

## Fuse residual-fork gradient sum into bn-block backward kernel

Each ResNet bottleneck now returns its output twice, once for the next block's main path and once for its identity path. The two incoming gradients then reach the fused bn-block backward separately instead of being added by autograd. The backward kernel gets a SUM2 template variant that loads both gradient tensors and adds them in registers, so the separate elementwise add pass and its temporary tensor go away. In exchange the kernel reads one more tensor per element. The keep-first-read caching heuristic and the autograd plumbing get more complex, with a fallback to a plain add when layouts don't match.

New measurement: 8715, median of 3. No clear change (+0.1%).

```diff
diff --git a/crossnorm-selfnorm_amd/_ffi.py b/crossnorm-selfnorm_amd/_ffi.py
--- a/crossnorm-selfnorm_amd/_ffi.py
+++ b/crossnorm-selfnorm_amd/_ffi.py
@@ -124,6 +124,10 @@
                                          C.c_void_p, C.POINTER(Gate), C.c_void_p, C.c_void_p, C.c_void_p, C.c_void_p,
                                          C.POINTER(GateGrad), C.c_void_p, C.c_void_p, C.c_void_p, C.c_void_p, C.c_void_p, C.c_size_t,
                                          C.c_void_p]),
+    "cnsn_backward_bn_block_fork": (C.c_int, [C.POINTER(Problem), C.POINTER(Epilogue), C.POINTER(BnTail), C.POINTER(BnTail),
+                                              C.c_void_p, C.c_void_p, C.c_void_p, C.POINTER(Gate), C.c_void_p, C.c_void_p,
+                                              C.c_void_p, C.c_void_p, C.POINTER(GateGrad), C.c_void_p, C.c_void_p, C.c_void_p,
+                                              C.c_void_p, C.c_void_p, C.c_size_t, C.c_void_p]),
     "cnsn_forward_bnrelu": (C.c_int, [C.POINTER(Problem), C.POINTER(Epilogue), C.POINTER(BnTail), C.c_void_p,
                                       C.POINTER(Gate), C.c_void_p, C.c_void_p, C.c_void_p, C.c_void_p, C.c_void_p,
                                       C.c_size_t, C.c_void_p]),
diff --git a/crossnorm-selfnorm_amd/callers/_sites.py b/crossnorm-selfnorm_amd/callers/_sites.py
--- a/crossnorm-selfnorm_amd/callers/_sites.py
+++ b/crossnorm-selfnorm_amd/callers/_sites.py
@@ -6,6 +6,7 @@
 FUSE_BLOCK = os.environ.get("CNSN_FUSE_BLOCK", "1") != "0"
 FUSE_TAIL = FUSE_BLOCK and os.environ.get("CNSN_FUSE_TAIL", "1") != "0"
 FUSE_BN_ACT = os.environ.get("CNSN_BN_ACT", "1") != "0"
+FUSE_FORK = os.environ.get("CNSN_FORK_SUM", "1") != "0"
 
 
 def residual_sum(cnsn, pos, residual, skip, relu, skip_first=False):
diff --git a/crossnorm-selfnorm_amd/callers/resnet.py b/crossnorm-selfnorm_amd/callers/resnet.py
--- a/crossnorm-selfnorm_amd/callers/resnet.py
+++ b/crossnorm-selfnorm_amd/callers/resnet.py
@@ -31,8 +31,9 @@
             self.cnsn = make_cnsn(impl, cnsn_type, crop, beta, c_in if pos == "pre" else c_out)
         self.pos = pos if cnsn_type is not None else None
 
-    def forward(self, x):
-        h = self.cnsn(x) if self.pos == "pre" else x
+    def forward(self, x, fork=False):
+        x, main = (x[1], x[0]) if isinstance(x, tuple) else (x, x)
+        h = self.cnsn(main) if self.pos == "pre" else main
         h = self.conv1(h)
         h = self.bn1.forward_act(h) if self.ibn == "a" else bn_act(self.bn1, h)
         h = bn_act(self.bn2, self.conv2(h))
@@ -47,11 +48,12 @@
             return self.IN.forward_act(h, skip, relu=True)
         fb = getattr(getattr(self, "cnsn", None), "forward_bn_block", None) if (_sites.FUSE_BLOCK and self.pos == "post") else None
         if fb is not None and h.is_cuda:
+            kw = dict(fork=True) if fork else {}
             if self.downsample is None:
-                return fb(h, self.bn3, x, relu=True)
+                return fb(h, self.bn3, x, relu=True, **kw)
             if len(self.downsample) == 2 and isinstance(self.downsample[1], nn.BatchNorm2d):
-                return fb(h, self.bn3, self.downsample[0](x), relu=True, identity_bn=self.downsample[1])
-            return fb(h, self.bn3, self.downsample(x), relu=True)
+                return fb(h, self.bn3, self.downsample[0](x), relu=True, identity_bn=self.downsample[1], **kw)
+            return fb(h, self.bn3, self.downsample(x), relu=True, **kw)
         skip = x if self.downsample is None else self.downsample(x)
         if getattr(self, "cnsn", None) is None:
             return bn_act(self.bn3, h, skip)
@@ -94,5 +96,11 @@
         if aug:
             self._enable_cross_norm()
         x = self.maxpool(bn_act(self.bn1, self.conv1(x)))
-        x = self.layer4(self.layer3(self.layer2(self.layer1(x))))
+        if _sites.FUSE_FORK:
+            blocks = [b for layer in (self.layer1, self.layer2, self.layer3, self.layer4) for b in layer]
+            for b in blocks[:-1]:
+                x = b(x, fork=True)
+            x = blocks[-1](x)
+        else:
+            x = self.layer4(self.layer3(self.layer2(self.layer1(x))))
         return self.fc(torch.flatten(self.avgpool(x), 1))
diff --git a/crossnorm-selfnorm_amd/cnsn.py b/crossnorm-selfnorm_amd/cnsn.py
--- a/crossnorm-selfnorm_amd/cnsn.py
+++ b/crossnorm-selfnorm_amd/cnsn.py
@@ -268,7 +268,7 @@
         cfg = FusedConfig(add_mode=add_mode, relu=bool(relu), **kw)
         return _F.fused_cnsn(x, cfg, perm=perm, chan_perm=chan, g=g, f=f, addend=addend)
 
-    def forward_bn_block(self, conv_out, bn, identity, relu=True, identity_bn=None):
+    def forward_bn_block(self, conv_out, bn, identity, relu=True, identity_bn=None, fork=False):
         cn, sn = self.crossnorm, self.selfnorm
         armed = cn is not None and cn.active
 
@@ -293,7 +293,7 @@
             extra = (identity_bn.weight, identity_bn.bias, identity_bn.running_mean, identity_bn.running_var, e2, m2, c2)
         return _F.FusedBnBlock.apply(conv_out, identity, cfg, g.fc_weight, g.bn_weight, g.bn_bias, g.running_mean, g.running_var,
                                      bn.weight, bn.bias, bn.running_mean, bn.running_var, bn_eps, bn_mom, g.num_batches_tracked,
-                                     bn_counter, *extra)
+                                     bn_counter, *(extra or (None, None, None, None, 0.0, 0.0, None)), bool(fork))
 
     def forward_block_bn(self, x, addend, add_mode, bn, want_y=True):
         assert add_mode in ("none", "pre")
diff --git a/crossnorm-selfnorm_amd/csrc/cnsn_env.h b/crossnorm-selfnorm_amd/csrc/cnsn_env.h
--- a/crossnorm-selfnorm_amd/csrc/cnsn_env.h
+++ b/crossnorm-selfnorm_amd/csrc/cnsn_env.h
@@ -31,6 +31,7 @@
     K_MID_BLOCK,
     K_NHWC_FUSED,
     K_ARENA_MAX_MB,
+    K_FORK_KEEP,
     K_COUNT
 };
 
diff --git a/crossnorm-selfnorm_amd/csrc/cnsn_env.hip b/crossnorm-selfnorm_amd/csrc/cnsn_env.hip
--- a/crossnorm-selfnorm_amd/csrc/cnsn_env.hip
+++ b/crossnorm-selfnorm_amd/csrc/cnsn_env.hip
@@ -21,6 +21,7 @@
     "CNSN_MID_BLOCK",
     "CNSN_NHWC_FUSED",
     "CNSN_ARENA_MAX_MB",
+    "CNSN_FORK_KEEP",
 };
 
 struct Table {
diff --git a/crossnorm-selfnorm_amd/csrc/cnsn_fused.hip b/crossnorm-selfnorm_amd/csrc/cnsn_fused.hip
--- a/crossnorm-selfnorm_amd/csrc/cnsn_fused.hip
+++ b/crossnorm-selfnorm_amd/csrc/cnsn_fused.hip
@@ -166,6 +166,17 @@
                            const float* bn_stats, void* grad_conv_out, void* grad_identity, const cnsn_gate_grad_t* dg, float* d_bn_weight,
                            float* d_bn_bias, float* d_bn_skip_weight, float* d_bn_skip_bias, void* workspace, size_t workspace_bytes,
                            void* stream_) {
+    return cnsn_backward_bn_block_fork(prob, epi, bn, bn_skip, grad_y, nullptr, conv_out, g, saved, bn_stats, grad_conv_out,
+                                       grad_identity, dg, d_bn_weight, d_bn_bias, d_bn_skip_weight, d_bn_skip_bias, workspace,
+                                       workspace_bytes, stream_);
+}
+
+int cnsn_backward_bn_block_fork(const cnsn_problem_t* prob, const cnsn_epilogue_t* epi, const cnsn_bn_tail_t* bn,
+                                const cnsn_bn_tail_t* bn_skip, const void* grad_y, const void* grad_y2, const void* conv_out,
+                                const cnsn_gate_t* g, const float* saved, const float* bn_stats, void* grad_conv_out,
+                                void* grad_identity, const cnsn_gate_grad_t* dg, float* d_bn_weight, float* d_bn_bias,
+                                float* d_bn_skip_weight, float* d_bn_skip_bias, void* workspace, size_t workspace_bytes,
+                                void* stream_) {
     if (!bn) return CNSN_E_NULL;
     if (bn_skip && (bn_skip->struct_bytes != (int32_t)sizeof(cnsn_bn_tail_t))) return CNSN_E_STRUCT;
     if (bn_skip && (!bn_skip->weight || !d_bn_skip_weight || !d_bn_skip_bias)) return CNSN_E_NULL;
@@ -174,12 +185,12 @@
     const int st = bn_block_parse(prob, epi, bn, pl, e, false, false);
     if (st) return st;
     if (!grad_y || !conv_out || !grad_conv_out || !grad_identity || !saved || !bn_stats || !workspace || !bn->weight) return CNSN_E_NULL;
-    if ((((uintptr_t)grad_y | (uintptr_t)conv_out | (uintptr_t)grad_conv_out | (uintptr_t)grad_identity | (uintptr_t)workspace |
-          (uintptr_t)bn_stats) & 15u) != 0)
+    if ((((uintptr_t)grad_y | (uintptr_t)grad_y2 | (uintptr_t)conv_out | (uintptr_t)grad_conv_out | (uintptr_t)grad_identity |
+          (uintptr_t)workspace | (uintptr_t)bn_stats) & 15u) != 0)
         return CNSN_E_ALIGN;
     if (!gate_ok(g) || !dg || !dg->d_fc_weight || !dg->d_bn_weight || !dg->d_bn_bias) return CNSN_E_NULL;
-    return nhwc_bnhead_backward(pl, e.relu, *bn, bn_skip, grad_y, conv_out, e.addend, gate_dev(g), saved, bn_stats, grad_conv_out,
-                                grad_identity, gate_grad_dev(dg), d_bn_weight, d_bn_bias, d_bn_skip_weight, d_bn_skip_bias, workspace,
+    return nhwc_bnhead_backward(pl, e.relu, *bn, bn_skip, grad_y, grad_y2, conv_out, e.addend, gate_dev(g), saved, bn_stats,
+                                grad_conv_out, grad_identity, gate_grad_dev(dg), d_bn_weight, d_bn_bias, d_bn_skip_weight, d_bn_skip_bias, workspace,
                                 workspace_bytes, (hipStream_t)stream_);
 }
 
diff --git a/crossnorm-selfnorm_amd/csrc/cnsn_nhwc.h b/crossnorm-selfnorm_amd/csrc/cnsn_nhwc.h
--- a/crossnorm-selfnorm_amd/csrc/cnsn_nhwc.h
+++ b/crossnorm-selfnorm_amd/csrc/cnsn_nhwc.h
@@ -79,8 +79,8 @@
 size_t nhwc_bnhead_extra_bytes(const Plan& pl);
 int nhwc_bnhead_forward(Plan& pl, int relu, const cnsn_bn_tail_t& bn, const cnsn_bn_tail_t* bn2, const void* conv_out, const void* identity,
                         GateDev gg, void* y, float* saved, float* bn_stats, void* workspace, size_t workspace_bytes, hipStream_t stream);
-int nhwc_bnhead_backward(Plan& pl, int relu, const cnsn_bn_tail_t& bn, const cnsn_bn_tail_t* bn2, const void* gy, const void* conv_out,
-                         const void* identity, GateDev gg, const float* saved, const float* bn_stats, void* d_conv, void* d_identity,
+int nhwc_bnhead_backward(Plan& pl, int relu, const cnsn_bn_tail_t& bn, const cnsn_bn_tail_t* bn2, const void* gy, const void* gy2,
+                         const void* conv_out, const void* identity, GateDev gg, const float* saved, const float* bn_stats, void* d_conv, void* d_identity,
                          GateGradDev dg, float* dbn_w, float* dbn_b, float* dbn2_w, float* dbn2_b, void* workspace,
                          size_t workspace_bytes, hipStream_t stream);
 
diff --git a/crossnorm-selfnorm_amd/csrc/cnsn_nhwc_bnhead_kernels.h b/crossnorm-selfnorm_amd/csrc/cnsn_nhwc_bnhead_kernels.h
--- a/crossnorm-selfnorm_amd/csrc/cnsn_nhwc_bnhead_kernels.h
+++ b/crossnorm-selfnorm_amd/csrc/cnsn_nhwc_bnhead_kernels.h
@@ -370,8 +370,9 @@
     }
 }
 
-template <typename T, int VEC, bool KEEP, bool TWO>
+template <typename T, int VEC, bool KEEP, bool TWO, bool SUM2 = false>
 __global__ __launch_bounds__(kBlock, TWO ? 2 : CNSN_BNHEAD_WG_PER_CU) void nhwc_bnhead_bwd_kernel(NhwcBnArgs a, const T* __restrict__ gy,
+                                                                                         const T* __restrict__ gy2,
                                                                                          const T* __restrict__ cv,
                                                                                          const T* __restrict__ idt, T* __restrict__ dconv,
                                                                                          T* __restrict__ didt, GateDev gg, GateGradDev dg) {
@@ -408,12 +409,13 @@
                 load_planes<VEC>(st2 + (size_t)BS_BETA * g.C + ch, be2);
                 load_planes<VEC>(st2 + (size_t)BS_MEAN * g.C + ch, m2ch);
             }
-            auto eat = [&](const Vec<T, VEC>& vg, const Vec<T, VEC>& vc, const Vec<T, VEC>& vb) {
+            auto eat = [&](const Vec<T, VEC>& vg, const Vec<T, VEC>& vh, const Vec<T, VEC>& vc, const Vec<T, VEC>& vb) {
 #pragma unroll
                 for (int j = 0; j < VEC; ++j) {
                     const float c = to_float(vc.v[j]), c2 = to_float(vb.v[j]);
                     const float X = bn_sum<T>(c, bn_skip<T, TWO>(c2, al2[TWO ? j : 0], be2[TWO ? j : 0]), al[j], be[j]);
                     float G = to_float(vg.v[j]);
+                    if constexpr (SUM2) G = sum_t<T>(G, to_float(vh.v[j]));
                     if (relu) G = relu_open<T>(gate[j] * X) ? G : 0.f;
                     acc[0][j] += G;
                     acc[1][j] = fmaf(G, X - mu[j], acc[1][j]);
@@ -423,20 +425,22 @@
             };
             int p = t.p0 + t.r;
             for (; p + g.rows < t.p1; p += 2 * g.rows) {
-                Vec<T, VEC> vg[2], vc[2], vb[2];
+                Vec<T, VEC> vg[2], vh[SUM2 ? 2 : 1], vc[2], vb[2];
 #pragma unroll
                 for (int u = 0; u < 2; ++u) {
                     const size_t e = t.elem(g, p + u * g.rows);
                     vg[u] = nhwc_ld<T, VEC, !KEEP>(gy + e);
+                    if constexpr (SUM2) vh[u] = nhwc_ld<T, VEC, !KEEP>(gy2 + e);
                     vc[u] = nhwc_ld<T, VEC, !KEEP>(cv + e);
                     vb[u] = nhwc_ld<T, VEC, !KEEP>(idt + e);
                 }
 #pragma unroll
-                for (int u = 0; u < 2; ++u) eat(vg[u], vc[u], vb[u]);
+                for (int u = 0; u < 2; ++u) eat(vg[u], vh[SUM2 ? u : 0], vc[u], vb[u]);
             }
             for (; p < t.p1; p += g.rows) {
                 const size_t e = t.elem(g, p);
-                eat(nhwc_ld<T, VEC, !KEEP>(gy + e), nhwc_ld<T, VEC, !KEEP>(cv + e), nhwc_ld<T, VEC, !KEEP>(idt + e));
+                const Vec<T, VEC> vg = nhwc_ld<T, VEC, !KEEP>(gy + e);
+                eat(vg, SUM2 ? nhwc_ld<T, VEC, !KEEP>(gy2 + e) : vg, nhwc_ld<T, VEC, !KEEP>(cv + e), nhwc_ld<T, VEC, !KEEP>(idt + e));
             }
         }
         nhwc_rows_sum_part<VEC, 3, kBnBwd>(g, t, acc, 0, lds, a.f.part);
@@ -602,13 +606,14 @@
             eb.load<VEC>(2 * (size_t)g.C + ch, e0b);
             eb.load<VEC>(3 * (size_t)g.C + ch, e1b);
         }
-        auto emit = [&](const Vec<T, VEC>& vg, const Vec<T, VEC>& vc, const Vec<T, VEC>& vb, size_t e) {
+        auto emit = [&](const Vec<T, VEC>& vg, const Vec<T, VEC>& vh, const Vec<T, VEC>& vc, const Vec<T, VEC>& vb, size_t e) {
             Vec<T, VEC> o, od;
 #pragma unroll
             for (int j = 0; j < VEC; ++j) {
                 const float c = to_float(vc.v[j]), c2 = to_float(vb.v[j]);
                 const float X = bn_sum<T>(c, bn_skip<T, TWO>(c2, al2[TWO ? j : 0], be2[TWO ? j : 0]), al[j], be[j]);
                 float G = to_float(vg.v[j]);
+                if constexpr (SUM2) G = sum_t<T>(G, to_float(vh.v[j]));
                 if (relu) G = relu_open<T>(cG[j] * X) ? G : 0.f;
                 const float dX = fmaf(cG[j], G, fmaf(cX[j], X - xr[j], c0[j]));
                 if constexpr (TWO)
@@ -623,9 +628,10 @@
         const int cnt = (t.p1 - t.p0 - t.r + g.rows - 1) / g.rows;
         for (int q = cnt - 1; q >= 0; --q) {
             const size_t e = t.elem(g, t.p0 + t.r + q * g.rows);
-            emit(load_vec_nt<T, VEC>(gy + e), load_vec_nt<T, VEC>(cv + e), load_vec_nt<T, VEC>(idt + e), e);
-        }
-    }
-}
-
-}
+            const Vec<T, VEC> vg = load_vec_nt<T, VEC>(gy + e);
+            emit(vg, SUM2 ? load_vec_nt<T, VEC>(gy2 + e) : vg, load_vec_nt<T, VEC>(cv + e), load_vec_nt<T, VEC>(idt + e), e);
+        }
+    }
+}
+
+}
diff --git a/crossnorm-selfnorm_amd/csrc/cnsn_nhwc_fused.hip b/crossnorm-selfnorm_amd/csrc/cnsn_nhwc_fused.hip
--- a/crossnorm-selfnorm_amd/csrc/cnsn_nhwc_fused.hip
+++ b/crossnorm-selfnorm_amd/csrc/cnsn_nhwc_fused.hip
@@ -202,8 +202,8 @@
     return status;
 }
 
-int nhwc_bnhead_backward(Plan& pl, int relu, const cnsn_bn_tail_t& bn, const cnsn_bn_tail_t* bn2, const void* gy, const void* conv_out,
-                         const void* identity, GateDev gg, const float* saved, const float* bn_stats, void* d_conv, void* d_identity,
+int nhwc_bnhead_backward(Plan& pl, int relu, const cnsn_bn_tail_t& bn, const cnsn_bn_tail_t* bn2, const void* gy, const void* gy2,
+                         const void* conv_out, const void* identity, GateDev gg, const float* saved, const float* bn_stats, void* d_conv, void* d_identity,
                          GateGradDev dg, float* dbn_w, float* dbn_b, float* dbn2_w, float* dbn2_b, void* workspace,
                          size_t workspace_bytes, hipStream_t stream) {
     if (!nhwc_bnhead_ok(pl, false) || !bn.training || (bn2 && !bn2->training)) return CNSN_E_UNSUPPORTED;
@@ -217,25 +217,29 @@
     a.dbn_b = dbn_b;
     a.dbn2_w = dbn2_w;
     a.dbn2_b = dbn2_b;
-    a.f.keep = keep_first_read(3, tensor_bytes(pl));
+    a.f.keep = keep_first_read(gy2 ? 4 : 3, tensor_bytes(pl));
+    if (const char* e = gy2 ? knob(K_FORK_KEEP) : nullptr) a.f.keep = e[0] == '1' ? 1 : (e[0] == '0' ? 0 : a.f.keep);
     int status = CNSN_E_UNSUPPORTED;
     dispatch_t(pl.pr.dtype, [&](auto tt, auto vt) {
         using T = typename decltype(tt)::type;
         constexpr int VEC = decltype(vt)::value;
         const size_t lds = (size_t)3 * ng.rows * ng.tcb * VEC * 4;
         auto go = [&](auto kern) {
-            status = launch_fused(pl, kern, lds, a, a.f, w.bar, stream, (const T*)gy, (const T*)conv_out, (const T*)identity,
-                                  (T*)d_conv, (T*)d_identity, gg, dg);
-        };
-        if (bn2)
-            a.f.keep ? go(nhwc_bnhead_bwd_kernel<T, VEC, true, true>) : go(nhwc_bnhead_bwd_kernel<T, VEC, false, true>);
-        else
-            a.f.keep ? go(nhwc_bnhead_bwd_kernel<T, VEC, true, false>) : go(nhwc_bnhead_bwd_kernel<T, VEC, false, false>);
+            status = launch_fused(pl, kern, lds, a, a.f, w.bar, stream, (const T*)gy, (const T*)gy2, (const T*)conv_out,
+                                  (const T*)identity, (T*)d_conv, (T*)d_identity, gg, dg);
+        };
+        with_flag(bn2 != nullptr, [&](auto two) {
+            with_flag(gy2 != nullptr, [&](auto sum2) {
+                constexpr bool TWO = decltype(two)::value, SUM2 = decltype(sum2)::value;
+                a.f.keep ? go(nhwc_bnhead_bwd_kernel<T, VEC, true, TWO, SUM2>) : go(nhwc_bnhead_bwd_kernel<T, VEC, false, TWO, SUM2>);
+            });
+        });
     });
     if (knob(K_DEBUG))
         fprintf(stderr, "[cnsn] nhwc bn-block bwd: tiles=%d (S=%d rows=%d tcb=%d) groups=%d keep=%d -> status %d\n", a.f.ntiles, ng.S,
                 ng.rows, ng.tcb, a.f.ngroups, a.f.keep, status);
-    return status;
-}
-
-}
+    if (gy2 && knob(K_DEBUG)) fprintf(stderr, "[cnsn] nhwc bn-block bwd: two gradients (grad_y = grad_y + grad_y2 in the launch)\n");
+    return status;
+}
+
+}
diff --git a/crossnorm-selfnorm_amd/functional.py b/crossnorm-selfnorm_amd/functional.py
--- a/crossnorm-selfnorm_amd/functional.py
+++ b/crossnorm-selfnorm_amd/functional.py
@@ -601,12 +601,25 @@
     return _remembered(_bn_block_plan_cache, (tuple(x.shape), x.dtype, x.device.index, cfg.relu, cfg.sn_two, _strategy), ask)
 
 
+FORK_COUNTS = {"two": 0, "added": 0, "one": 0}
+_FORK_MIN_BYTES = int(float(os.environ.get("CNSN_FORK_SUM_MIN_MB", "0")) * (1 << 20))
+
+
+def fork_sum_takes(x: torch.Tensor) -> bool:
+    return x.numel() * x.element_size() >= _FORK_MIN_BYTES
+
+
+def _launch_reads(g: torch.Tensor, x: torch.Tensor) -> bool:
+    return (g.dtype == x.dtype and g.shape == x.shape and g.is_contiguous(memory_format=torch.channels_last)
+            and g.data_ptr() % 16 == 0)
+
+
 class FusedBnBlock(torch.autograd.Function):
 
     @staticmethod
     def forward(ctx, conv_out, identity, cfg: FusedConfig, g_w, g_gamma, g_beta, g_rm, g_rv, bn_w, bn_b, bn_rm, bn_rv, bn_eps,
                 bn_momentum, g_nbt=None, bn_nbt=None, bn2_w=None, bn2_b=None, bn2_rm=None, bn2_rv=None, bn2_eps=0.0,
-                bn2_momentum=0.0, bn2_nbt=None):
+                bn2_momentum=0.0, bn2_nbt=None, fork=False):
         _require_device(conv_out, "cnsn_forward_bn_block")
         with torch.cuda.device(conv_out.device):
             lib = _ffi.lib()
@@ -639,15 +652,30 @@
                 ctx.param_dtypes = (g_w.dtype, g_gamma.dtype, g_beta.dtype, bn_w.dtype, bn_b.dtype,
                                     bn2_w.dtype if skip else None, bn2_b.dtype if skip else None)
                 ctx.save_for_backward(x, idt, saved, stats)
-            return y
-
-    @staticmethod
-    def backward(ctx, gy):
+            ctx.fork = bool(fork)
+            if not fork:
+                return y
+            ctx.set_materialize_grads(False)
+            return y, y.detach()
+
+    @staticmethod
+    def backward(ctx, gy, gy2=None):
+        if gy is None:
+            gy, gy2 = gy2, None
+        if gy is None:
+            return (None,) * 24
         x, idt, saved, stats = ctx.saved_tensors
         with torch.cuda.device(x.device):
             lib = _ffi.lib()
             cfg, prob, gate, head, skip = ctx.cfg, ctx.prob, ctx.gate, ctx.head, ctx.skip
             dev = x.device
+            if gy2 is None:
+                FORK_COUNTS["one"] += int(ctx.fork)
+            elif fork_sum_takes(x) and _launch_reads(gy, x) and _launch_reads(gy2, x):
+                FORK_COUNTS["two"] += 1
+            else:
+                gy, gy2 = gy + gy2, None
+                FORK_COUNTS["added"] += 1
             gy = _grad_like(gy, x, True)
             hs = head.struct()
             ss = skip.struct() if skip else None
@@ -660,14 +688,14 @@
                 prob.context, prob.context_bytes = None, 0
             ws = _workspace(ws_bytes, dev)
             epi = _epilogue(cfg, idt)
-            st = lib.cnsn_backward_bn_block(C.byref(prob), C.byref(epi), C.byref(hs), C.byref(ss) if ss else None, _ptr(gy), _ptr(x),
-                                            C.byref(gate.c), _ptr(saved), _ptr(stats), _ptr(d_conv), _ptr(d_idt), C.byref(gg),
-                                            _ptr(dbw), _ptr(dbb), _ptr(d2w) if skip else None, _ptr(d2b) if skip else None, _ptr(ws),
-                                            ws_bytes, _stream(x))
-            _ffi.check(st, "cnsn_backward_bn_block")
+            st = lib.cnsn_backward_bn_block_fork(C.byref(prob), C.byref(epi), C.byref(hs), C.byref(ss) if ss else None, _ptr(gy),
+                                                 _ptr(gy2), _ptr(x), C.byref(gate.c), _ptr(saved), _ptr(stats), _ptr(d_conv),
+                                                 _ptr(d_idt), C.byref(gg), _ptr(dbw), _ptr(dbb), _ptr(d2w) if skip else None,
+                                                 _ptr(d2b) if skip else None, _ptr(ws), ws_bytes, _stream(x))
+            _ffi.check(st, "cnsn_backward_bn_block_fork" if gy2 is not None else "cnsn_backward_bn_block")
             outs = _cast_grads(grads, ctx.param_dtypes)
             return (d_conv, d_idt, None, outs[0], outs[1], outs[2], None, None, outs[3], outs[4], None, None, None, None, None, None,
-                    outs[5], outs[6], None, None, None, None, None)
+                    outs[5], outs[6], None, None, None, None, None, None)
 
 
 def _glue_cfg(cfg: FusedConfig, need_bwd: bool, inline: bool = False):
diff --git a/include/cnsn_hip.h b/include/cnsn_hip.h
--- a/include/cnsn_hip.h
+++ b/include/cnsn_hip.h
@@ -176,6 +176,12 @@
                            const float* saved, const float* bn_stats, void* grad_conv_out, void* grad_identity,
                            const cnsn_gate_grad_t* dg, float* d_bn_weight, float* d_bn_bias, float* d_bn_skip_weight,
                            float* d_bn_skip_bias, void* workspace, size_t workspace_bytes, void* stream);
+int cnsn_backward_bn_block_fork(const cnsn_problem_t* prob, const cnsn_epilogue_t* epi, const cnsn_bn_tail_t* bn,
+                                const cnsn_bn_tail_t* bn_skip, const void* grad_y, const void* grad_y2, const void* conv_out,
+                                const cnsn_gate_t* g, const float* saved, const float* bn_stats, void* grad_conv_out,
+                                void* grad_identity, const cnsn_gate_grad_t* dg, float* d_bn_weight, float* d_bn_bias,
+                                float* d_bn_skip_weight, float* d_bn_skip_bias, void* workspace, size_t workspace_bytes,
+                                void* stream);
 
 typedef struct cnsn_ibn {
     int32_t struct_bytes;
```
